# samukallio/path-tracer

Measured on AMD Instinct MI355X. Metric: Mrays/s + Msamples/s, Viking Room 1920x1080 1024spp, 1/2/4/8 GPUs, higher is better.
Workload: dtype f32; 1 GPU; C3 scene, one 1920x1080 1024-spp frame per step (Reset, Run(2), Run(1) until the frame's sample count reaches 1024 x pixels); each of 1 GPU(s) renders every pixel with its own RNG stream to 1/1 of the samples, then the reduce of radiance + sample counts to rank 0; spp_target=1024, streams=1, slots_per_launch_rank0=2073600, split=3, class_lists=False, frame_target_samples_rank0=2123366400, mesh_faces=3976, parallelism=sample-shards x1

## Files before the change

include/pt_api.h:

```cpp
#ifndef PT_API_H
#define PT_API_H

#include <stdint.h>
#include "pt_packed.h"

#ifdef __cplusplus
extern "C" {
#endif

typedef struct pt_device pt_device;
typedef struct pt_scene pt_scene;
typedef struct pt_sample_buffer pt_sample_buffer;
typedef struct pt_basic_renderer pt_basic_renderer;
typedef struct pt_comm pt_comm;
typedef struct pt_preview pt_preview;
typedef struct pt_denoise_guides pt_denoise_guides;

typedef struct pt_basic_renderer_params {
    uint32_t FrameIndex;
    uint32_t CameraIndex;
    uint32_t RenderFlags;
    uint32_t PathLengthLimit;
    float    PathTerminationProbability;
} pt_basic_renderer_params;

typedef struct pt_hit_record {
    float    time;
    uint32_t shape_material;
    uint32_t packed_normal;
    uint32_t packed_tangent;
    float    u, v;
} pt_hit_record;

typedef struct pt_pixel_state {
    float    origin[3];
    uint32_t packed_velocity;
    pt_hit_record hit;
    float    lambda0;
    float    throughput[4];
    float    probability[4];
    float    sample[3];
    uint32_t active01, active23;
} pt_pixel_state;

enum {
    PT_KERNEL_RAYGEN  = 0,
    PT_KERNEL_EXTEND  = 1,
    PT_KERNEL_SHADE   = 2,
    PT_KERNEL_RESOLVE = 3,
    PT_KERNEL_PREVIEW = 4,
    PT_KERNEL_ROUND   = 5,
    PT_KERNEL_ROUNDS  = 6,
    PT_KERNEL_DENOISE = 7,
    PT_KERNEL_GUIDES  = 8,
    PT_KERNEL_STATS   = 9,
    PT_KERNEL_REPROJECT = 10,
    PT_KERNEL_COUNT   = 11,
};

enum {
    PT_TONE_MAPPING_CLAMP    = 0,
    PT_TONE_MAPPING_REINHARD = 1,
    PT_TONE_MAPPING_HABLE    = 2,
    PT_TONE_MAPPING_ACES     = 3,
};

enum {
    PT_PREVIEW_RENDER_MODE_BASE_COLOR        = 0,
    PT_PREVIEW_RENDER_MODE_BASE_COLOR_SHADED = 1,
    PT_PREVIEW_RENDER_MODE_NORMAL            = 2,
    PT_PREVIEW_RENDER_MODE_MATERIAL_INDEX    = 3,
    PT_PREVIEW_RENDER_MODE_PRIMITIVE_INDEX   = 4,
    PT_PREVIEW_RENDER_MODE_MESH_COMPLEXITY   = 5,
    PT_PREVIEW_RENDER_MODE_SCENE_COMPLEXITY  = 6,
};

typedef struct pt_preview_parameters {
    pt_packed_transform CameraTransform;
    uint32_t RenderMode;
    float    Brightness;
    uint32_t SelectedShapeIndex;
    uint32_t RenderSizeX, RenderSizeY;
    uint32_t MouseX, MouseY;
} pt_preview_parameters;

typedef struct pt_preview_aov {
    float    time;
    uint32_t shape_index;
    uint32_t material_index;
    uint32_t primitive_index;
    uint32_t mesh_complexity;
    uint32_t scene_complexity;
    float    normal[3];
    float    u, v;
    uint32_t reserved;
} pt_preview_aov;

typedef struct pt_resolve_parameters {
    float    Brightness;
    uint32_t ToneMappingMode;
    float    ToneMappingWhiteLevel;
} pt_resolve_parameters;

const char* ptGetLastError(void);

pt_device* ptCreateDevice(int hip_device);
void       ptDestroyDevice(pt_device* device);
int        ptSynchronize(pt_device* device);
int        ptGetDeviceCount(int* count);

pt_scene* ptCreateScene(pt_device* device);
int       ptUpdateScene(pt_device* device, pt_scene* scene, const pt_scene_packs* packs, uint32_t dirty_flags);
void      ptDestroyScene(pt_device* device, pt_scene* scene);
enum {
    PT_STACK_FORMAT_AUTO       = 0,
    PT_STACK_FORMAT_WORDS32    = 1,
    PT_STACK_FORMAT_NODE_INDEX = 2,
    PT_HIT_RECORD_AUTO         = 0,
    PT_HIT_RECORD_FACE_INDEX   = 1,
};
int       ptSetSceneStackFormat(pt_scene* scene, uint32_t format);
int       ptSetSceneHitRecordForm(pt_scene* scene, uint32_t form);
enum {
    PT_EXTEND_FORM_AUTO    = 0,
    PT_EXTEND_FORM_GENERAL = 1,
    PT_EXTEND_FORM_MESH    = 2,
};
int       ptSetSceneExtendForm(pt_scene* scene, uint32_t form);
int       ptGetSceneExtendForm(pt_scene* scene, uint32_t* form);
int       ptSceneStackNeeded(pt_scene* scene, uint32_t* entries);
int       ptSceneNodeCache(pt_scene* scene, uint32_t* pairs);

pt_sample_buffer* ptCreateSampleBuffer(pt_device* device, uint32_t width, uint32_t height);
void              ptDestroySampleBuffer(pt_device* device, pt_sample_buffer* buffer);
int               ptReadSampleBuffer(pt_device* device, pt_sample_buffer* buffer, float* rgba);
int               ptWriteSampleBuffer(pt_device* device, pt_sample_buffer* buffer, const float* rgba);
int               ptRenderSampleBuffer(pt_device* device, pt_sample_buffer* buffer, const pt_resolve_parameters* params);
int               ptReadResolvedImage(pt_device* device, pt_sample_buffer* buffer, float* rgba);
int               ptReadResolvedImageSRGB8(pt_device* device, pt_sample_buffer* buffer, uint8_t* rgba8);

pt_basic_renderer* ptCreateBasicRenderer(pt_device* device, pt_scene* scene, pt_sample_buffer* buffer);
pt_basic_renderer* ptCreateBasicRendererPartitioned(pt_device* device, pt_scene* scene, pt_sample_buffer* buffer,
                                                    uint32_t rank, uint32_t nranks);
pt_basic_renderer* ptCreateBasicRendererStreams(pt_device* device, pt_scene* scene, pt_sample_buffer* buffer,
                                                uint32_t rank, uint32_t nranks, uint32_t streams);
int                ptMergeBasicRendererStreams(pt_device* device, pt_basic_renderer* renderer);
uint32_t           ptBasicRendererStreams(pt_basic_renderer* renderer);
void               ptDestroyBasicRenderer(pt_device* device, pt_basic_renderer* renderer);
pt_basic_renderer_params* ptBasicRendererParams(pt_basic_renderer* renderer);
int                ptResetBasicRenderer(pt_device* device, pt_basic_renderer* renderer);
int                ptRunBasicRenderer(pt_device* device, pt_basic_renderer* renderer, uint32_t rounds);
uint32_t           ptBasicRendererSlotCount(pt_basic_renderer* renderer);
int                ptSetBasicRendererFusedRounds(pt_basic_renderer* renderer, int mode);
int                ptRunBasicRendererRounds(pt_device* device, pt_basic_renderer* renderer, uint32_t count);
int                ptSetBasicRendererRoundBatch(pt_basic_renderer* renderer, uint32_t rounds);
#define PT_MAX_SPLIT 4
int                ptSetBasicRendererClassLists(pt_basic_renderer* renderer, uint32_t mode);
int                ptGetBasicRendererClassLists(const pt_basic_renderer* renderer, uint32_t* used);
enum { PT_RAY_ORDER_AUTO = 0, PT_RAY_ORDER_OCTANT = 1, PT_RAY_ORDER_LENGTH = 2 };
int                ptSetBasicRendererRayOrder(pt_basic_renderer* renderer, uint32_t order);
int                ptGetBasicRendererRayOrder(const pt_basic_renderer* renderer, uint32_t* order, uint32_t* used);
int                ptReadSceneLengthTable(pt_device* device, pt_scene* scene, uint8_t* classes, uint32_t* trained,
                                          uint64_t* rounds);
int                ptReadBasicRendererRayPositions(pt_device* device, pt_basic_renderer* renderer, uint16_t* positions);
int                ptSetBasicRendererSplit(pt_basic_renderer* renderer, uint32_t groups);
int                ptGetBasicRendererSplit(const pt_basic_renderer* renderer, uint32_t* groups, uint32_t* timed_tiles,
                                           uint32_t* tiles);
int                ptSetBasicRendererActiveTiles(pt_device* device, pt_basic_renderer* renderer, const uint8_t* mask,
                                                 uint32_t tiles);
int                ptGetBasicRendererActiveTiles(const pt_basic_renderer* renderer, uint32_t* active, uint32_t* tiles);
int                ptSetBasicRendererOpenPBR(pt_basic_renderer* renderer, int enable);
int                ptGetStats(pt_device* device, pt_basic_renderer* renderer, uint64_t* rays, uint64_t* samples);
int                ptRenderFrame(pt_device* device, pt_basic_renderer* renderer, uint64_t target_samples,
                                 uint32_t max_rounds, uint32_t* rounds_out, uint64_t* samples_out);
int                ptReadBasicRendererState(pt_device* device, pt_basic_renderer* renderer, pt_pixel_state* out);
int                ptReadBasicRendererStreamState(pt_device* device, pt_basic_renderer* renderer, uint32_t stream,
                                                  pt_pixel_state* out);
int                ptWriteBasicRendererState(pt_device* device, pt_basic_renderer* renderer, const pt_pixel_state* in);
int                ptWriteBasicRendererStreamState(pt_device* device, pt_basic_renderer* renderer, uint32_t stream,
                                                   const pt_pixel_state* in);
int                ptReadBasicRendererStreamAccumulator(pt_device* device, pt_basic_renderer* renderer, uint32_t stream,
                                                        float* rgba);
int                ptWriteBasicRendererStreamAccumulator(pt_device* device, pt_basic_renderer* renderer,
                                                         uint32_t stream, const float* rgba);

enum {
    PT_SHADE_DIFFUSE     = 1,
    PT_SHADE_METAL       = 2,
    PT_SHADE_TRANSLUCENT = 4,
    PT_SHADE_SCATTER     = 8,
    PT_SHADE_OPENPBR     = 16,
    PT_SHADE_PRIMS       = 32,
    PT_SHADE_SKY         = 64,
    PT_SHADE_TEXWRAP     = 128,
};
typedef struct pt_shade_info {
    uint32_t scene_mask;
    uint32_t kernel_mask;
    uint32_t completion_queue;
    uint32_t grey_records;
    uint32_t ray_order;
    uint32_t length_trained;
} pt_shade_info;
int                ptGetBasicRendererShadeInfo(pt_basic_renderer* renderer, pt_shade_info* info);

pt_preview* ptCreatePreviewRenderContext(pt_device* device, pt_scene* scene);
void        ptDestroyPreviewRenderContext(pt_device* device, pt_preview* context);
int         ptRenderPreview(pt_device* device, pt_preview* context, const pt_preview_parameters* params);
int         ptRetrievePreviewQueryResult(pt_device* device, pt_preview* context, uint32_t* hit_shape_index);
int         ptReadPreviewImage(pt_device* device, pt_preview* context, float* rgba);
int         ptReadPreviewAOVs(pt_device* device, pt_preview* context, pt_preview_aov* aov);

pt_denoise_guides* ptCreateDenoiseGuides(pt_device* device, uint32_t width, uint32_t height);
void ptDestroyDenoiseGuides(pt_device* device, pt_denoise_guides* guides);
int  ptRenderDenoiseGuides(pt_device* device, pt_scene* scene, pt_denoise_guides* guides, uint32_t camera_index);
#define PT_GUIDE_MAX_BOUNCES 8
int  ptRenderDenoiseGuidesSpecular(pt_device* device, pt_scene* scene, pt_denoise_guides* guides,
                                   uint32_t camera_index, uint32_t max_bounces);
int  ptReadDenoiseGuides(pt_device* device, pt_denoise_guides* guides, pt_denoise_guide* out);
int  ptWriteDenoiseGuides(pt_device* device, pt_denoise_guides* guides, const pt_denoise_guide* in);
int  ptDenoiseSampleBuffer(pt_device* device, pt_sample_buffer* src, pt_denoise_guides* guides,
                           const pt_denoise_parameters* params, pt_sample_buffer* dst);
enum {
    PT_DENOISE_VARIANT_AUTO    = 0,
    PT_DENOISE_VARIANT_GATHER  = 1,
    PT_DENOISE_VARIANT_LATTICE = 2,
};
int  ptSetDenoiseVariant(pt_denoise_guides* guides, uint32_t variant);
int  ptDenoiseSampleBufferPair(pt_device* device, pt_sample_buffer* a, pt_sample_buffer* b, pt_denoise_guides* guides,
                               const pt_denoise_pair_parameters* params, pt_sample_buffer* dst);
int  ptDespikeSampleBuffer(pt_device* device, pt_sample_buffer* src, pt_denoise_guides* guides,
                           const pt_despike_parameters* params, pt_sample_buffer* dst);

int  ptReprojectSampleBuffer(pt_device* device, pt_sample_buffer* prev, pt_denoise_guides* prev_guides,
                             const pt_packed_camera* prev_camera, pt_denoise_guides* guides,
                             const pt_packed_camera* camera, const pt_reproject_parameters* params,
                             pt_sample_buffer* dst);
int  ptReprojectSampleBufferMoving(pt_device* device, pt_sample_buffer* prev, pt_denoise_guides* prev_guides,
                                   const pt_packed_camera* prev_camera, pt_denoise_guides* guides,
                                   const pt_packed_camera* camera, const pt_shape_motion* motion,
                                   uint32_t motion_count, const pt_reproject_parameters* params,
                                   pt_sample_buffer* dst);
int  ptRectifyHistory(pt_device* device, pt_sample_buffer* history, pt_sample_buffer* current,
                      pt_denoise_guides* guides, const pt_rectify_parameters* params, pt_sample_buffer* dst);

int  ptComputeFrameStatistics(pt_device* device, pt_sample_buffer* a, pt_sample_buffer* b,
                              pt_frame_statistics* out);
int  ptComputeTileStatistics(pt_device* device, pt_sample_buffer* a, pt_sample_buffer* b, float noise_threshold,
                             pt_tile_statistics* out);
int  ptAccumulateSampleBuffer(pt_device* device, pt_sample_buffer* dst, pt_sample_buffer* src);
enum {
    PT_STATS_VARIANT_AUTO    = 0,
    PT_STATS_VARIANT_PLAIN   = 1,
    PT_STATS_VARIANT_UNIFORM = 2,
};
int  ptSetFrameStatisticsVariant(pt_device* device, uint32_t variant);

int ptTraceRays(pt_device* device, pt_scene* scene, uint32_t n, const float* origins,
                const uint32_t* packed_velocities, const float* durations, pt_hit_record* out);

int ptCheckFastDivision(pt_device* device, uint64_t n, uint32_t seed, uint64_t* mismatches);

int ptCheckFastReciprocal(pt_device* device, uint64_t* mismatches);

int ptEvalNumerics(pt_device* device, uint32_t op, uint32_t n, const uint32_t* a, const uint32_t* b,
                   const uint32_t* c, uint32_t* out);

int ptSampleTextures(pt_device* device, pt_scene* scene, uint32_t n, const uint32_t* texture_index,
                     const float* uv, uint32_t wrap, float* rgba);

#define PT_EXTEND_STATS_COUNT 14
int ptExtendStats(pt_device* device, pt_basic_renderer* renderer, uint64_t out[PT_EXTEND_STATS_COUNT]);
int ptExtendStepCounts(pt_device* device, pt_basic_renderer* renderer, uint32_t* steps);

int ptTraceRaysStats(pt_device* device, pt_scene* scene, uint32_t n, const float* origins,
                     const uint32_t* packed_velocities, const float* durations,
                     uint64_t out[PT_EXTEND_STATS_COUNT], uint32_t* steps);

int ptSetProfiling(pt_device* device, int enable);
int ptSetProfilingPeriod(pt_device* device, uint32_t period);
int ptGetKernelStats(pt_device* device, int kernel, uint64_t* launches, double* total_ms);
int ptGetKernelRounds(pt_device* device, int kernel, uint64_t* rounds);
int ptResetKernelStats(pt_device* device);

enum {
    PT_ERROR_COMM_ABORTED = -2,
    PT_ERROR_TIMEOUT      = -3,
};
int      ptCommGetUniqueId(uint8_t id[128]);
pt_comm* ptCommCreate(pt_device* device, int nranks, int rank, const uint8_t id[128]);
void     ptCommDestroy(pt_comm* comm);
int      ptCommSetTimeout(pt_comm* comm, double seconds);
int      ptCommReduceSampleBuffer(pt_device* device, pt_comm* comm, pt_sample_buffer* buffer, int root);
int      ptCommGatherSampleBuffer(pt_device* device, pt_comm* comm, pt_sample_buffer* buffer, int root);
int      ptCommReduceSampleBufferInto(pt_device* device, pt_comm* comm, pt_sample_buffer* buffer,
                                      pt_sample_buffer* total, int root);

#ifdef __cplusplus
}
#endif

#endif
```

path-tracer_amd/_native.py:

```python
from __future__ import annotations

import ctypes as C
import os
from pathlib import Path

import numpy as np

PKG = Path(__file__).resolve().parent
SCENE_LIB_PATH = PKG / "libptscene.so"
HIP_LIB_PATH = PKG / "libpathtracer.so"


class NativeLibraryMissing(RuntimeError):
    pass



class pt_scene_packs(C.Structure):
    _fields_ = [
        ("globals", C.c_void_p),
        ("textures", C.c_void_p), ("texture_count", C.c_uint32),
        ("material_data", C.c_void_p), ("material_word_count", C.c_uint32),
        ("shapes", C.c_void_p), ("shape_count", C.c_uint32),
        ("shape_nodes", C.c_void_p), ("shape_node_count", C.c_uint32),
        ("mesh_faces", C.c_void_p), ("mesh_face_count", C.c_uint32),
        ("mesh_vertices", C.c_void_p), ("mesh_vertex_count", C.c_uint32),
        ("mesh_nodes", C.c_void_p), ("mesh_node_count", C.c_uint32),
        ("cameras", C.c_void_p), ("camera_count", C.c_uint32),
        ("atlas", C.c_void_p),
        ("atlas_width", C.c_uint32), ("atlas_height", C.c_uint32), ("atlas_layer_count", C.c_uint32),
    ]


class pt_shade_info(C.Structure):
    _fields_ = [("scene_mask", C.c_uint32), ("kernel_mask", C.c_uint32), ("completion_queue", C.c_uint32),
                ("grey_records", C.c_uint32), ("ray_order", C.c_uint32), ("length_trained", C.c_uint32)]


RAY_ORDER_AUTO, RAY_ORDER_OCTANT, RAY_ORDER_LENGTH = 0, 1, 2
RAYKEY_COUNT = 32768


SHADE_DIFFUSE, SHADE_METAL, SHADE_TRANSLUCENT, SHADE_SCATTER = 1, 2, 4, 8
SHADE_OPENPBR, SHADE_PRIMS, SHADE_SKY, SHADE_TEXWRAP = 16, 32, 64, 128


class pt_basic_renderer_params(C.Structure):
    _fields_ = [
        ("FrameIndex", C.c_uint32),
        ("CameraIndex", C.c_uint32),
        ("RenderFlags", C.c_uint32),
        ("PathLengthLimit", C.c_uint32),
        ("PathTerminationProbability", C.c_float),
    ]


class pts_load_model_options(C.Structure):
    _fields_ = [
        ("name", C.c_char_p), ("directory_path", C.c_char_p),
        ("vertex_transform", C.c_float * 16), ("normal_transform", C.c_float * 16),
        ("texcoord_transform", C.c_float * 9), ("openpbr_as_diffuse", C.c_int),
    ]


class pt_resolve_parameters(C.Structure):
    _fields_ = [
        ("Brightness", C.c_float),
        ("ToneMappingMode", C.c_uint32),
        ("ToneMappingWhiteLevel", C.c_float),
    ]


class pt_denoise_parameters(C.Structure):
    _fields_ = [
        ("Iterations", C.c_uint32),
        ("SigmaColor", C.c_float),
        ("SigmaNormal", C.c_float),
        ("SigmaDepth", C.c_float),
        ("SigmaAlbedo", C.c_float),
    ]


class pt_denoise_pair_parameters(C.Structure):
    _fields_ = [
        ("Iterations", C.c_uint32),
        ("SigmaLuminance", C.c_float),
        ("SigmaNormal", C.c_float),
        ("SigmaDepth", C.c_float),
        ("SigmaAlbedo", C.c_float),
    ]


class pt_reproject_parameters(C.Structure):
    _fields_ = [
        ("NormalCosine", C.c_float),
        ("DepthTolerance", C.c_float),
        ("MinWeight", C.c_float),
        ("MaxHistory", C.c_float),
    ]


class pt_rectify_parameters(C.Structure):
    _fields_ = [
        ("Radius", C.c_uint32),
        ("MinNeighbours", C.c_uint32),
        ("Sigma", C.c_float),
        ("ClampedHistory", C.c_float),
        ("NormalCosine", C.c_float),
    ]


assert C.sizeof(pt_rectify_parameters) == 20


class pt_despike_parameters(C.Structure):
    _fields_ = [
        ("Radius", C.c_uint32),
        ("Rank", C.c_uint32),
        ("MinNeighbours", C.c_uint32),
        ("Scale", C.c_float),
        ("Floor", C.c_float),
        ("NormalCosine", C.c_float),
    ]


assert C.sizeof(pt_despike_parameters) == 24

STATS_BINS = 256


class pt_frame_statistics(C.Structure):
    _fields_ = [
        ("pixels", C.c_uint64),
        ("filled", C.c_uint64),
        ("empty", C.c_uint64),
        ("nonfinite", C.c_uint64),
        ("dark", C.c_uint64),
        ("luminance_histogram", C.c_uint32 * STATS_BINS),
        ("min_luminance", C.c_float),
        ("max_luminance", C.c_float),
        ("min_samples", C.c_float),
        ("max_samples", C.c_float),
        ("noise_pixels", C.c_uint64),
        ("noise_skipped", C.c_uint64),
        ("noise_histogram", C.c_uint32 * STATS_BINS),
    ]


TILE_SIZE = 16
TILE_STATS_DTYPE = np.dtype([("filled", "<u4"), ("empty", "<u4"), ("nonfinite", "<u4"), ("pair", "<u4"),
                             ("over", "<u4"), ("min_count", "<f4"), ("max_count", "<f4"), ("reserved", "<u4")])
assert TILE_STATS_DTYPE.itemsize == 32


class pt_packed_transform(C.Structure):
    _fields_ = [("To", C.c_float * 16), ("From", C.c_float * 16)]


class pt_packed_camera(C.Structure):
    _fields_ = [
        ("Model", C.c_uint32),
        ("FocalLength", C.c_float),
        ("ApertureRadius", C.c_float),
        ("SensorDistance", C.c_float),
        ("SensorSize", C.c_float * 2),
        ("Pad0", C.c_uint32 * 2),
        ("Transform", pt_packed_transform),
    ]


class pt_preview_parameters(C.Structure):
    _fields_ = [
        ("CameraTransform", pt_packed_transform),
        ("RenderMode", C.c_uint32),
        ("Brightness", C.c_float),
        ("SelectedShapeIndex", C.c_uint32),
        ("RenderSizeX", C.c_uint32), ("RenderSizeY", C.c_uint32),
        ("MouseX", C.c_uint32), ("MouseY", C.c_uint32),
    ]


class pts_config_info(C.Structure):
    _fields_ = [
        ("width", C.c_uint32), ("height", C.c_uint32), ("spp", C.c_uint32), ("camera_count", C.c_uint32),
        ("render_flags", C.c_uint32), ("termination_probability", C.c_float),
        ("mesh_face_count", C.c_uint32), ("shape_count", C.c_uint32),
    ]


HIT_RECORD_DTYPE = np.dtype([
    ("time", "<f4"), ("shape_material", "<u4"), ("packed_normal", "<u4"),
    ("packed_tangent", "<u4"), ("u", "<f4"), ("v", "<f4"),
])
assert HIT_RECORD_DTYPE.itemsize == 24

PIXEL_STATE_DTYPE = np.dtype([
    ("origin", "<f4", (3,)), ("packed_velocity", "<u4"),
    ("hit", HIT_RECORD_DTYPE),
    ("lambda0", "<f4"), ("throughput", "<f4", (4,)), ("probability", "<f4", (4,)),
    ("sample", "<f4", (3,)), ("active01", "<u4"), ("active23", "<u4"),
])
assert PIXEL_STATE_DTYPE.itemsize == 96

PREVIEW_AOV_DTYPE = np.dtype([
    ("time", "<f4"), ("shape_index", "<u4"), ("material_index", "<u4"), ("primitive_index", "<u4"),
    ("mesh_complexity", "<u4"), ("scene_complexity", "<u4"), ("normal", "<f4", (3,)), ("u", "<f4"), ("v", "<f4"),
    ("reserved", "<u4"),
])
assert PREVIEW_AOV_DTYPE.itemsize == 48

DENOISE_GUIDE_DTYPE = np.dtype([("normal", "<f4", (3,)), ("time", "<f4"), ("albedo", "<f4", (3,)), ("shape", "<u4")])
assert DENOISE_GUIDE_DTYPE.itemsize == 32

SHAPE_NODE_DTYPE = np.dtype([("Minimum", "<f4", (3,)), ("ChildNodeIndices", "<u4"),
                             ("Maximum", "<f4", (3,)), ("ShapeIndex", "<u4")])
MESH_NODE_DTYPE = np.dtype([("Minimum", "<f4", (3,)), ("FaceBeginOrNodeIndex", "<u4"),
                            ("Maximum", "<f4", (3,)), ("FaceEndIndex", "<u4")])
MESH_FACE_DTYPE = np.dtype([("Position0", "<f4", (3,)), ("VertexIndex0", "<u4"),
                            ("Position1", "<f4", (3,)), ("VertexIndex1", "<u4"),
                            ("Position2", "<f4", (3,)), ("VertexIndex2", "<u4")])
MESH_VERTEX_DTYPE = np.dtype([("PackedNormal", "<u4"), ("PackedUV", "<u4")])
TRANSFORM_DTYPE = np.dtype([("To", "<f4", (16,)), ("From", "<f4", (16,))])
SHAPE_DTYPE = np.dtype([("Type", "<i4"), ("MaterialIndex", "<u4"), ("MeshRootNodeIndex", "<u4"),
                        ("Pad0", "<u4"), ("Transform", TRANSFORM_DTYPE)])
CAMERA_DTYPE = np.dtype([("Model", "<u4"), ("FocalLength", "<f4"), ("ApertureRadius", "<f4"),
                         ("SensorDistance", "<f4"), ("SensorSize", "<f4", (2,)), ("Pad0", "<u4", (2,)),
                         ("Transform", TRANSFORM_DTYPE)])
TEXTURE_DTYPE = np.dtype([("AtlasPlacementMinimum", "<f4", (2,)), ("AtlasPlacementMaximum", "<f4", (2,)),
                          ("AtlasImageIndex", "<u4"), ("Type", "<u4"), ("Flags", "<u4"), ("Unused0", "<u4")])
GLOBALS_DTYPE = np.dtype([("SkyboxMeanDirection", "<f4", (3,)), ("SkyboxConcentration", "<f4"),
                          ("SkyboxSamplingProbability", "<f4"), ("SkyboxBrightness", "<f4"),
                          ("SkyboxTextureIndex", "<u4"), ("ShapeCount", "<u4"), ("SceneScatterRate", "<f4"),
                          ("Pad0", "<u4", (3,))])
assert SHAPE_NODE_DTYPE.itemsize == 32 and MESH_NODE_DTYPE.itemsize == 32 and MESH_FACE_DTYPE.itemsize == 48
assert SHAPE_DTYPE.itemsize == 144 and CAMERA_DTYPE.itemsize == 160 and GLOBALS_DTYPE.itemsize == 48
assert TEXTURE_DTYPE.itemsize == 32
SHAPE_MOTION_DTYPE = np.dtype([("Point", "<f4", (12,)), ("Normal", "<f4", (9,)), ("Flags", "<u4"),
                               ("Pad0", "<u4", (2,))])
assert SHAPE_MOTION_DTYPE.itemsize == 96
SHAPE_MOTION_MOVED, SHAPE_MOTION_NO_HISTORY = 1, 2

KERNEL_RAYGEN, KERNEL_EXTEND, KERNEL_SHADE, KERNEL_RESOLVE = 0, 1, 2, 3
TONE_MAPPING_CLAMP, TONE_MAPPING_REINHARD, TONE_MAPPING_HABLE, TONE_MAPPING_ACES = 0, 1, 2, 3
(PREVIEW_RENDER_MODE_BASE_COLOR, PREVIEW_RENDER_MODE_BASE_COLOR_SHADED, PREVIEW_RENDER_MODE_NORMAL,
 PREVIEW_RENDER_MODE_MATERIAL_INDEX, PREVIEW_RENDER_MODE_PRIMITIVE_INDEX, PREVIEW_RENDER_MODE_MESH_COMPLEXITY,
 PREVIEW_RENDER_MODE_SCENE_COMPLEXITY) = range(7)
KERNEL_PREVIEW = 4
KERNEL_ROUND = 5
KERNEL_ROUNDS = 6
MAX_SPLIT = 4
KERNEL_DENOISE = 7
KERNEL_GUIDES = 8
GUIDE_MAX_BOUNCES = 8
DENOISE_MAX_ITERATIONS = 8
DENOISE_VARIANT_AUTO, DENOISE_VARIANT_GATHER, DENOISE_VARIANT_LATTICE = 0, 1, 2
KERNEL_STATS = 9
STATS_VARIANT_AUTO, STATS_VARIANT_PLAIN, STATS_VARIANT_UNIFORM = 0, 1, 2
KERNEL_REPROJECT = 10

NUMERICS_OPS = (
    "add", "mul", "div", "sqrt", "fma", "min", "max", "clamp", "floor", "fract", "rint", "round_half_away", "mix",
    "exp", "log", "pow", "sin", "cos", "atan2", "asin", "u32_to_float", "floor_to_int", "random", "random01",
    "pack_snorm16", "unpack_snorm16", "half_to_float", "pack_unit_vector", "unpack_unit_vector", "fast_rcp", "xdiv",
)
NUMERICS_OPERANDS = {"fma": 3, "clamp": 3, "mix": 3, "pack_unit_vector": 3, "add": 2, "mul": 2, "div": 2, "min": 2,
                     "max": 2, "pow": 2, "atan2": 2, "xdiv": 2}
NUMERICS_OUTPUTS = {"random": 2, "unpack_unit_vector": 3}
NUMERICS_DEVICE_ONLY = ("fast_rcp", "xdiv")

_vp = C.c_void_p
_u32 = C.c_uint32
_f32 = C.c_float
_i32 = C.c_int
_fptr = C.POINTER(C.c_float)
_u32ptr = C.POINTER(C.c_uint32)

SCENE_API = {
    "ptsGetLastError": (C.c_char_p, []),
    "ptsCreateScene": (_vp, []),
    "ptsCreateEmptyScene": (_vp, []),
    "ptsCreateConfigScene": (_vp, [_i32, C.POINTER(pts_config_info)]),
    "ptsDestroyScene": (None, [_vp]),
    "ptsSceneRoot": (_vp, [_vp]),
    "ptsCreateEntity": (_vp, [_vp, _i32, _vp]),
    "ptsSetEntityTransform": (None, [_vp, _vp, _fptr, _fptr, _fptr]),
    "ptsSetEntityActive": (None, [_vp, _vp, _i32]),
    "ptsSetEntityMaterial": (None, [_vp, _vp, _vp]),
    "ptsSetEntityMesh": (None, [_vp, _vp, _vp]),
    "ptsEntityPackedShapeIndex": (_u32, [_vp]),
    "ptsSetCameraPinhole": (None, [_vp, _vp, _f32, _f32]),
    "ptsSetCameraThinLens": (None, [_vp, _vp, _f32, _f32, _f32, _f32, _f32]),
    "ptsSetCamera360": (None, [_vp, _vp]),
    "ptsFindCamera": (_vp, [_vp, _u32]),
    "ptsSetCameraTransform": (None, [_vp, _vp, _fptr, _fptr]),
    "ptsSetRootParameters": (None, [_vp, _f32, _f32, _f32, _vp]),
    "ptsCreateMaterial": (_vp, [_vp, _i32, C.c_char_p]),
    "ptsSetMaterialParameter": (_i32, [_vp, _vp, C.c_char_p, _fptr, _i32]),
    "ptsSetMaterialTexture": (_i32, [_vp, _vp, C.c_char_p, _vp]),
    "ptsMaterialPackedIndex": (_u32, [_vp]),
    "ptsCreateCheckerTexture": (_vp, [_vp, C.c_char_p, _i32, _fptr, _fptr]),
    "ptsCreateTexture": (_vp, [_vp, C.c_char_p, _i32, _u32, _u32, _fptr, _i32]),
    "ptsCreateMesh": (_vp, [_vp, C.c_char_p, _u32, _fptr, _fptr, _fptr, _u32, _u32ptr]),
    "ptsMeshDepth": (_u32, [_vp]),
    "ptsMeshNodeCount": (_u32, [_vp]),
    "ptsMeshFaces": (None, [_vp, _u32ptr]),
    "ptsDefaultLoadModelOptions": (None, [C.POINTER(pts_load_model_options)]),
    "ptsLoadTexture": (_vp, [_vp, C.c_char_p, _i32, C.c_char_p]),
    "ptsLoadImageRGBA8": (_i32, [C.c_char_p, C.POINTER(C.c_uint32), C.POINTER(C.c_uint32), _vp]),
    "ptsLoadModelAsPrefab": (_vp, [_vp, C.c_char_p, C.POINTER(pts_load_model_options)]),
    "ptsInstantiatePrefab": (_vp, [_vp, _vp, _vp]),
    "ptsLoadScene": (_vp, [C.c_char_p]),
    "ptsSaveScene": (_i32, [_vp, C.c_char_p]),
    "ptsSceneTextureCount": (_u32, [_vp]),
    "ptsSceneMaterialCount": (_u32, [_vp]),
    "ptsSceneMeshCount": (_u32, [_vp]),
    "ptsScenePrefabCount": (_u32, [_vp]),
    "ptsPrefabMeshCount": (_u32, [_vp]),
    "ptsPrefabMesh": (_vp, [_vp, _u32, C.POINTER(_vp), _fptr]),
    "ptsMeshVertexCount": (_u32, [_vp]),
    "ptsMeshFaceCount": (_u32, [_vp]),
    "ptsMeshVertices": (None, [_vp, _fptr]),
    "ptsMaterialType": (_i32, [_vp]),
    "ptsPackSceneData": (_u32, [_vp]),
    "ptsGetScenePacks": (None, [_vp, C.POINTER(pt_scene_packs)]),
    "ptsMarkDirty": (None, [_vp, _u32]),
    "ptsGetParametricSpectrumCoefficients": (_i32, [_fptr, _fptr]),
    "ptsBuildSpectrumTable": (_i32, [_i32]),
    "ptsSaveSpectrumTable": (_i32, [C.c_char_p]),
    "ptsLoadSpectrumTable": (_i32, [C.c_char_p]),
    "ptsSetSpectrumTablePath": (None, [C.c_char_p]),
    "ptsDenoise": (_i32, [_u32, _u32, _fptr, _vp, C.POINTER(pt_denoise_parameters), _fptr]),
    "ptsDenoisePair": (_i32, [_u32, _u32, _fptr, _fptr, _vp, C.POINTER(pt_denoise_pair_parameters), _fptr]),
    "ptsReproject": (_i32, [_u32, _u32, _fptr, _vp, C.POINTER(pt_packed_camera), _u32, _u32, _vp,
                            C.POINTER(pt_packed_camera), C.POINTER(pt_reproject_parameters), _fptr]),
    "ptsShapeMotion": (_i32, [_vp, _u32, _vp, _u32, _vp]),
    "ptsReprojectMoving": (_i32, [_u32, _u32, _fptr, _vp, C.POINTER(pt_packed_camera), _u32, _u32, _vp,
                                  C.POINTER(pt_packed_camera), _vp, _u32, C.POINTER(pt_reproject_parameters), _fptr]),
    "ptsRectifyHistory": (_i32, [_u32, _u32, _fptr, _fptr, _vp, C.POINTER(pt_rectify_parameters), _fptr]),
    "ptsDespike": (_i32, [_u32, _u32, _fptr, _vp, C.POINTER(pt_despike_parameters), _fptr]),
    "ptsCentralCameraRay": (_i32, [C.POINTER(pt_packed_camera), _u32, _u32, _u32, _u32, _fptr, _fptr]),
    "ptsFrameStatistics": (_i32, [_u32, _u32, _fptr, _fptr, C.POINTER(pt_frame_statistics)]),
    "ptsTileStatistics": (_i32, [_u32, _u32, _fptr, _fptr, _f32, _vp]),
    "ptsStatsBin": (_i32, [C.c_float]),
    "ptsStatsBinEdge": (C.c_double, [_i32]),
    "ptsStatsPercentileBin": (_i32, [_u32ptr, C.c_double]),
    "ptsStatsLogAverage": (C.c_double, [_u32ptr, C.c_double, C.c_double]),
    "ptsStatsAutoBrightness": (C.c_double, [C.POINTER(pt_frame_statistics), C.c_double, C.c_double, C.c_double]),
    "ptsStatsNoise": (C.c_double, [C.POINTER(pt_frame_statistics), C.c_double]),
    "ptsRayKey": (_u32, [_fptr, _fptr, _fptr, _fptr]),
}

HIP_API = {
    "ptGetLastError": (C.c_char_p, []),
    "ptGetDeviceCount": (_i32, [C.POINTER(_i32)]),
    "ptCreateDevice": (_vp, [_i32]),
    "ptDestroyDevice": (None, [_vp]),
    "ptSynchronize": (_i32, [_vp]),
    "ptCreateScene": (_vp, [_vp]),
    "ptUpdateScene": (_i32, [_vp, _vp, C.POINTER(pt_scene_packs), _u32]),
    "ptSetSceneStackFormat": (_i32, [_vp, _u32]),
    "ptSetSceneHitRecordForm": (_i32, [_vp, _u32]),
    "ptSetSceneExtendForm": (_i32, [_vp, _u32]),
    "ptGetSceneExtendForm": (_i32, [_vp, C.POINTER(C.c_uint32)]),
    "ptDestroyScene": (None, [_vp, _vp]),
    "ptCreateSampleBuffer": (_vp, [_vp, _u32, _u32]),
    "ptDestroySampleBuffer": (None, [_vp, _vp]),
    "ptReadSampleBuffer": (_i32, [_vp, _vp, _fptr]),
    "ptWriteSampleBuffer": (_i32, [_vp, _vp, _fptr]),
    "ptRenderSampleBuffer": (_i32, [_vp, _vp, C.POINTER(pt_resolve_parameters)]),
    "ptReadResolvedImage": (_i32, [_vp, _vp, _fptr]),
    "ptReadResolvedImageSRGB8": (_i32, [_vp, _vp, C.POINTER(C.c_uint8)]),
    "ptCreateBasicRenderer": (_vp, [_vp, _vp, _vp]),
    "ptCreateBasicRendererPartitioned": (_vp, [_vp, _vp, _vp, _u32, _u32]),
    "ptCreateBasicRendererStreams": (_vp, [_vp, _vp, _vp, _u32, _u32, _u32]),
    "ptMergeBasicRendererStreams": (_i32, [_vp, _vp]),
    "ptBasicRendererStreams": (_u32, [_vp]),
    "ptReadBasicRendererStreamState": (_i32, [_vp, _vp, _u32, _vp]),
    "ptWriteBasicRendererState": (_i32, [_vp, _vp, _vp]),
    "ptWriteBasicRendererStreamState": (_i32, [_vp, _vp, _u32, _vp]),
    "ptReadBasicRendererStreamAccumulator": (_i32, [_vp, _vp, _u32, _fptr]),
    "ptWriteBasicRendererStreamAccumulator": (_i32, [_vp, _vp, _u32, _fptr]),
    "ptGetBasicRendererShadeInfo": (_i32, [_vp, C.POINTER(pt_shade_info)]),
    "ptDestroyBasicRenderer": (None, [_vp, _vp]),
    "ptBasicRendererParams": (C.POINTER(pt_basic_renderer_params), [_vp]),
    "ptResetBasicRenderer": (_i32, [_vp, _vp]),
    "ptRunBasicRenderer": (_i32, [_vp, _vp, _u32]),
    "ptBasicRendererSlotCount": (_u32, [_vp]),
    "ptSetBasicRendererFusedRounds": (_i32, [_vp, _i32]),
    "ptRunBasicRendererRounds": (_i32, [_vp, _vp, _u32]),
    "ptSetBasicRendererRoundBatch": (_i32, [_vp, _u32]),
    "ptSetBasicRendererSplit": (_i32, [_vp, _u32]),
    "ptSetBasicRendererClassLists": (_i32, [_vp, _u32]),
    "ptGetBasicRendererClassLists": (_i32, [_vp, _u32ptr]),
    "ptGetBasicRendererSplit": (_i32, [_vp, _u32ptr, _u32ptr, _u32ptr]),
    "ptSetBasicRendererRayOrder": (_i32, [_vp, _u32]),
    "ptGetBasicRendererRayOrder": (_i32, [_vp, _u32ptr, _u32ptr]),
    "ptReadSceneLengthTable": (_i32, [_vp, _vp, _vp, _u32ptr, C.POINTER(C.c_uint64)]),
    "ptReadBasicRendererRayPositions": (_i32, [_vp, _vp, _vp]),
    "ptSetBasicRendererOpenPBR": (_i32, [_vp, _i32]),
    "ptGetStats": (_i32, [_vp, _vp, C.POINTER(C.c_uint64), C.POINTER(C.c_uint64)]),
    "ptTraceRaysStats": (_i32, [_vp, _vp, _u32, _fptr, _u32ptr, _fptr, C.POINTER(C.c_uint64), _vp]),
    "ptRenderFrame": (_i32, [_vp, _vp, C.c_uint64, C.c_uint32, C.POINTER(C.c_uint32), C.POINTER(C.c_uint64)]),
    "ptReadBasicRendererState": (_i32, [_vp, _vp, _vp]),
    "ptTraceRays": (_i32, [_vp, _vp, _u32, _fptr, _u32ptr, _fptr, _vp]),
    "ptCreatePreviewRenderContext": (_vp, [_vp, _vp]),
    "ptDestroyPreviewRenderContext": (None, [_vp, _vp]),
    "ptRenderPreview": (_i32, [_vp, _vp, C.POINTER(pt_preview_parameters)]),
    "ptRetrievePreviewQueryResult": (_i32, [_vp, _vp, C.POINTER(C.c_uint32)]),
    "ptReadPreviewImage": (_i32, [_vp, _vp, _fptr]),
    "ptReadPreviewAOVs": (_i32, [_vp, _vp, _vp]),
    "ptCreateDenoiseGuides": (_vp, [_vp, _u32, _u32]),
    "ptDestroyDenoiseGuides": (None, [_vp, _vp]),
    "ptRenderDenoiseGuides": (_i32, [_vp, _vp, _vp, _u32]),
    "ptRenderDenoiseGuidesSpecular": (_i32, [_vp, _vp, _vp, _u32, _u32]),
    "ptReadDenoiseGuides": (_i32, [_vp, _vp, _vp]),
    "ptWriteDenoiseGuides": (_i32, [_vp, _vp, _vp]),
    "ptDenoiseSampleBuffer": (_i32, [_vp, _vp, _vp, C.POINTER(pt_denoise_parameters), _vp]),
    "ptSetDenoiseVariant": (_i32, [_vp, _u32]),
    "ptDenoiseSampleBufferPair": (_i32, [_vp, _vp, _vp, _vp, C.POINTER(pt_denoise_pair_parameters), _vp]),
    "ptReprojectSampleBuffer": (_i32, [_vp, _vp, _vp, C.POINTER(pt_packed_camera), _vp, C.POINTER(pt_packed_camera),
                                       C.POINTER(pt_reproject_parameters), _vp]),
    "ptReprojectSampleBufferMoving": (_i32, [_vp, _vp, _vp, C.POINTER(pt_packed_camera), _vp,
                                             C.POINTER(pt_packed_camera), _vp, _u32,
                                             C.POINTER(pt_reproject_parameters), _vp]),
    "ptRectifyHistory": (_i32, [_vp, _vp, _vp, _vp, C.POINTER(pt_rectify_parameters), _vp]),
    "ptDespikeSampleBuffer": (_i32, [_vp, _vp, _vp, C.POINTER(pt_despike_parameters), _vp]),
    "ptComputeFrameStatistics": (_i32, [_vp, _vp, _vp, C.POINTER(pt_frame_statistics)]),
    "ptComputeTileStatistics": (_i32, [_vp, _vp, _vp, _f32, _vp]),
    "ptSetBasicRendererActiveTiles": (_i32, [_vp, _vp, _vp, _u32]),
    "ptGetBasicRendererActiveTiles": (_i32, [_vp, _u32ptr, _u32ptr]),
    "ptAccumulateSampleBuffer": (_i32, [_vp, _vp, _vp]),
    "ptSetFrameStatisticsVariant": (_i32, [_vp, _u32]),
    "ptCheckFastDivision": (_i32, [_vp, C.c_uint64, _u32, C.POINTER(C.c_uint64)]),
    "ptCheckFastReciprocal": (_i32, [_vp, C.POINTER(C.c_uint64)]),
    "ptEvalNumerics": (_i32, [_vp, _u32, _u32, _u32ptr, _u32ptr, _u32ptr, _u32ptr]),
    "ptSampleTextures": (_i32, [_vp, _vp, _u32, _u32ptr, _fptr, _u32, _fptr]),
    "ptExtendStats": (_i32, [_vp, _vp, C.POINTER(C.c_uint64)]),
    "ptExtendStepCounts": (_i32, [_vp, _vp, _vp]),
    "ptSetProfilingPeriod": (_i32, [_vp, C.c_uint32]),
    "ptSceneStackNeeded": (_i32, [_vp, C.POINTER(C.c_uint32)]),
    "ptSceneNodeCache": (_i32, [_vp, C.POINTER(C.c_uint32)]),
    "ptSetProfiling": (_i32, [_vp, _i32]),
    "ptGetKernelStats": (_i32, [_vp, _i32, C.POINTER(C.c_uint64), C.POINTER(C.c_double)]),
    "ptGetKernelRounds": (_i32, [_vp, _i32, C.POINTER(C.c_uint64)]),
    "ptResetKernelStats": (_i32, [_vp]),
    "ptCommGetUniqueId": (_i32, [C.POINTER(C.c_uint8)]),
    "ptCommCreate": (_vp, [_vp, _i32, _i32, C.POINTER(C.c_uint8)]),
    "ptCommDestroy": (None, [_vp]),
    "ptCommSetTimeout": (_i32, [_vp, C.c_double]),
    "ptCommReduceSampleBuffer": (_i32, [_vp, _vp, _vp, _i32]),
    "ptCommGatherSampleBuffer": (_i32, [_vp, _vp, _vp, _i32]),
    "ptCommReduceSampleBufferInto": (_i32, [_vp, _vp, _vp, _vp, _i32]),
}

_scene_lib = None
_hip_lib = None


def _bind(lib, table, required=True):
    for name, (res, args) in table.items():
        if not required and not hasattr(lib, name):
            continue
        fn = getattr(lib, name)
        fn.restype = res
        fn.argtypes = args
    return lib


def scene_lib():
    global _scene_lib
    if _scene_lib is None:
        if not SCENE_LIB_PATH.exists():
            raise NativeLibraryMissing(f"{SCENE_LIB_PATH} not built (run __graft_entry__.build())")
        lib = C.CDLL(str(SCENE_LIB_PATH))
        _scene_lib = _bind(lib, SCENE_API)
        table = os.environ.get("PT_SPECTRUM_TABLE")
        if table and Path(table).exists():
            _scene_lib.ptsLoadSpectrumTable(table.encode())
    return _scene_lib


def hip_lib():
    global _hip_lib
    if _hip_lib is None:
        path = Path(os.environ.get("PT_HIP_LIB", str(HIP_LIB_PATH)))
        if not path.exists():
            raise NativeLibraryMissing(f"{path} not built (run __graft_entry__.build())")
        lib = C.CDLL(str(path))
        _hip_lib = _bind(lib, HIP_API, required="PT_HIP_LIB" not in os.environ)
    return _hip_lib


def fptr(a: np.ndarray):
    assert a.dtype == np.float32 and a.flags.c_contiguous
    return a.ctypes.data_as(_fptr)


def u32ptr(a: np.ndarray):
    assert a.dtype == np.uint32 and a.flags.c_contiguous
    return a.ctypes.data_as(_u32ptr)
```

path-tracer_amd/csrc/hip/extend.hip:

```cpp
#include "extend.hpp"
#include "variants.hpp"

namespace ptd {

template <class Src, bool SPILL, int MINW, int CAP, class E = uint32_t, bool NC = false, bool MESH = false,
          bool TRAIN = false>
__global__ __launch_bounds__(256, (MESH && !NC) ? 8 : MINW) void extend_kernel(dscene S, Src src, uint32_t n,
                                                                               uint32_t* spill, uint32_t spill_stride)
{
    __shared__ E smem[CAP * 256];
    __shared__ float4 ncache[NC ? 4 * PT_NODE_CACHE_PAIRS : 1];
    if constexpr (kRendererSource<Src>) {
        if (src.L.stop && *src.L.stop) return;
    }
    const uint32_t ncn = NC ? NodeCacheFill(S, ncache) : 0u;
    uint32_t tile = blockIdx.x;
    bool timed = false;
    if constexpr (kRendererSource<Src>) {
        if (src.L.order) {
            tile = src.L.order[blockIdx.x];
            timed = true;
        }
    }
    ExtendTile<Src, SPILL, CAP, E, MESH, TRAIN>(S, src, n, spill, spill_stride, smem, tile, timed, ncache, ncn);
}

constexpr uint32_t LEN_MEAN_BINS = 4096;
__global__ __launch_bounds__(1024) void length_classes_kernel(uint32_t* sum, uint32_t* cnt, uint8_t* cls)
{
    __shared__ unsigned long long hist[LEN_MEAN_BINS];
    __shared__ unsigned long long part[1024];
    __shared__ uint32_t bound[PT_RAYKEY_CLASSES - 1];
    const uint32_t t = threadIdx.x;
    for (uint32_t i = t; i < LEN_MEAN_BINS; i += 1024) hist[i] = 0;
    if (t < PT_RAYKEY_CLASSES - 1) bound[t] = LEN_MEAN_BINS;
    __syncthreads();
    auto mean = [](uint32_t s, uint32_t c) { return min((s << 4) / c, LEN_MEAN_BINS - 1u); };
    for (uint32_t i = t; i < PT_RAYKEY_COUNT; i += 1024) {
        uint32_t c = cnt[i], s = sum[i];
        if (c > 65535u) {
            const uint32_t sh = 16u - (uint32_t)__clz(c);
            c >>= sh;
            s >>= sh;
            cnt[i] = c;
        }
        s = min(s, 255u * c);
        sum[i] = s;
        if (c) atomicAdd(&hist[mean(s, c)], (unsigned long long)c);
    }
    __syncthreads();
    unsigned long long h[4], own = 0;
#pragma unroll
    for (uint32_t k = 0; k < 4; k++) { h[k] = hist[4 * t + k]; own += h[k]; }
    part[t] = own;
    __syncthreads();
    for (uint32_t o = 1; o < 1024; o <<= 1) {
        const unsigned long long v = t >= o ? part[t - o] : 0ull;
        __syncthreads();
        part[t] += v;
        __syncthreads();
    }
    const unsigned long long total = part[1023];
    unsigned long long before = part[t] - own;
#pragma unroll
    for (uint32_t k = 0; k < 4; k++) {
        const unsigned long long after = before + h[k];
        for (uint32_t j = 1; j < PT_RAYKEY_CLASSES; j++)
            if (before * PT_RAYKEY_CLASSES < j * total && after * PT_RAYKEY_CLASSES >= j * total) bound[j - 1] = 4 * t + k;
        before = after;
    }
    __syncthreads();
    for (uint32_t i = t; i < PT_RAYKEY_COUNT; i += 1024) {
        const uint32_t c = cnt[i];
        uint32_t k = PT_RAYKEY_CLASSES / 2;
        if (c) {
            const uint32_t m = mean(sum[i], c);
            k = 0;
            for (uint32_t j = 0; j < PT_RAYKEY_CLASSES - 1; j++) k += m > bound[j] ? 1u : 0u;
        }
        cls[i] = (uint8_t)k;
    }
}

PT_DEV uint32_t WaveSum(uint32_t v)
{
    for (int o = 32; o > 0; o >>= 1) v += __shfl_xor(v, o, 64);
    return v;
}

PT_DEV uint32_t WaveMax(uint32_t v)
{
    for (int o = 32; o > 0; o >>= 1) v = max(v, (uint32_t)__shfl_xor(v, o, 64));
    return v;
}

template <class Src, bool SPILL, int CAP, class E = uint32_t>
__global__ __launch_bounds__(256) void extend_stats_kernel(dscene S, Src src, uint32_t n, uint32_t* spill,
                                                           uint32_t spill_stride, unsigned long long* out,
                                                           uint32_t* steps)
{
    __shared__ E smem[CAP * 256];
    uint32_t slot = blockIdx.x * 256 + threadIdx.x;
    tstack<SPILL, CAP, E> st;
    st.lds = &smem[threadIdx.x];
    st.spill = spill + slot;
    st.stride = spill_stride;
    lane_stats ss;
    pt3 O, V;
    float D;
    uint32_t ray = 0;
    if (slot < n && src.load(slot, O, V, D)) {
        ray = 1;
        lane_state Ln;
        LaneBegin(S, Ln, O, V, D);
        if (S.g.ShapeCount != 0)
            while (!LaneStep<SPILL, CAP, Src, lane_stats, true, E>(S, Ln, st, src, slot, ss)) {}
        src.store(slot, Ln, S.vidx21 != 0);
    }
    if (steps && slot < n) steps[slot] = ss.steps;
    uint32_t v[14] = {WaveSum(ray), WaveSum(ss.steps), WaveMax(ss.steps) * 64u, WaveSum(ss.internals),
                      WaveSum(ss.leaves), WaveSum(ss.faces), WaveSum(ss.pops), WaveSum(ss.shapes), 1u,
                      WaveSum(ss.uniq[0]), WaveSum(ss.uniq[1]), WaveSum(ss.uniq[2]), WaveSum(ss.uniq[3]),
                      WaveSum(ss.uniq[4])};
    if ((threadIdx.x & 63u) == 0)
        for (int i = 0; i < 14; i++) atomicAdd(&out[i], (unsigned long long)v[i]);
}

}


using ptv::Blocks;

uint32_t pt_extend_stack_cap() { return PT_EXTEND_CAP; }

template <class Src>
static hipError_t LaunchExtend(const ptd::dscene& S, const Src& src, uint32_t n, uint32_t blocks, uint32_t* spill,
                               bool train, hipStream_t st)
{
    constexpr bool renderer = ptd::kRendererSource<Src>;
    if (train && !ptv::HasTrain(renderer, S.single_mesh != 0, spill != nullptr)) return hipErrorNotSupported;
    if (n == 0 || blocks == 0) return hipSuccess;
    ptv::SelectStackEntry(S.stack16 != 0, [&](auto entry) {
        using E = typename decltype(entry)::type;
        const bool cache = S.node_cache && ptv::HasNodeCache<E>(spill != nullptr);
        ptv::SelectFlags(
            [&](auto SPILL, auto NC, auto MESH, auto TRAIN) {
                if constexpr ((!NC || ptv::HasNodeCache<E>(SPILL)) && (!TRAIN || ptv::HasTrain(renderer, MESH, SPILL)))
                    hipLaunchKernelGGL((ptd::extend_kernel<Src, SPILL, PT_EXTEND_MINW, PT_EXTEND_CAP, E, NC, MESH, TRAIN>),
                                       dim3(blocks), dim3(256), 0, st, S, src, n, spill, n);
            },
            spill != nullptr, cache, S.single_mesh != 0, train);
    });
    return hipGetLastError();
}

bool pt_length_train_supported(const ptd::dscene& S, bool spill) { return ptv::HasTrain(true, S.single_mesh != 0, spill); }

hipError_t pt_launch_extend(const ptd::dscene& S, const ptd::dslots& L, const ptd::dframe& F, uint32_t* spill,
                            hipStream_t st, bool train)
{
    if (train && (!L.len_sum || !L.len_cnt || !L.len_cam)) return hipErrorNotSupported;
    return LaunchExtend(S, ptd::ray_source_slots{L, F}, L.n, L.tile_count, spill, train, st);
}

hipError_t pt_launch_trace_rays(const ptd::dscene& S, uint32_t n, const float* origins, const uint32_t* vel,
                                const float* dur, float4* hit, float2* hc, float4* rec, float2* uv, uint32_t* spill,
                                hipStream_t st)
{
    hipError_t e = LaunchExtend(S, ptd::ray_source_arrays{origins, vel, dur, hit, hc}, n, Blocks(n), spill, false, st);
    if (e != hipSuccess) return e;
    return pt_launch_finalize(S, n, hit, hc, rec, uv, st);
}

template <class Src>
static hipError_t LaunchExtendStats(const ptd::dscene& S, const Src& src, uint32_t n, uint32_t* spill,
                                    unsigned long long* out, uint32_t* steps, hipStream_t st)
{
    if (n == 0) return hipSuccess;
    ptv::SelectStackEntry(S.stack16 != 0, [&](auto entry) {
        using E = typename decltype(entry)::type;
        ptv::SelectFlags(
            [&](auto SPILL) {
                hipLaunchKernelGGL((ptd::extend_stats_kernel<Src, SPILL, PT_EXTEND_CAP, E>), dim3(Blocks(n)), dim3(256),
                                   0, st, S, src, n, spill, n, out, steps);
            },
            spill != nullptr);
    });
    return hipGetLastError();
}

hipError_t pt_launch_trace_rays_stats(const ptd::dscene& S, uint32_t n, const float* origins, const uint32_t* vel,
                                      const float* dur, float4* hit, float2* hc, uint32_t* spill,
                                      unsigned long long* out, uint32_t* steps, hipStream_t st)
{
    return LaunchExtendStats(S, ptd::ray_source_arrays{origins, vel, dur, hit, hc}, n, spill, out, steps, st);
}

hipError_t pt_launch_extend_stats(const ptd::dscene& S, const ptd::dslots& L, const ptd::dframe& F, uint32_t* spill,
                                  unsigned long long* out, uint32_t* steps, hipStream_t st)
{
    return LaunchExtendStats(S, ptd::ray_source_slots{L, F}, L.n, spill, out, steps, st);
}

hipError_t pt_launch_length_classes(uint32_t* sum, uint32_t* cnt, uint8_t* cls, hipStream_t st)
{
    hipLaunchKernelGGL(ptd::length_classes_kernel, dim3(1), dim3(1024), 0, st, sum, cnt, cls);
    return hipGetLastError();
}
```

path-tracer_amd/csrc/hip/extend.hpp:

```cpp
#pragma once

#include "path.hpp"

#include <type_traits>

namespace ptd {


struct ray_source_slots {
    dslots L;
    dframe F;
    PT_DEV bool load(uint32_t s, pt3& O, pt3& V, float& D) const
    {
        if (!PositionValid(F, s)) return false;
        float4 r = L.ray[s];
        O = v3(r.x, r.y, r.z);
        V = UnpackUnitVector(__float_as_uint(r.w));
        D = PT_HIT_TIME_LIMIT;
        return true;
    }
    PT_DEV void store(uint32_t s, const lane_state& Ln, bool vidx21) const
    {
        L.hit[s] = CompactHit(Ln, vidx21);
        L.uv[s] = make_float2(Ln.C.y, Ln.C.z);
    }
    PT_DEV void outcome(uint32_t q, uint32_t cls, bool classes) const
    {
        uint64_t* m = L.outcome + (size_t)(q >> 8) * (4 * PT_OUTCOME_CLASSES) + ((q >> 6) & 3u);
        if (!classes) {
            uint64_t b = __ballot(cls == PT_OUTCOME_CLASSES - 1);
            if ((q & 63u) == 0) m[4 * (PT_OUTCOME_CLASSES - 1)] = b;
            return;
        }
#pragma unroll
        for (uint32_t c = 0; c < PT_OUTCOME_CLASSES; c++) {
            uint64_t b = __ballot(cls == c);
            if ((q & 63u) == 0) m[4 * c] = b;
        }
    }
};

struct ray_source_arrays {
    PT_DEV void outcome(uint32_t, uint32_t, bool) const {}
    const float* origins;
    const uint32_t* vel;
    const float* dur;
    float4* hit;
    float2* hc;
    PT_DEV bool load(uint32_t i, pt3& O, pt3& V, float& D) const
    {
        O = v3(origins[3 * i], origins[3 * i + 1], origins[3 * i + 2]);
        V = UnpackUnitVector(vel[i]);
        D = dur[i];
        return true;
    }
    PT_DEV void store(uint32_t i, const lane_state& Ln, bool vidx21) const
    {
        hit[i] = CompactHit(Ln, vidx21);
        hc[i] = make_float2(Ln.C.y, Ln.C.z);
    }
};

template <class Src>
constexpr bool kRendererSource = std::is_same<Src, ray_source_slots>::value;

template <bool SPILL, int CAP, class E, bool MESH = false, bool TRAIN = false, class Src>
PT_DEV void ExtendRay(const dscene& S, const Src& src, tstack<SPILL, CAP, E>& st, uint32_t slot)
{
    static_assert(!TRAIN || (MESH && kRendererSource<Src>), "training counts the mesh-only loop's steps");
    pt3 O, V;
    float D;
    uint32_t cls = 0;
    if (src.load(slot, O, V, D)) {
        lane_state Ln;
        if constexpr (MESH && TRAIN) {
            uint32_t steps = 0;
            MeshBegin(S, Ln, O, V, D);
            if (Ln.exact) {
                while (!MeshStep<true>(S, Ln, st)) steps++;
            } else {
                while (!MeshStep<false>(S, Ln, st)) steps++;
            }
            if (Ln.Shape == 0xFFFFFFFEu) Ln.Shape = 0;
            if ((slot & 255u) >= src.L.len_cam[slot >> 8]) {
                const float4 r = src.L.ray[slot];
                const pt3 W = UnpackUnitVector(__float_as_uint(r.w));
                const uint32_t key = pt_ray_key(r.x, r.y, r.z, W.x, W.y, W.z, &src.L.len_bounds);
                atomicAdd(&src.L.len_sum[key], min(steps, 255u));
                atomicAdd(&src.L.len_cnt[key], 1u);
            }
        } else if constexpr (MESH) {
            MeshBegin(S, Ln, O, V, D);
            if (Ln.exact) {
                while (!MeshStep<true>(S, Ln, st)) {}
            } else {
                while (!MeshStep<false>(S, Ln, st)) {}
            }
            if (Ln.Shape == 0xFFFFFFFEu) Ln.Shape = 0;
        } else {
            LaneBegin(S, Ln, O, V, D);
            no_stats ns;
            if (S.g.ShapeCount != 0) {
                while (!LaneStep<SPILL, CAP, Src, no_stats, true, E>(S, Ln, st, src, slot, ns)) {}
            }
        }
        src.store(slot, Ln, S.vidx21 != 0);
        if (Ln.Shape == SHAPE_INDEX_NONE) {
            cls = 4;
        } else if (S.mat_classes) {
            uint32_t T = S.material[32 * (size_t)S.shapes[Ln.Shape].MaterialIndex];
            cls = T == PT_MATERIAL_TYPE_BASIC_DIFFUSE ? 0u
                : T == PT_MATERIAL_TYPE_BASIC_METAL ? 1u
                : T == PT_MATERIAL_TYPE_BASIC_TRANSLUCENT ? 2u : 3u;
        }
    }
    src.outcome(slot, cls, S.mat_classes != 0);
}

template <class Src, bool SPILL, int CAP, class E, bool MESH = false, bool TRAIN = false>
PT_DEV void ExtendTile(const dscene& S, const Src& src, uint32_t n, uint32_t* spill, uint32_t spill_stride, E* smem,
                       uint32_t tile, bool timed, const float4* nc = nullptr, uint32_t ncn = 0)
{
    uint64_t t0 = timed ? __builtin_amdgcn_s_memtime() : 0;
    uint32_t slot = tile * 256 + threadIdx.x;
    if (slot >= n) return;
    tstack<SPILL, CAP, E> st;
    st.lds = &smem[threadIdx.x];
    st.spill = spill + slot;
    st.stride = spill_stride;
    st.nc = nc;
    st.ncn = ncn;
    ExtendRay<SPILL, CAP, E, MESH, TRAIN>(S, src, st, slot);
    if constexpr (kRendererSource<Src>) {
        if (timed && (threadIdx.x & 63u) == 0)
            src.L.tilecost[tile * 4 + (threadIdx.x >> 6)] = (uint32_t)(__builtin_amdgcn_s_memtime() - t0);
    }
}

PT_DEV uint32_t NodeCacheFill(const dscene& S, float4* nc)
{
    const uint32_t nodes = min(S.node_cache, 2u * PT_NODE_CACHE_PAIRS);
    for (uint32_t i = threadIdx.x; i < 2 * nodes; i += 256) nc[i] = S.mesh_nodes[i];
    __syncthreads();
    return nodes;
}

}
```

path-tracer_amd/csrc/hip/kernels.hip:

```cpp
#include "pt_device.hpp"
#include "kernels.hpp"
#include "variants.hpp"

namespace ptd {

__global__ __launch_bounds__(1024) void tile_order_kernel(const uint32_t* cost, uint32_t* order, uint32_t tiles,
                                                          uint32_t groups, uint32_t group, uint32_t start)
{
    const uint32_t nt = pt_tile_group_count(tiles, groups, group);
    __shared__ uint32_t count[512];
    for (uint32_t i = threadIdx.x; i < 512; i += 1024) count[i] = 0;
    __syncthreads();
    auto key = [&](uint32_t t) -> uint32_t {
        uint32_t c = max(max(cost[4 * t], cost[4 * t + 1]), max(cost[4 * t + 2], cost[4 * t + 3]));
        if (c < 16) return 511u;
        uint32_t e = 31u - __clz(c);
        uint32_t m = (c >> (e - 4)) & 15u;
        uint32_t k = min(e * 16u + m, 511u);
        return 511u - k;
    };
    for (uint32_t i = threadIdx.x; i < nt; i += 1024) atomicAdd(&count[key(pt_tile_group_tile(tiles, groups, group, i))], 1u);
    __syncthreads();
    __shared__ uint32_t wsum[8];
    uint32_t c = 0, incl = 0;
    if (threadIdx.x < 512) {
        c = count[threadIdx.x];
        incl = c;
        for (int o = 1; o < 64; o <<= 1) {
            uint32_t t = (uint32_t)__shfl_up((int)incl, o, 64);
            if ((threadIdx.x & 63u) >= (uint32_t)o) incl += t;
        }
        if ((threadIdx.x & 63u) == 63u) wsum[threadIdx.x >> 6] = incl;
    }
    __syncthreads();
    if (threadIdx.x < 512) {
        uint32_t before = 0;
        for (uint32_t w = 0; w < (threadIdx.x >> 6); w++) before += wsum[w];
        count[threadIdx.x] = before + incl - c;
    }
    __syncthreads();
    for (uint32_t i = threadIdx.x; i < nt; i += 1024) {
        const uint32_t t = pt_tile_group_tile(tiles, groups, group, i);
        order[start + atomicAdd(&count[key(t)], 1u)] = t;
    }
}

__global__ __launch_bounds__(1024) void guard_kernel(const uint32_t* done, uint32_t words, unsigned long long target,
                                                     uint32_t* flags)
{
    __shared__ unsigned long long part[1024];
    unsigned long long s = 0;
    for (uint32_t i = threadIdx.x; i < words; i += 1024) s += done[i];
    part[threadIdx.x] = s;
    __syncthreads();
    for (uint32_t h = 512; h > 0; h >>= 1) {
        if (threadIdx.x < h) part[threadIdx.x] += part[threadIdx.x + h];
        __syncthreads();
    }
    if (threadIdx.x == 0 && flags[0] == 0u) {
        if (part[0] >= target) flags[0] = 1u;
        else flags[1] += 1u;
    }
}

__global__ __launch_bounds__(256) void vertex_decode_kernel(const uint2* v, uint32_t n, float4* attr, float* vv)
{
    uint32_t i = blockIdx.x * 256 + threadIdx.x;
    if (i >= n) return;
    uint2 V = v[i];
    pt3 N = UnpackUnitVector(V.x);
    attr[i] = make_float4(N.x, N.y, N.z, pt_half_to_float(V.y & 0xFFFF));
    vv[i] = pt_half_to_float(V.y >> 16);
}

__global__ __launch_bounds__(256) void atlas_tile_kernel(const float4* src, float4* dst, uint32_t w, uint32_t h,
                                                         uint64_t texels)
{
    for (uint64_t i = (uint64_t)blockIdx.x * 256 + threadIdx.x; i < texels; i += (uint64_t)gridDim.x * 256) {
        uint64_t plane = (uint64_t)w * h;
        uint64_t layer = i / plane, r = i - layer * plane;
        uint32_t blk = (uint32_t)(r >> 3), in = (uint32_t)(r & 7u);
        uint32_t by = blk / (w >> 2), bx = blk - by * (w >> 2);
        uint32_t x = bx * 4 + (in & 3u), y = by * 2 + (in >> 2);
        dst[i] = src[layer * plane + (uint64_t)y * w + x];
    }
}

__global__ __launch_bounds__(256) void merge_streams_kernel(float4* accum, float4* accx, uint32_t width, uint32_t height,
                                                            uint32_t rank, uint32_t nranks, uint32_t streams)
{
    const size_t frame = (size_t)width * height;
    for (uint32_t y = blockIdx.y; y < height; y += gridDim.y) {
        if (((y >> 4) % nranks) != rank) continue;
        for (uint32_t x = blockIdx.x * 256 + threadIdx.x; x < width; x += gridDim.x * 256) {
            const size_t p = (size_t)y * width + x;
            float4 v = accx[p];
            for (uint32_t k = 1; k < streams; k++) {
                float4 a = accx[(size_t)k * frame + p];
                v.x = v.x + a.x; v.y = v.y + a.y; v.z = v.z + a.z; v.w = v.w + a.w;
            }
            accum[p] = v;
        }
    }
}

__global__ __launch_bounds__(256) void zero_unowned_kernel(float4* accum, uint32_t width, uint32_t height,
                                                           uint32_t rank, uint32_t nranks)
{
    for (uint32_t y = blockIdx.y; y < height; y += gridDim.y) {
        if (((y >> 4) % nranks) == rank) continue;
        for (uint32_t x = blockIdx.x * 256 + threadIdx.x; x < width; x += gridDim.x * 256)
            accum[(size_t)y * width + x] = make_float4(0, 0, 0, 0);
    }
}

__global__ __launch_bounds__(256) void rcp_check_kernel(unsigned long long* mismatches)
{
    uint64_t i = (uint64_t)blockIdx.x * 256 + threadIdx.x;
    uint64_t stride = (uint64_t)gridDim.x * 256;
    unsigned long long bad = 0;
    for (; i < (1ull << 32); i += stride) {
        float d = __uint_as_float((uint32_t)i);
        if (!FastRcpRange(d)) continue;
        bad += __float_as_uint(FastRcp(d)) != __float_as_uint(1.0f / d);
    }
    if (bad) atomicAdd(mismatches, bad);
}

__global__ __launch_bounds__(256) void xdiv_check_kernel(uint64_t n, uint32_t seed, unsigned long long* mismatches)
{
    uint64_t i = (uint64_t)blockIdx.x * 256 + threadIdx.x;
    uint64_t stride = (uint64_t)gridDim.x * 256;
    unsigned long long bad = 0;
    for (; i < n; i += stride) {
        uint32_t s = (uint32_t)i * 2654435761u ^ seed;
        uint32_t ra = pt_random(&s), rb = pt_random(&s), rc = pt_random(&s);
        float a = pt_u2f(((87u + (ra >> 26) + (rc & 15)) << 23) | (ra & 0x7fffffu) | ((rc >> 31) << 31));
        float b = pt_u2f(((107u + ((rb >> 27) & 31)) << 23) | (rb & 0x7fffffu) | (((rc >> 30) & 1u) << 31));
        if ((rc & 0xff0) == 0) a = 0.0f;
        if ((rc & 0xff00) == 0) b = 0.0f;
        float y = RecipForDiv(b);
        float q = XDiv(a, b, y);
        float e = a / b;
        if (pt_f2u(q) != pt_f2u(e) && !(q != q && e != e)) bad++;
    }
    if (bad) atomicAdd(mismatches, bad);
}

}


using ptv::Blocks;

hipError_t pt_launch_vertex_decode(const uint2* v, uint32_t n, float4* attr, float* vv, hipStream_t st)
{
    if (n == 0) return hipSuccess;
    hipLaunchKernelGGL(ptd::vertex_decode_kernel, dim3(Blocks(n)), dim3(256), 0, st, v, n, attr, vv);
    return hipGetLastError();
}

hipError_t pt_launch_guard(const uint32_t* done, uint32_t words, uint64_t target, uint32_t* flags, hipStream_t st)
{
    hipLaunchKernelGGL(ptd::guard_kernel, dim3(1), dim3(1024), 0, st, done, words, (unsigned long long)target, flags);
    return hipGetLastError();
}

hipError_t pt_launch_tile_order(const ptd::dslots& L, hipStream_t st, uint32_t groups, uint32_t group)
{
    if (!L.order || L.tile_count == 0 || groups == 0 || group >= groups) return hipSuccess;
    hipLaunchKernelGGL(ptd::tile_order_kernel, dim3(1), dim3(1024), 0, st, L.tilecost, L.order, L.tile_count, groups,
                       group, pt_tile_group_start(L.tile_count, groups, group));
    return hipGetLastError();
}

hipError_t pt_launch_atlas_tile(const float4* src, float4* dst, uint32_t w, uint32_t h, uint32_t layers, hipStream_t st)
{
    uint64_t texels = (uint64_t)w * h * layers;
    if (texels == 0) return hipSuccess;
    uint64_t blocks = (texels + 255) / 256;
    hipLaunchKernelGGL(ptd::atlas_tile_kernel, dim3((uint32_t)(blocks < 65536 ? blocks : 65536)), dim3(256), 0, st, src,
                       dst, w, h, texels);
    return hipGetLastError();
}

hipError_t pt_launch_merge_streams(float4* accum, float4* accx, uint32_t width, uint32_t height, uint32_t rank,
                                   uint32_t nranks, uint32_t streams, hipStream_t st)
{
    if (streams <= 1 || width == 0 || height == 0) return hipSuccess;
    hipLaunchKernelGGL(ptd::merge_streams_kernel, dim3(Blocks(width), height < 32768u ? height : 32768u), dim3(256), 0,
                       st, accum, accx, width, height, rank, nranks, streams);
    return hipGetLastError();
}

hipError_t pt_launch_zero_unowned(float4* accum, uint32_t width, uint32_t height, uint32_t rank, uint32_t nranks,
                                  hipStream_t st)
{
    if (nranks <= 1 || width == 0 || height == 0) return hipSuccess;
    hipLaunchKernelGGL(ptd::zero_unowned_kernel, dim3(Blocks(width), height < 32768u ? height : 32768u), dim3(256), 0,
                       st, accum, width, height, rank, nranks);
    return hipGetLastError();
}

hipError_t pt_launch_rcp_check(unsigned long long* mismatches, hipStream_t st)
{
    hipLaunchKernelGGL(ptd::rcp_check_kernel, dim3(8192), dim3(256), 0, st, mismatches);
    return hipGetLastError();
}

hipError_t pt_launch_xdiv_check(uint64_t n, uint32_t seed, unsigned long long* mismatches, hipStream_t st)
{
    hipLaunchKernelGGL(ptd::xdiv_check_kernel, dim3(4096), dim3(256), 0, st, n, seed, mismatches);
    return hipGetLastError();
}
```

path-tracer_amd/csrc/hip/kernels.hpp:

```cpp
#pragma once

#include <hip/hip_runtime.h>
#include <stdint.h>
#include "../../../include/pt_packed.h"
#include "../../../include/pt_api.h"
#include "../../../include/pt_raykey.h"

namespace ptd {

struct dscene;

constexpr uint32_t PT_OUTCOME_CLASSES = 5;

struct dslots {
    float4* ray;
    float4* hit;
    float2* uv;
    float4* thr;
    float4* prob;
    float* prob1;
    float* lam;
    uint2* act;
    uint16_t* pos;
    uint8_t* slotof;
    uint64_t* outcome;
    uint32_t* tilecost;
    uint32_t* order;
    uint32_t* done;
    uint32_t* spill;
    const uint32_t* stop = nullptr;
    uint32_t n;
    uint32_t tile_count;
    uint32_t len_order = 0;
    const uint8_t* len_cls = nullptr;
    uint16_t* len_cam = nullptr;
    uint32_t* len_sum = nullptr;
    uint32_t* len_cnt = nullptr;
    pt_raykey_bounds len_bounds{};
};

struct dframe {
    float4* accum;
    uint32_t width, height;
    uint32_t rank, nranks;
    uint32_t tiles_x;
    uint32_t tiles_x_magic;
    uint32_t streams;
    uint32_t stream_tiles;
    uint32_t stream_magic;
    float4* accx;
};

struct dparams {
    uint32_t camera_index;
    uint32_t render_flags;
    float termination_probability;
    uint32_t seed;
    uint32_t rounds = 1;
    uint32_t seed_step = 0;
};

}

hipError_t pt_launch_raygen(const ptd::dscene& S, const ptd::dslots& L, const ptd::dframe& F, const ptd::dparams& P,
                            hipStream_t st);
hipError_t pt_launch_extend(const ptd::dscene& S, const ptd::dslots& L, const ptd::dframe& F, uint32_t* spill,
                            hipStream_t st, bool train = false);
bool pt_length_train_supported(const ptd::dscene& S, bool spill);
bool pt_length_order_supported(uint32_t scene_mats);
hipError_t pt_launch_length_classes(uint32_t* sum, uint32_t* cnt, uint8_t* cls, hipStream_t st);
hipError_t pt_launch_extend_stats(const ptd::dscene& S, const ptd::dslots& L, const ptd::dframe& F, uint32_t* spill,
                                  unsigned long long* out, uint32_t* steps, hipStream_t st);
enum : uint32_t {
    PT_MATS_DIFFUSE = 1,
    PT_MATS_METAL = 2,
    PT_MATS_TRANSLUCENT = 4,
    PT_MATS_SCATTER = 8,
    PT_MATS_ALL = 15,
    PT_MATS_OPENPBR = 16,
    PT_MATS_PRIMS = 32,
    PT_MATS_SKY = 64,
    PT_MATS_SCENE = PT_MATS_PRIMS | PT_MATS_SKY,
    PT_MATS_TEXWRAP = 128,
};
uint32_t pt_shade_mats(uint32_t scene_mats);
constexpr bool pt_grey_mats(uint32_t shade_mats) { return !(shade_mats & (PT_MATS_TRANSLUCENT | PT_MATS_OPENPBR)); }
hipError_t pt_launch_restore_rays(const ptd::dslots& L, const ptd::dframe& F, const float4* rays, uint32_t tile0,
                                  uint32_t tiles, hipStream_t st);
hipError_t pt_launch_grey_check(const ptd::dslots& L, const ptd::dframe& F, uint32_t* count, hipStream_t st);
hipError_t pt_launch_grey_convert(const ptd::dslots& L, const ptd::dframe& F, float* prob1, bool to_grey,
                                  hipStream_t st);
constexpr uint32_t PT_OBSERVE_TABLE_FLOATS = 16 * 5;
hipError_t pt_launch_observe_table(float* table, hipStream_t st);
hipError_t pt_launch_preview(const ptd::dscene& S, const pt_preview_parameters* p, uint32_t* spill, float4* out,
                             pt_preview_aov* aov, uint32_t* query, const float* observe_table, hipStream_t st);
uint32_t pt_preview_stack_cap();
hipError_t pt_launch_resolve(const float4* accum, uint32_t n, float brightness, uint32_t mode, float white, float4* out,
                             uint32_t* out8, hipStream_t st);
hipError_t pt_launch_denoise_guides(const ptd::dscene& S, uint32_t camera_index, uint32_t w, uint32_t h,
                                    uint32_t* spill, float4* guides, const float* observe_table, hipStream_t st);
hipError_t pt_launch_denoise_guides_specular(const ptd::dscene& S, uint32_t camera_index, uint32_t max_bounces,
                                             uint32_t w, uint32_t h, uint32_t* spill, float4* guides,
                                             const float* observe_table, hipStream_t st);
uint32_t pt_guides_stack_cap();
hipError_t pt_launch_denoise(const float4* in, bool accumulator, const float4* guides, uint32_t w, uint32_t h,
                             const pt_denoise_parameters* p, uint32_t iteration, bool lattice, float4* out,
                             hipStream_t st);
hipError_t pt_launch_denoise_mean(const float4* accum, uint32_t n, float4* out, hipStream_t st);
hipError_t pt_launch_denoise_pair_prepare(const float4* a, const float4* b, const float4* guides, uint32_t w,
                                          uint32_t h, bool final, float4* out, hipStream_t st);
hipError_t pt_launch_denoise_pair(const float4* in, const float4* guides, uint32_t w, uint32_t h,
                                  const pt_denoise_pair_parameters* p, uint32_t iteration, bool last, bool lattice,
                                  float4* out, hipStream_t st);
uint32_t pt_frame_statistics_grid(uint64_t n, uint32_t cu_count);
hipError_t pt_launch_frame_statistics(const float4* a, const float4* b, uint64_t n, uint32_t cu_count, bool uniform,
                                      pt_frame_statistics* out, hipStream_t st);
hipError_t pt_launch_tile_statistics(const float4* a, const float4* b, uint32_t width, uint32_t height,
                                     float threshold, pt_tile_statistics* out, hipStream_t st);
hipError_t pt_launch_reproject(const float4* prev, const float4* prev_guides, uint32_t wp, uint32_t hp,
                               const pt_packed_camera* prev_camera, const float4* guides, uint32_t w, uint32_t h,
                               const pt_packed_camera* camera, const pt_shape_motion* motion, uint32_t motion_count,
                               const pt_reproject_parameters* p, float4* out, hipStream_t st);
hipError_t pt_launch_rectify(const float4* hist, const float4* cur, const float4* guides, uint32_t w, uint32_t h,
                             const pt_rectify_parameters* p, float4* out, hipStream_t st);
hipError_t pt_launch_despike(const float4* src, const float4* guides, uint32_t w, uint32_t h,
                             const pt_despike_parameters* p, float4* out, hipStream_t st);
hipError_t pt_launch_accumulate(float4* dst, const float4* src, uint64_t n, hipStream_t st);
hipError_t pt_launch_shade(const ptd::dscene& S, const ptd::dslots& L, const ptd::dframe& F, const ptd::dparams& P,
                           uint32_t scene_mats, bool compact, hipStream_t st);
constexpr uint32_t CQ_SUB = 1;
inline uint32_t pt_classq_sub_capacity(uint32_t tiles) { return (tiles + CQ_SUB - 1) / CQ_SUB * 256; }
bool pt_class_lists_supported(uint32_t scene_mats);
hipError_t pt_launch_shade_classq(const ptd::dscene& S, const ptd::dslots& L, const ptd::dframe& F,
                                  const ptd::dparams& P, uint32_t scene_mats, bool compact, uint32_t* counts,
                                  uint32_t* next_counts, uint32_t* list, hipStream_t st, uint32_t tiles_all = 0,
                                  uint32_t groups = 1, uint32_t group = 0);
hipError_t pt_launch_vertex_decode(const uint2* v, uint32_t n, float4* attr, float* vv, hipStream_t st);
__host__ __device__ inline uint32_t pt_tile_group_count(uint32_t tiles, uint32_t groups, uint32_t group)
{
    return group < tiles ? (tiles - group + groups - 1) / groups : 0u;
}
__host__ __device__ inline uint32_t pt_tile_group_tile(uint32_t tiles, uint32_t groups, uint32_t group, uint32_t i)
{
    return group + i * groups;
}
__host__ __device__ inline uint32_t pt_tile_group_start(uint32_t tiles, uint32_t groups, uint32_t group)
{
    uint32_t s = 0;
    for (uint32_t h = 0; h < group; h++) s += pt_tile_group_count(tiles, groups, h);
    return s;
}
hipError_t pt_launch_tile_order(const ptd::dslots& L, hipStream_t st, uint32_t groups = 1, uint32_t group = 0);
hipError_t pt_launch_guard(const uint32_t* done, uint32_t words, uint64_t target, uint32_t* flags, hipStream_t st);
uint32_t pt_round_capacity(uint32_t scene_mats, bool stack16, uint32_t cu_count);
hipError_t pt_launch_round(const ptd::dscene& S, const ptd::dslots& L, const ptd::dframe& F, const ptd::dparams& P,
                           uint32_t scene_mats, hipStream_t st);
hipError_t pt_launch_rounds(const ptd::dscene& S, const ptd::dslots& L, const ptd::dframe& F, const ptd::dparams& P,
                            uint32_t scene_mats, hipStream_t st);
bool pt_rounds_available(const ptd::dslots& L);
hipError_t pt_launch_zero_unowned(float4* accum, uint32_t width, uint32_t height, uint32_t rank, uint32_t nranks,
                                  hipStream_t st);
hipError_t pt_launch_merge_streams(float4* accum, float4* accx, uint32_t width, uint32_t height, uint32_t rank,
                                   uint32_t nranks, uint32_t streams, hipStream_t st);
hipError_t pt_launch_atlas_tile(const float4* src, float4* dst, uint32_t w, uint32_t h, uint32_t layers, hipStream_t st);
hipError_t pt_launch_rcp_check(unsigned long long* mismatches, hipStream_t st);
hipError_t pt_launch_xdiv_check(uint64_t n, uint32_t seed, unsigned long long* mismatches, hipStream_t st);
hipError_t pt_launch_trace_rays_stats(const ptd::dscene& S, uint32_t n, const float* origins, const uint32_t* vel,
                                      const float* dur, float4* hit, float2* hc, uint32_t* spill,
                                      unsigned long long* out, uint32_t* steps, hipStream_t st);
hipError_t pt_launch_trace_rays(const ptd::dscene& S, uint32_t n, const float* origins, const uint32_t* vel,
                                const float* dur, float4* hit, float2* hc, float4* rec, float2* uv, uint32_t* spill,
                                hipStream_t st);
hipError_t pt_launch_finalize(const ptd::dscene& S, uint32_t n, const float4* hit, const float2* hc, float4* rec,
                              float2* uv, hipStream_t st);
uint32_t pt_extend_stack_cap();
hipError_t pt_launch_numerics_probe(uint32_t op, uint32_t n, const uint32_t* a, const uint32_t* b, const uint32_t* c,
                                    uint32_t* out, hipStream_t st);
hipError_t pt_launch_sample_textures(const ptd::dscene& S, uint32_t n, const uint32_t* index, const float2* uv,
                                     bool unit_wrap, float4* rgba, hipStream_t st);
```

path-tracer_amd/csrc/hip/rt_renderer.hip:

```cpp
#include "runtime.hpp"

using namespace ptrt;

extern "C" {

pt_basic_renderer* ptCreateBasicRendererStreams(pt_device* d, pt_scene* s, pt_sample_buffer* b, uint32_t rank,
                                                uint32_t nranks, uint32_t streams)
{
    if (!d || !s || !b) { SetError("null argument"); return nullptr; }
    if (nranks == 0 || rank >= nranks) { SetError("bad partition %u/%u", rank, nranks); return nullptr; }
    if (streams == 0 || streams > 256) { SetError("bad stream count %u (1..256)", streams); return nullptr; }
    if (hipSetDevice(d->id) != hipSuccess) { SetError("hipSetDevice failed"); return nullptr; }
    pt_basic_renderer* r = new pt_basic_renderer;
    r->dev = d;
    r->scene = s;
    r->buffer = b;
    r->rank = rank;
    r->nranks = nranks;
    r->tiles_x = (b->width + 15) / 16;
    uint32_t bands = (b->height + 15) / 16;
    uint32_t owned = bands > rank ? (bands - rank + nranks - 1) / nranks : 0;
    const uint64_t T = (uint64_t)owned * r->tiles_x;
    uint64_t n = T * streams * 256;
    if (T * r->tiles_x >= (1ull << 32) || (streams > 1 && T * T * streams >= (1ull << 32))) {
        SetError("frame too large");
        delete r;
        return nullptr;
    }
    if (n > 0xFFFFFFFFull / 2) { SetError("too many slots"); delete r; return nullptr; }
    uint32_t ns = (uint32_t)n;
    const size_t tiles = ns / 256, frame_px = (size_t)b->width * b->height;
    bool ok = r->ray.alloc_zero(ns) == hipSuccess && r->hit.alloc_zero(ns) == hipSuccess &&
              r->thr.alloc_zero(ns) == hipSuccess && r->prob.alloc_zero(ns) == hipSuccess &&
              r->prob1.alloc_zero(ns) == hipSuccess && r->grey_count.alloc(1) == hipSuccess &&
              r->lam.alloc_zero(ns) == hipSuccess && r->uv.alloc_zero(ns) == hipSuccess &&
              r->act.alloc_zero(ns) == hipSuccess && r->pos.alloc(ns) == hipSuccess && r->slotof.alloc(ns) == hipSuccess &&
              r->outcome.alloc_zero(tiles * 4 * ptd::PT_OUTCOME_CLASSES + 1) == hipSuccess &&
              r->tilecost.alloc_zero(tiles * 4 + 1) == hipSuccess && r->order.alloc(tiles + 1) == hipSuccess &&
              r->done.alloc_zero(ns / 64 + 1) == hipSuccess &&
              (streams == 1 || r->accx.alloc_zero((size_t)streams * frame_px) == hipSuccess);
    if (ok && ns) {
        std::vector<uint16_t> pos(ns);
        std::vector<uint8_t> slotof(ns);
        for (uint32_t i = 0; i < ns; i++) { pos[i] = (uint16_t)(((i & 255u) << 8) | (i & 255u)); slotof[i] = (uint8_t)(i & 255u); }
        std::vector<uint32_t> order(tiles);
        for (uint32_t t = 0; t < tiles; t++) order[t] = t;
        ok = hipMemcpy(r->pos.ptr, pos.data(), (size_t)ns * 2, hipMemcpyHostToDevice) == hipSuccess &&
             hipMemcpy(r->slotof.ptr, slotof.data(), ns, hipMemcpyHostToDevice) == hipSuccess &&
             hipMemcpy(r->order.ptr, order.data(), tiles * 4, hipMemcpyHostToDevice) == hipSuccess;
    }
    if (!ok) {
        SetError("renderer slot allocation failed (%u slots)", ns);
        delete r;
        return nullptr;
    }
    r->streams = streams;
    r->stream_tiles = (uint32_t)T;
    r->slots.ray = r->ray.ptr;
    r->slots.hit = r->hit.ptr;
    r->slots.uv = r->uv.ptr;
    r->slots.thr = r->thr.ptr;
    r->slots.prob = r->prob.ptr;
    r->slots.lam = r->lam.ptr;
    r->slots.act = r->act.ptr;
    r->slots.pos = r->pos.ptr;
    r->slots.slotof = r->slotof.ptr;
    r->slots.outcome = r->outcome.ptr;
    r->slots.tilecost = r->tilecost.ptr;
    r->slots.order = ns ? r->order.ptr : nullptr;
    r->slots.done = r->done.ptr;
    r->slots.spill = nullptr;
    r->slots.n = ns;
    r->slots.tile_count = ns / 256;
    for (uint32_t band = rank; band < bands; band += nranks)
        r->pixels += (uint64_t)b->width * std::min<uint32_t>(16u, b->height - band * 16u);
    r->valid_slots = r->pixels * streams;
    b->rank = rank;
    b->nranks = nranks;
    return r;
}

pt_basic_renderer* ptCreateBasicRendererPartitioned(pt_device* d, pt_scene* s, pt_sample_buffer* b, uint32_t rank,
                                                    uint32_t nranks)
{
    return ptCreateBasicRendererStreams(d, s, b, rank, nranks, 1);
}

int ptMergeBasicRendererStreams(pt_device* d, pt_basic_renderer* r)
{
    if (!d || !r || !r->buffer) { SetError("null argument"); return -1; }
    if (r->streams == 1) return 0;
    PT_HIP(hipSetDevice(d->id));
    PT_HIP(pt_launch_merge_streams(r->buffer->accum, r->accx.ptr, r->buffer->width, r->buffer->height, r->rank,
                                   r->nranks, r->streams, d->stream));
    return 0;
}

uint32_t ptBasicRendererStreams(pt_basic_renderer* r) { return r ? r->streams : 0; }

pt_basic_renderer* ptCreateBasicRenderer(pt_device* d, pt_scene* s, pt_sample_buffer* b)
{
    return ptCreateBasicRendererPartitioned(d, s, b, 0, 1);
}

void ptDestroyBasicRenderer(pt_device* d, pt_basic_renderer* r)
{
    if (!r) return;
    if (d) { (void)hipSetDevice(d->id); (void)DeviceWait(d); }
    delete r;
}

pt_basic_renderer_params* ptBasicRendererParams(pt_basic_renderer* r) { return r ? &r->params : nullptr; }
uint32_t ptBasicRendererSlotCount(pt_basic_renderer* r) { return r ? r->slots.n : 0; }

int ptResetBasicRenderer(pt_device* d, pt_basic_renderer* r)
{
    if (!d) { SetError("null device"); return -1; }
    if (CheckReady(r) != 0) return -1;
    PT_HIP(hipSetDevice(d->id));
    r->grey = GreyForm(r);
    r->grey_blocked = false;
    r->slots.prob1 = r->grey ? r->prob1.ptr : nullptr;
    if (int e = SyncRayOrder(r)) return e;
    r->len_cam_stale = false;
    PT_TIMED(d, PT_KERNEL_RAYGEN,
             pt_launch_raygen(r->scene->d, r->slots, Frame(r), Params(r, r->params.FrameIndex), d->stream));
    PT_HIP(hipMemsetAsync(r->done.ptr, 0, (size_t)(r->slots.n / 64 + 1) * 4, d->stream));
    r->rays = 0;
    return 0;
}

int ptSetBasicRendererRoundBatch(pt_basic_renderer* r, uint32_t rounds)
{
    if (!r) { SetError("ptSetBasicRendererRoundBatch: null renderer"); return -1; }
    r->round_batch = rounds;
    return 0;
}

int ptSetBasicRendererClassLists(pt_basic_renderer* r, uint32_t mode)
{
    if (!r || mode > 1) { SetError("ptSetBasicRendererClassLists: bad argument (0 automatic, 1 off)"); return -1; }
    r->class_lists = mode;
    return 0;
}

int ptGetBasicRendererClassLists(const pt_basic_renderer* r, uint32_t* used)
{
    if (!r || !used) { SetError("ptGetBasicRendererClassLists: null argument"); return -1; }
    *used = ClassListRounds(r) ? 1u : 0u;
    return 0;
}

int ptSetBasicRendererRayOrder(pt_basic_renderer* r, uint32_t order)
{
    if (!r || order > PT_RAY_ORDER_LENGTH) {
        SetError("ptSetBasicRendererRayOrder: bad argument (0 automatic, 1 octant, 2 length)");
        return -1;
    }
    r->ray_order = order;
    return 0;
}

int ptGetBasicRendererRayOrder(const pt_basic_renderer* r, uint32_t* order, uint32_t* used)
{
    if (!r) { SetError("ptGetBasicRendererRayOrder: null renderer"); return -1; }
    if (used && (!r->scene || !r->scene->valid)) {
        SetError("renderer: scene has no valid packs (call ptUpdateScene)");
        return -1;
    }
    if (order) *order = r->ray_order;
    if (used) *used = LengthOrder(r) ? PT_RAY_ORDER_LENGTH : PT_RAY_ORDER_OCTANT;
    return 0;
}

int ptReadBasicRendererRayPositions(pt_device* d, pt_basic_renderer* r, uint16_t* positions)
{
    if (!d || !r || !positions) { SetError("ptReadBasicRendererRayPositions: null argument"); return -1; }
    PT_HIP(hipSetDevice(d->id));
    PT_WAIT(d);
    if (r->slots.n) PT_HIP(hipMemcpy(positions, r->pos.ptr, (size_t)r->slots.n * 2, hipMemcpyDeviceToHost));
    return 0;
}

int ptSetBasicRendererSplit(pt_basic_renderer* r, uint32_t groups)
{
    if (!r || groups > PT_MAX_SPLIT) {
        SetError("ptSetBasicRendererSplit: bad argument (groups 0..%u)", PT_MAX_SPLIT);
        return -1;
    }
    r->split = groups;
    return 0;
}

int ptGetBasicRendererSplit(const pt_basic_renderer* r, uint32_t* groups, uint32_t* timed_tiles, uint32_t* tiles)
{
    if (!r) { SetError("ptGetBasicRendererSplit: null renderer"); return -1; }
    const uint32_t K = SplitGroups(r);
    if (groups) *groups = K;
    if (timed_tiles) *timed_tiles = pt_tile_group_count(r->slots.tile_count, K, 0);
    if (tiles) *tiles = r->slots.tile_count;
    return 0;
}

int ptSetBasicRendererFusedRounds(pt_basic_renderer* r, int mode)
{
    if (!r || mode < 0 || mode > 2) { SetError("ptSetBasicRendererFusedRounds: bad argument"); return -1; }
    r->fused = mode;
    return 0;
}

int ptSetBasicRendererOpenPBR(pt_basic_renderer* r, int enable)
{
    if (!r || enable < 0 || enable > 1) { SetError("ptSetBasicRendererOpenPBR: bad argument"); return -1; }
    r->openpbr = enable;
    return 0;
}

int ptGetStats(pt_device* d, pt_basic_renderer* r, uint64_t* rays, uint64_t* samples)
{
    if (!d || !r) { SetError("null argument"); return -1; }
    PT_HIP(hipSetDevice(d->id));
    PT_WAIT(d);
    if (rays) *rays = r->rays;
    if (samples) {
        std::vector<uint32_t> w(r->slots.n / 64 + 1);
        PT_HIP(hipMemcpy(w.data(), r->done.ptr, w.size() * 4, hipMemcpyDeviceToHost));
        uint64_t sum = 0;
        for (uint32_t v : w) sum += v;
        *samples = sum;
    }
    return 0;
}

int ptReadBasicRendererStreamState(pt_device* d, pt_basic_renderer* r, uint32_t stream, pt_pixel_state* out)
{
    if (!d || !r || !out) { SetError("null argument"); return -1; }
    if (stream >= r->streams) { SetError("stream %u >= the renderer's %u streams", stream, r->streams); return -1; }
    PT_HIP(hipSetDevice(d->id));
    PT_WAIT(d);
    uint32_t n = r->slots.n;
    std::vector<float4> ray(n), hit(n), thr(n), prob(n);
    std::vector<float> lam(n);
    std::vector<float2> uv(n);
    std::vector<uint2> act(n);
    std::vector<uint16_t> pos(n);
    if (n && r->scene->valid) {
        dbuf<float4> rec;
        dbuf<float2> ruv;
        PT_HIP(rec.alloc(n));
        PT_HIP(ruv.alloc(n));
        PT_HIP(pt_launch_finalize(r->scene->d, n, r->hit.ptr, r->uv.ptr, rec.ptr, ruv.ptr, d->stream));
        PT_HIP(hipStreamSynchronize(d->stream));
        PT_HIP(hipMemcpy(hit.data(), rec.ptr, (size_t)n * 16, hipMemcpyDeviceToHost));
        PT_HIP(hipMemcpy(uv.data(), ruv.ptr, (size_t)n * 8, hipMemcpyDeviceToHost));
    }
    PT_HIP(hipMemcpy(ray.data(), r->ray.ptr, (size_t)n * 16, hipMemcpyDeviceToHost));
    PT_HIP(hipMemcpy(thr.data(), r->thr.ptr, (size_t)n * 16, hipMemcpyDeviceToHost));
    if (r->grey) {
        std::vector<float> p1(n);
        PT_HIP(hipMemcpy(p1.data(), r->prob1.ptr, (size_t)n * 4, hipMemcpyDeviceToHost));
        for (uint32_t i = 0; i < n; i++) prob[i] = make_float4(p1[i], p1[i], p1[i], p1[i]);
    } else {
        PT_HIP(hipMemcpy(prob.data(), r->prob.ptr, (size_t)n * 16, hipMemcpyDeviceToHost));
    }
    PT_HIP(hipMemcpy(lam.data(), r->lam.ptr, (size_t)n * 4, hipMemcpyDeviceToHost));
    PT_HIP(hipMemcpy(act.data(), r->act.ptr, (size_t)n * 8, hipMemcpyDeviceToHost));
    PT_HIP(hipMemcpy(pos.data(), r->pos.ptr, (size_t)n * 2, hipMemcpyDeviceToHost));
    uint32_t W = r->buffer->width, H = r->buffer->height;
    auto bits = [](float f) { uint32_t u; std::memcpy(&u, &f, 4); return u; };
    const uint32_t s0 = stream * r->stream_tiles * 256, s1 = s0 + r->stream_tiles * 256;
    for (uint32_t s = s0; s < s1; s++) {
        uint32_t t = (s >> 8) - stream * r->stream_tiles, l = s & 255u, k = t / r->tiles_x, tx = t - k * r->tiles_x;
        uint32_t x = tx * 16 + (l & 15u), y = (r->rank + k * r->nranks) * 16 + (l >> 4);
        if (x >= W || y >= H) continue;
        pt_pixel_state& O = out[(size_t)y * W + x];
        uint32_t qr = (s & ~255u) | (pos[s] >> 8u), qh = (s & ~255u) | (pos[s] & 255u);
        O.origin[0] = ray[qr].x; O.origin[1] = ray[qr].y; O.origin[2] = ray[qr].z;
        O.packed_velocity = bits(ray[qr].w);
        O.hit.time = hit[qh].x;
        O.hit.shape_material = bits(hit[qh].y);
        O.hit.packed_normal = bits(hit[qh].z);
        O.hit.packed_tangent = bits(hit[qh].w);
        O.hit.u = uv[qh].x;
        O.hit.v = uv[qh].y;
        O.lambda0 = lam[s];
        O.throughput[0] = thr[s].x; O.throughput[1] = thr[s].y; O.throughput[2] = thr[s].z; O.throughput[3] = thr[s].w;
        O.probability[0] = prob[s].x; O.probability[1] = prob[s].y; O.probability[2] = prob[s].z; O.probability[3] = prob[s].w;
        O.sample[0] = O.sample[1] = O.sample[2] = 0.0f;
        O.active01 = act[s].x;
        O.active23 = act[s].y;
    }
    return 0;
}

int ptReadBasicRendererState(pt_device* d, pt_basic_renderer* r, pt_pixel_state* out)
{
    return ptReadBasicRendererStreamState(d, r, 0, out);
}

int ptWriteBasicRendererStreamState(pt_device* d, pt_basic_renderer* r, uint32_t stream, const pt_pixel_state* in)
{
    if (!d || !in) { SetError("null argument"); return -1; }
    if (CheckReady(r) != 0) return -1;
    if (stream >= r->streams) { SetError("stream %u >= the renderer's %u streams", stream, r->streams); return -1; }
    const uint32_t W = r->buffer->width, H = r->buffer->height;
    const uint32_t shapes = r->scene->d.g.ShapeCount;
    const uint32_t T = r->stream_tiles, s0 = stream * T * 256;
    std::vector<float4> ray((size_t)T * 256), thr((size_t)T * 256), prob((size_t)T * 256);
    std::vector<float> lam((size_t)T * 256);
    std::vector<uint2> act((size_t)T * 256);
    for (uint32_t i = 0; i < T * 256; i++) {
        const uint32_t t = i >> 8, l = i & 255u, k = t / r->tiles_x, tx = t - k * r->tiles_x;
        const uint32_t x = tx * 16 + (l & 15u), y = (r->rank + k * r->nranks) * 16 + (l >> 4);
        ray[i] = make_float4(0, 0, 0, 0);
        thr[i] = prob[i] = make_float4(0, 0, 0, 0);
        lam[i] = 0.0f;
        act[i] = make_uint2(0xFFFFFFFFu, 0xFFFFFFFFu);
        if (x >= W || y >= H) continue;
        const pt_pixel_state& S = in[(size_t)y * W + x];
        if (S.sample[0] != 0.0f || S.sample[1] != 0.0f || S.sample[2] != 0.0f) {
            SetError("pixel (%u, %u): a live path's sample is 0 between rounds", x, y);
            return -1;
        }
        if (!(S.lambda0 >= 0.0f && S.lambda0 <= 1.0f)) {
            SetError("pixel (%u, %u): lambda0 %g outside [0, 1]", x, y, (double)S.lambda0);
            return -1;
        }
        const uint32_t e[4] = {S.active01 & 0xFFFFu, S.active01 >> 16, S.active23 & 0xFFFFu, S.active23 >> 16};
        for (uint32_t v : e)
            if (v != 0xFFFFu && v >= shapes) {
                SetError("pixel (%u, %u): active shape %u >= the scene's %u shapes", x, y, v, shapes);
                return -1;
            }
        float w;
        std::memcpy(&w, &S.packed_velocity, 4);
        ray[i] = make_float4(S.origin[0], S.origin[1], S.origin[2], w);
        thr[i] = make_float4(S.throughput[0], S.throughput[1], S.throughput[2], S.throughput[3]);
        prob[i] = make_float4(S.probability[0], S.probability[1], S.probability[2], S.probability[3]);
        lam[i] = S.lambda0;
        act[i] = make_uint2(S.active01, S.active23);
    }
    PT_HIP(hipSetDevice(d->id));
    if (r->grey) PT_HIP(pt_launch_grey_convert(r->slots, Frame(r), r->prob1.ptr, false, d->stream));
    r->grey = false;
    r->grey_blocked = false;
    r->slots.prob1 = nullptr;
    PT_WAIT(d);
    const size_t n = (size_t)T * 256;
    PT_HIP(hipMemcpy(r->thr.ptr + s0, thr.data(), n * 16, hipMemcpyHostToDevice));
    PT_HIP(hipMemcpy(r->prob.ptr + s0, prob.data(), n * 16, hipMemcpyHostToDevice));
    PT_HIP(hipMemcpy(r->lam.ptr + s0, lam.data(), n * 4, hipMemcpyHostToDevice));
    PT_HIP(hipMemcpy(r->act.ptr + s0, act.data(), n * 8, hipMemcpyHostToDevice));
    dbuf<float4> stage;
    PT_HIP(stage.upload(ray.data(), n));
    if (int e = SyncRayOrder(r)) return e;
    if (r->slots.len_order && r->len_cam_stale) {
        PT_HIP(hipMemsetAsync(r->len_cam.ptr, 0, ((size_t)r->slots.tile_count + 1) * sizeof(uint16_t), d->stream));
        r->len_cam_stale = false;
    }
    PT_HIP(pt_launch_restore_rays(r->slots, Frame(r), stage.ptr, s0 / 256, T, d->stream));
    PT_WAIT(d);
    return 0;
}

int ptWriteBasicRendererState(pt_device* d, pt_basic_renderer* r, const pt_pixel_state* in)
{
    return ptWriteBasicRendererStreamState(d, r, 0, in);
}

static float4* StreamAccumulator(pt_basic_renderer* r, uint32_t stream)
{
    return r->streams == 1 ? r->buffer->accum : r->accx.ptr + (size_t)stream * r->buffer->width * r->buffer->height;
}

int ptReadBasicRendererStreamAccumulator(pt_device* d, pt_basic_renderer* r, uint32_t stream, float* rgba)
{
    if (!d || !r || !r->buffer || !rgba) { SetError("null argument"); return -1; }
    if (stream >= r->streams) { SetError("stream %u >= the renderer's %u streams", stream, r->streams); return -1; }
    return ReadBack(d, rgba, StreamAccumulator(r, stream), (size_t)r->buffer->width * r->buffer->height * 16);
}

int ptWriteBasicRendererStreamAccumulator(pt_device* d, pt_basic_renderer* r, uint32_t stream, const float* rgba)
{
    if (!d || !r || !r->buffer || !rgba) { SetError("null argument"); return -1; }
    if (stream >= r->streams) { SetError("stream %u >= the renderer's %u streams", stream, r->streams); return -1; }
    return WriteThrough(d, StreamAccumulator(r, stream), rgba, (size_t)r->buffer->width * r->buffer->height * 16);
}

static_assert(PT_SHADE_DIFFUSE == PT_MATS_DIFFUSE && PT_SHADE_METAL == PT_MATS_METAL &&
              PT_SHADE_TRANSLUCENT == PT_MATS_TRANSLUCENT && PT_SHADE_SCATTER == PT_MATS_SCATTER &&
              PT_SHADE_OPENPBR == PT_MATS_OPENPBR && PT_SHADE_PRIMS == PT_MATS_PRIMS && PT_SHADE_SKY == PT_MATS_SKY &&
              PT_SHADE_TEXWRAP == PT_MATS_TEXWRAP, "pt_api.h shade mask bits");

int ptGetBasicRendererShadeInfo(pt_basic_renderer* r, pt_shade_info* info)
{
    if (!r || !info) { SetError("null argument"); return -1; }
    if (!r->scene || !r->scene->valid) { SetError("renderer: scene has no valid packs (call ptUpdateScene)"); return -1; }
    info->scene_mask = ShadeMats(r);
    info->kernel_mask = pt_shade_mats(ShadeMats(r));
    info->completion_queue = ShadeCompact(r) ? 1u : 0u;
    info->grey_records = r->grey ? 1u : 0u;
    info->ray_order = LengthOrder(r) ? PT_RAY_ORDER_LENGTH : PT_RAY_ORDER_OCTANT;
    info->length_trained = r->scene->len_trained ? 1u : 0u;
    return 0;
}

}
```

path-tracer_amd/csrc/hip/rt_rounds.hip:

```cpp
#include "runtime.hpp"

using namespace ptrt;

constexpr uint32_t AUTO_BATCH = 16;

#ifndef PT_TILE_ORDER_PERIOD
#define PT_TILE_ORDER_PERIOD 16
#endif
constexpr uint32_t TILE_ORDER_PERIOD = PT_TILE_ORDER_PERIOD;

uint32_t ptrt::ShadeMats(const pt_basic_renderer* r)
{
    uint32_t m = r->scene->mats;
    if (!(m & PT_MATS_OPENPBR)) return m;
    if (!r->openpbr) return m & ~(uint32_t)PT_MATS_OPENPBR;
    return m | PT_MATS_SCATTER;
}

bool ptrt::GreyForm(const pt_basic_renderer* r) { return pt_grey_mats(pt_shade_mats(ShadeMats(r))); }

static int SyncRecordForm(pt_device* d, pt_basic_renderer* r)
{
    const bool want = GreyForm(r);
    if (want != r->grey && r->slots.n) {
        const ptd::dframe F = Frame(r);
        if (!want) {
            PT_HIP(pt_launch_grey_convert(r->slots, F, r->prob1.ptr, false, d->stream));
            r->grey = false;
        } else if (!r->grey_blocked) {
            PT_HIP(hipMemsetAsync(r->grey_count.ptr, 0, sizeof(uint32_t), d->stream));
            PT_HIP(pt_launch_grey_check(r->slots, F, r->grey_count.ptr, d->stream));
            PT_WAIT(d);
            uint32_t bad = 0;
            PT_HIP(hipMemcpy(&bad, r->grey_count.ptr, sizeof(bad), hipMemcpyDeviceToHost));
            if (bad == 0) {
                PT_HIP(pt_launch_grey_convert(r->slots, F, r->prob1.ptr, true, d->stream));
                r->grey = true;
            } else {
                r->grey_blocked = true;
            }
        }
    }
    r->slots.prob1 = r->grey ? r->prob1.ptr : nullptr;
    return 0;
}


bool ptrt::ShadeCompact(const pt_basic_renderer* r)
{
    const uint32_t m = ShadeMats(r);
    return (m & (PT_MATS_METAL | PT_MATS_TRANSLUCENT | PT_MATS_OPENPBR)) != 0 ||
           r->scene->d.g.SkyboxSamplingProbability > 0.0f || r->params.PathTerminationProbability > 0.0f;
}

static bool Masked(const pt_basic_renderer* r) { return !r->mask.empty(); }

static uint64_t RoundSlots(const pt_basic_renderer* r) { return Masked(r) ? r->active_slots : r->valid_slots; }

static ptd::dslots ActiveSlots(const pt_basic_renderer* r)
{
    ptd::dslots L = r->slots;
    if (Masked(r)) L.tile_count = r->active_tiles;
    return L;
}

static bool RoundFused(const pt_basic_renderer* r, const ptd::dslots& g)
{
    const int mode = r->fused;
    if (mode == 0 || g.spill || g.tile_count == 0) return false;
    uint32_t cap = pt_round_capacity(ShadeMats(r), r->scene->d.stack16 != 0, r->dev->cu_count);
    if (cap == 0) return false;
    return mode == 2 || g.tile_count <= cap;
}

static size_t ClassListStride(uint32_t tiles, uint32_t K)
{
    return (size_t)ptd::PT_OUTCOME_CLASSES * CQ_SUB * pt_classq_sub_capacity((tiles + K - 1) / K);
}

static int ClassListBuffers(pt_device* d, pt_basic_renderer* r, uint32_t K)
{
    const size_t nc = (size_t)ptd::PT_OUTCOME_CLASSES * CQ_SUB;
    const uint32_t T = r->slots.tile_count;
    if (!r->cq_counts.ptr) {
        if (r->cq_counts.alloc((PT_MAX_SPLIT + 1) * 2 * nc) != hipSuccess ||
            hipMemsetAsync(r->cq_counts.ptr, 0, (PT_MAX_SPLIT + 1) * 2 * nc * sizeof(uint32_t), d->stream) != hipSuccess) {
            SetError("class list allocation failed");
            return -1;
        }
    }
    const size_t need = std::max(ClassListStride(T, 1), K * ClassListStride(T, K));
    if (need > r->cq_list.count) {
        if (r->cq_list.ptr) PT_WAIT(d);
        if (r->cq_list.alloc(need) != hipSuccess) {
            SetError("class list allocation failed");
            return -1;
        }
    }
    return 0;
}

constexpr uint32_t SPLIT_MIN_TILES = 2048;
constexpr uint32_t SPLIT_AUTO_GROUPS = 3;

uint32_t ptrt::SplitGroups(const pt_basic_renderer* r)
{
    const ptd::dslots L = ActiveSlots(r);
    if (!L.order || r->slots.tile_count < 2 || r->split == 1) return 1;
    if (r->split >= 2) return std::min(r->split, r->slots.tile_count);
    return (!RoundFused(r, L) && L.tile_count >= SPLIT_MIN_TILES) ? SPLIT_AUTO_GROUPS : 1u;
}

static bool ClassLists(const pt_basic_renderer* r)
{
    return r->class_lists != 1 && !Masked(r) && r->scene->d.mat_classes != 0 &&
           pt_class_lists_supported(ShadeMats(r));
}

bool ptrt::ClassListRounds(const pt_basic_renderer* r) { return SplitGroups(r) > 1 && ClassLists(r); }

constexpr uint64_t LEN_TRAIN_FIRST = 16, LEN_TRAIN_PERIOD = 64;

static bool LengthSupported(const pt_basic_renderer* r)
{
    return pt_length_train_supported(r->scene->d, Spills(r)) && pt_length_order_supported(ShadeMats(r));
}

bool ptrt::LengthOrder(const pt_basic_renderer* r)
{
    return r->ray_order != PT_RAY_ORDER_OCTANT && LengthSupported(r);
}

int ptrt::SyncRayOrder(pt_basic_renderer* r)
{
    ptd::dslots& L = r->slots;
    if (!LengthOrder(r)) {
        if (L.len_order) r->len_cam_stale = true;
        L.len_order = 0;
        L.len_cls = nullptr;
        L.len_cam = nullptr;
        L.len_sum = L.len_cnt = nullptr;
        return 0;
    }
    pt_scene* s = r->scene;
    if (!r->len_cam.ptr) {
        PT_HIP(r->len_cam.alloc((size_t)L.tile_count + 1));
        r->len_cam_stale = true;
    }
    if (!L.len_order) r->len_cam_stale = true;
    L.len_order = 1;
    L.len_cls = s->len_trained ? s->len_cls.ptr : nullptr;
    L.len_cam = r->len_cam.ptr;
    L.len_sum = s->len_sum.ptr;
    L.len_cnt = s->len_cnt.ptr;
    L.len_bounds = s->len_bounds;
    return 0;
}

static bool LengthTrainRound(pt_basic_renderer* r)
{
    if (!r->slots.len_order) return false;
    pt_scene* s = r->scene;
    const uint64_t t = s->len_rounds++;
    const bool train = t < LEN_TRAIN_FIRST || t % LEN_TRAIN_PERIOD == 0;
    if (train) s->len_pending = true;
    return train;
}

static int LengthFinalize(pt_device* d, pt_basic_renderer* r)
{
    pt_scene* s = r->scene;
    if (!r->slots.len_order || !s->len_pending) return 0;
    PT_HIP(pt_launch_length_classes(s->len_sum.ptr, s->len_cnt.ptr, s->len_cls.ptr, d->stream));
    s->len_pending = false;
    s->len_trained = true;
    return SyncRayOrder(r);
}

static int WriteOrder(pt_device* d, pt_basic_renderer* r, uint32_t K)
{
    if (!r->slots.order) return 0;
    const uint32_t T = r->slots.tile_count;
    std::vector<uint32_t> order(T);
    uint32_t i = 0;
    for (uint32_t g = 0; g < PT_MAX_SPLIT; g++) r->group_active[g] = 0;
    for (uint32_t g = 0; g < K; g++) {
        const uint32_t n = pt_tile_group_count(T, K, g);
        for (uint32_t pass = 0; pass < (Masked(r) ? 2u : 1u); pass++) {
            for (uint32_t j = 0; j < n; j++) {
                const uint32_t t = pt_tile_group_tile(T, K, g, j);
                if (Masked(r) && (r->mask[t] != 0) != (pass == 0)) continue;
                order[i++] = t;
                if (Masked(r) && pass == 0) r->group_active[g]++;
            }
        }
    }
    PT_WAIT(d);
    PT_HIP(hipMemcpy(r->order.ptr, order.data(), (size_t)T * 4, hipMemcpyHostToDevice));
    r->order_groups = K;
    return 0;
}

static int EnsureOrderGroups(pt_device* d, pt_basic_renderer* r, uint32_t K)
{
    if (r->order_groups == K || !r->slots.order) return 0;
    return WriteOrder(d, r, K);
}

static int EnsureGroupStreams(pt_device* d, uint32_t K)
{
    if (!d->fork_event) PT_HIP(hipEventCreateWithFlags(&d->fork_event, hipEventDisableTiming));
    for (uint32_t g = 0; g + 1 < K; g++) {
        if (!d->group_stream[g]) PT_HIP(hipStreamCreateWithFlags(&d->group_stream[g], hipStreamNonBlocking));
        if (!d->join_event[g]) PT_HIP(hipEventCreateWithFlags(&d->join_event[g], hipEventDisableTiming));
    }
    return 0;
}


struct class_lists { uint32_t *counts, *next_counts, *list; };

static int NextClassLists(pt_device* d, pt_basic_renderer* r, uint32_t K, uint32_t g, class_lists& q)
{
    if (int e = ClassListBuffers(d, r, K)) return e;
    const size_t nc = (size_t)ptd::PT_OUTCOME_CLASSES * CQ_SUB;
    const uint32_t region = K > 1 ? g : PT_MAX_SPLIT;
    uint32_t* cnt = r->cq_counts.ptr + region * 2 * nc;
    uint32_t& parity = r->cq_parity[region];
    q.counts = cnt + nc * parity;
    q.next_counts = cnt + nc * (parity ^ 1u);
    q.list = r->cq_list.ptr + (K > 1 ? g * ClassListStride(r->slots.tile_count, K) : 0);
    parity ^= 1u;
    return 0;
}

static int ResetGroupLists(pt_device* d, pt_basic_renderer* r, uint32_t K)
{
    if (int e = ClassListBuffers(d, r, K)) return e;
    PT_HIP(hipMemsetAsync(r->cq_counts.ptr, 0, PT_MAX_SPLIT * 2 * ptd::PT_OUTCOME_CLASSES * CQ_SUB * sizeof(uint32_t),
                          d->stream));
    for (uint32_t g = 0; g < PT_MAX_SPLIT; g++) r->cq_parity[g] = 0;
    return 0;
}

struct round_setup {
    bool idle;
    ptd::dframe F;
    uint32_t mats;
    bool compact;
    bool fused;
    bool lists;
};

static int BeginRounds(pt_device* d, pt_basic_renderer* r, uint32_t K, uint64_t seeds, round_setup& S)
{
    S = {};
    PT_HIP(hipSetDevice(d->id));
    S.idle = Masked(r) && r->active_tiles == 0;
    if (S.idle) {
        r->params.FrameIndex += (uint32_t)seeds;
        return 0;
    }
    if (int e = EnsureSpill(r)) return e;
    if (int e = SyncRecordForm(d, r)) return e;
    if (K > 1 || Masked(r))
        if (int e = EnsureOrderGroups(d, r, K)) return e;
    if (K > 1)
        if (int e = EnsureGroupStreams(d, K)) return e;
    S.F = Frame(r);
    S.mats = ShadeMats(r);
    S.compact = ShadeCompact(r);
    S.fused = K == 1 && RoundFused(r, ActiveSlots(r));
    S.lists = !S.fused && ClassLists(r) && (K > 1 || SplitGroups(r) > 1);
    if (int e = SyncRayOrder(r)) return e;
    if (r->slots.len_order && r->len_cam_stale && !S.fused) {
        PT_HIP(hipMemsetAsync(r->len_cam.ptr, 0, ((size_t)r->slots.tile_count + 1) * sizeof(uint16_t), d->stream));
        r->len_cam_stale = false;
    }
    return 0;
}

struct round_tick { bool sampled, sort; };

static round_tick NextRound(const pt_device* d, const pt_basic_renderer* r)
{
    return {d->profiling && d->run_tick % d->profile_period == 0,
            r->slots.order && r->order_tick % TILE_ORDER_PERIOD == 0 && !Masked(r)};
}

static void RoundsDone(pt_device* d, pt_basic_renderer* r, uint32_t n, uint32_t seeds, uint64_t slots)
{
    r->params.FrameIndex += seeds;
    r->rays += slots * n;
    d->run_tick += n;
    if (r->slots.order) r->order_tick += n;
}

static int Resort(pt_basic_renderer* r, uint32_t g0, uint32_t g1, hipStream_t st)
{
    for (uint32_t g = g0; g < g1; g++) PT_HIP(pt_launch_tile_order(r->slots, st, r->order_groups, g));
    return 0;
}

static int IssueRound(pt_device* d, pt_basic_renderer* r, const round_setup& S, const ptd::dslots& L,
                      const ptd::dparams& P, hipStream_t st, bool timed, uint32_t K = 1, uint32_t g = 0,
                      bool train = false)
{
    event_pair ep{};
    if (S.fused) {
        if (int e = BeginTimed(d, PT_KERNEL_ROUND, ep, timed)) return e;
        PT_HIP(pt_launch_round(r->scene->d, L, S.F, P, S.mats, st));
        r->len_cam_stale = true;
        return EndTimed(d, ep);
    }
    if (int e = BeginTimed(d, PT_KERNEL_EXTEND, ep, timed)) return e;
    PT_HIP(pt_launch_extend(r->scene->d, L, S.F, L.spill, st, train));
    if (int e = EndTimed(d, ep)) return e;
    if (int e = BeginTimed(d, PT_KERNEL_SHADE, ep, timed)) return e;
    if (S.lists) {
        class_lists q;
        if (int e = NextClassLists(d, r, K, g, q)) return e;
        PT_HIP(pt_launch_shade_classq(r->scene->d, L, S.F, P, S.mats, S.compact, q.counts, q.next_counts, q.list, st,
                                      r->slots.tile_count, K, g));
    } else {
        PT_HIP(pt_launch_shade(r->scene->d, L, S.F, P, S.mats, S.compact, st));
    }
    return EndTimed(d, ep);
}

static int IssueBatch(pt_device* d, pt_basic_renderer* r, const round_setup& S, const ptd::dslots& L,
                      uint32_t first_seed, uint32_t seed_step, uint32_t n)
{
    ptd::dparams P = Params(r, first_seed);
    P.rounds = n;
    P.seed_step = seed_step;
    const uint64_t t = d->run_tick % d->profile_period;
    const bool sampled = d->profiling && (t == 0 || t + n > d->profile_period);
    d->run_tick += n;
    event_pair ep{};
    if (int e = BeginTimed(d, PT_KERNEL_ROUNDS, ep, sampled, n)) return e;
    PT_HIP(pt_launch_rounds(r->scene->d, L, S.F, P, S.mats, d->stream));
    r->len_cam_stale = true;
    if (int e = EndTimed(d, ep)) return e;
    if (!Masked(r))
        if (int e = Resort(r, 0, r->order_groups, d->stream)) return e;
    r->rays += RoundSlots(r) * n;
    return 0;
}

static int SplitRounds(pt_device* d, pt_basic_renderer* r, const round_setup& S, uint64_t k, uint32_t K)
{
    ptd::dslots G[PT_MAX_SPLIT];
    hipStream_t St[PT_MAX_SPLIT];
    for (uint32_t g = 0; g < K; g++) {
        G[g] = r->slots;
        G[g].order = r->slots.order + pt_tile_group_start(r->slots.tile_count, K, g);
        G[g].tile_count = Masked(r) ? r->group_active[g] : pt_tile_group_count(r->slots.tile_count, K, g);
        St[g] = g ? d->group_stream[g - 1] : d->stream;
    }
    if (S.lists)
        if (int e = ResetGroupLists(d, r, K)) return e;
    PT_HIP(hipEventRecord(d->fork_event, d->stream));
    for (uint32_t g = 1; g < K; g++) PT_HIP(hipStreamWaitEvent(St[g], d->fork_event, 0));
    auto rounds = [&]() -> int {
        for (uint64_t i = 0; i < k; i++) {
            const ptd::dparams P = Params(r, r->params.FrameIndex + 1);
            const round_tick tick = NextRound(d, r);
            const bool train = LengthTrainRound(r);
            for (uint32_t g = 0; g < K; g++) {
                if (G[g].tile_count == 0) continue;
                if (int e = IssueRound(d, r, S, G[g], P, St[g], g == 0 && tick.sampled, K, g, train)) return e;
                if (tick.sort)
                    if (int e = Resort(r, g, g + 1, St[g])) return e;
            }
            RoundsDone(d, r, 1, 1, RoundSlots(r));
        }
        return 0;
    };
    const int rc = rounds();
    for (uint32_t g = 1; g < K; g++) {
        PT_HIP(hipEventRecord(d->join_event[g - 1], St[g]));
        PT_HIP(hipStreamWaitEvent(d->stream, d->join_event[g - 1], 0));
    }
    return rc;
}

static int RunRounds(pt_device* d, pt_basic_renderer* r, uint64_t k)
{
    if (!r || CheckReady(r) != 0) return -1;
    uint32_t B = r->round_batch;
    if (B == 0) B = RoundFused(r, ActiveSlots(r)) && r->fused == 1 ? AUTO_BATCH : 1u;
    const bool batches = B > 1 && !Spills(r);
    const uint32_t K = batches || k < 2 ? 1u : SplitGroups(r);
    round_setup S;
    if (int e = BeginRounds(d, r, K, k, S)) return e;
    if (S.idle) return 0;
    if (batches) {
        const ptd::dslots L = ActiveSlots(r);
        while (k > 0) {
            const uint32_t n = (uint32_t)std::min<uint64_t>(k, B);
            if (int e = IssueBatch(d, r, S, L, r->params.FrameIndex + 1, 1, n)) return e;
            r->params.FrameIndex += n;
            k -= n;
        }
        return 0;
    }
    if (K > 1) {
        while (k > 0) {
            uint64_t n = k;
            if (r->slots.len_order && r->scene->len_rounds < LEN_TRAIN_FIRST)
                n = std::min<uint64_t>(k, LEN_TRAIN_FIRST - r->scene->len_rounds);
            if (int e = SplitRounds(d, r, S, n, K)) return e;
            if (int e = LengthFinalize(d, r)) return e;
            k -= n;
        }
        return 0;
    }
    for (uint64_t i = 0; i < k; i++)
        if (int e = ptRunBasicRenderer(d, r, 1)) return e;
    return 0;
}

static int RunGuardedRounds(pt_device* d, pt_basic_renderer* r, uint32_t n, uint64_t target, uint32_t* ran)
{
    round_setup S;
    if (int e = BeginRounds(d, r, 1, 0, S)) return e;
    if (!r->guard.ptr) PT_HIP(r->guard.alloc(2));
    PT_HIP(hipMemsetAsync(r->guard.ptr, 0, 2 * sizeof(uint32_t), d->stream));
    ptd::dslots L = r->slots;
    L.stop = r->guard.ptr;
    const uint32_t base = r->params.FrameIndex;
    uint32_t& parity = r->cq_parity[PT_MAX_SPLIT];
    const uint32_t parity0 = parity;
    for (uint32_t i = 0; i < n; i++) {
        PT_HIP(pt_launch_guard(r->done.ptr, r->slots.n / 64 + 1, target, r->guard.ptr, d->stream));
        if (int e = IssueRound(d, r, S, L, Params(r, base + i + 1), d->stream, false)) return e;
    }
    uint32_t flags[2] = {0, 0};
    PT_WAIT(d);
    PT_HIP(hipMemcpy(flags, r->guard.ptr, sizeof(flags), hipMemcpyDeviceToHost));
    *ran = flags[1];
    if (S.lists) parity = parity0 ^ (*ran & 1u);
    RoundsDone(d, r, *ran, *ran, r->valid_slots);
    return 0;
}

constexpr double GUARD_PREDICTED = 8.0;

extern "C" {

int ptRunBasicRenderer(pt_device* d, pt_basic_renderer* r, uint32_t rounds)
{
    if (!d) { SetError("null device"); return -1; }
    if (CheckReady(r) != 0) return -1;
    round_setup S;
    if (int e = BeginRounds(d, r, 1, 1, S)) return e;
    if (S.idle) return 0;
    r->params.FrameIndex += 1;
    const uint32_t seed = r->params.FrameIndex;
    const ptd::dslots L = ActiveSlots(r);
    const uint32_t B = r->round_batch ? r->round_batch : (S.fused && r->fused == 1 ? AUTO_BATCH : 1u);
    if (S.fused && rounds >= 2 && B >= 2 && pt_rounds_available(L)) {
        for (uint32_t left = rounds; left > 0;) {
            const uint32_t n = std::min(left, B);
            if (int e = IssueBatch(d, r, S, L, seed, 0, n)) return e;
            left -= n;
        }
        return 0;
    }
    const ptd::dparams P = Params(r, seed);
    for (uint32_t i = 0; i < rounds; i++) {
        const round_tick tick = NextRound(d, r);
        const bool train = !S.fused && LengthTrainRound(r);
        if (int e = IssueRound(d, r, S, L, P, d->stream, tick.sampled, 1, 0, train)) return e;
        if (tick.sort)
            if (int e = Resort(r, 0, r->order_groups, d->stream)) return e;
        RoundsDone(d, r, 1, 0, RoundSlots(r));
    }
    return LengthFinalize(d, r);
}

int ptRunBasicRendererRounds(pt_device* d, pt_basic_renderer* r, uint32_t count)
{
    if (!d) { SetError("null device"); return -1; }
    if (CheckReady(r) != 0) return -1;
    return RunRounds(d, r, count);
}

int ptSetBasicRendererActiveTiles(pt_device* d, pt_basic_renderer* r, const uint8_t* mask, uint32_t tiles)
{
    if (!d || !r) { SetError("ptSetBasicRendererActiveTiles: null argument"); return -1; }
    if (r->dev != d) { SetError("ptSetBasicRendererActiveTiles: renderer of another device"); return -1; }
    if (r->nranks != 1 || r->streams != 1) {
        SetError("ptSetBasicRendererActiveTiles: partitioned and multi-stream renderers take no active tile set");
        return -1;
    }
    if (!mask && tiles != 0) { SetError("ptSetBasicRendererActiveTiles: null mask with %u tiles", tiles); return -1; }
    if (mask && tiles != r->slots.tile_count) {
        SetError("ptSetBasicRendererActiveTiles: %u tiles given, the renderer has %u", tiles, r->slots.tile_count);
        return -1;
    }
    if (!mask && !Masked(r)) return 0;
    PT_HIP(hipSetDevice(d->id));
    std::vector<uint8_t> previous;
    const uint32_t previous_tiles = r->active_tiles;
    const uint64_t previous_slots = r->active_slots;
    previous.swap(r->mask);
    r->active_tiles = 0;
    r->active_slots = 0;
    if (mask && tiles) {
        r->mask.assign(mask, mask + tiles);
        const uint32_t w = r->buffer->width, h = r->buffer->height;
        for (uint32_t t = 0; t < tiles; t++) {
            if (!mask[t]) continue;
            const uint32_t ty = t / r->tiles_x, tx = t - ty * r->tiles_x;
            r->active_tiles++;
            r->active_slots += (uint64_t)std::min(16u, w - tx * 16u) * std::min(16u, h - ty * 16u);
        }
    }
    if (int e = WriteOrder(d, r, r->order_groups)) {
        r->mask.swap(previous);
        r->active_tiles = previous_tiles;
        r->active_slots = previous_slots;
        return e;
    }
    return 0;
}

int ptGetBasicRendererActiveTiles(const pt_basic_renderer* r, uint32_t* active, uint32_t* tiles)
{
    if (!r) { SetError("ptGetBasicRendererActiveTiles: null renderer"); return -1; }
    if (active) *active = Masked(r) ? r->active_tiles : r->slots.tile_count;
    if (tiles) *tiles = r->slots.tile_count;
    return 0;
}

int ptRenderFrame(pt_device* d, pt_basic_renderer* r, uint64_t target_samples, uint32_t max_rounds,
                  uint32_t* rounds_out, uint64_t* samples_out)
{
    if (!d || !r) { SetError("null argument"); return -1; }
    if (max_rounds < 2) { SetError("ptRenderFrame: max_rounds must be >= 2"); return -1; }
    if (Masked(r)) { SetError("ptRenderFrame: an active tile set is in place (ptSetBasicRendererActiveTiles)"); return -1; }
    if (int e = ptResetBasicRenderer(d, r)) return e;
    if (int e = ptRunBasicRenderer(d, r, 2)) return e;
    uint32_t rounds = 2;
    uint64_t samples = 0, prev = 0;
    uint32_t last_batch = 0;
    const uint64_t px = std::max<uint64_t>(r->valid_slots, 1);
    if (target_samples > 2 * px) {
        const uint64_t k = std::min<uint64_t>((target_samples - 2 * px + px - 1) / px, max_rounds - rounds);
        if (k >= 1) {
            if (int e = RunRounds(d, r, k)) return e;
            rounds += (uint32_t)k;
            last_batch = rounds;
        }
    }
    for (;;) {
        if (int e = ptGetStats(d, r, nullptr, &samples)) return e;
        if (samples >= target_samples || rounds >= max_rounds) break;
        const uint64_t remaining = target_samples - samples;
        if (last_batch > 0 && samples > prev) {
            const double rate = (double)(samples - prev) / last_batch;
            const double predicted = (double)remaining / rate;
            if (predicted <= GUARD_PREDICTED) {
                const uint64_t ks = std::min<uint64_t>((remaining + px - 1) / px, max_rounds - rounds);
                if (int e = RunRounds(d, r, ks)) return e;
                rounds += (uint32_t)ks;
                const double left = std::max(predicted - (double)ks, 0.0);
                const uint32_t n = (uint32_t)std::min<uint64_t>((uint64_t)(1.25 * left) + 2, max_rounds - rounds);
                uint32_t ran = 0;
                if (n >= 1)
                    if (int e = RunGuardedRounds(d, r, n, target_samples, &ran)) return e;
                rounds += ran;
                prev = samples;
                last_batch = (uint32_t)ks + ran;
                continue;
            }
        }
        const uint64_t k = std::min<uint64_t>((remaining + px - 1) / px, max_rounds - rounds);
        if (int e = RunRounds(d, r, k)) return e;
        rounds += (uint32_t)k;
        prev = samples;
        last_batch = (uint32_t)k;
    }
    if (rounds_out) *rounds_out = rounds;
    if (samples_out) *samples_out = samples;
    return 0;
}

}
```

path-tracer_amd/csrc/hip/runtime.hpp:

```cpp
#pragma once
#include "pt_device.hpp"
#include "kernels.hpp"
#include "../../../include/pt_api.h"
#include "../../../include/pt_denoise.h"
#include "../../../include/pt_reproject.h"
#include "../../../include/pt_rectify.h"
#include "../../../include/pt_despike.h"
#include "../../../include/pt_guides.h"
#include "../../../include/pt_stats.h"
#include "../../../include/pt_numerics.h"

#include <rccl/rccl.h>

#include <algorithm>
#include <cstring>
#include <vector>

namespace ptrt __attribute__((visibility("hidden"))) {

void SetError(const char* fmt, ...);

#define PT_HIP(call)                                                                         \
    do {                                                                                     \
        hipError_t e_ = (call);                                                              \
        if (e_ != hipSuccess) {                                                              \
            ptrt::SetError("%s failed: %s (%s:%d)", #call, hipGetErrorString(e_), __FILE__, __LINE__); \
            return (int)e_;                                                                  \
        }                                                                                    \
    } while (0)

template <class T>
struct dbuf {
    T* ptr = nullptr;
    size_t count = 0;
    dbuf() = default;
    dbuf(const dbuf&) = delete;
    dbuf& operator=(const dbuf&) = delete;
    ~dbuf() { release(); }
    void release() { if (ptr) (void)hipFree(ptr); ptr = nullptr; count = 0; }
    hipError_t upload(const T* src, size_t n)
    {
        if (!ptr || n > count) {
            release();
            hipError_t e = hipMalloc(&ptr, std::max<size_t>(n, 1) * sizeof(T));
            if (e != hipSuccess) { ptr = nullptr; return e; }
            count = n;
        }
        if (n == 0) return hipMemset(ptr, 0, sizeof(T));
        return hipMemcpy(ptr, src, n * sizeof(T), hipMemcpyHostToDevice);
    }
    hipError_t alloc(size_t n)
    {
        if (n <= count && ptr) return hipSuccess;
        release();
        hipError_t e = hipMalloc(&ptr, std::max<size_t>(n, 1) * sizeof(T));
        if (e != hipSuccess) { ptr = nullptr; return e; }
        count = n;
        return hipSuccess;
    }
    hipError_t alloc_zero(size_t n)
    {
        hipError_t e = alloc(n);
        return e != hipSuccess || n == 0 ? e : hipMemset(ptr, 0, n * sizeof(T));
    }
};

struct event_pair { hipEvent_t a, b; int kernel; uint32_t rounds; hipStream_t stream; };

}

struct pt_device {
    int id = 0;
    hipStream_t stream = nullptr;
    uint32_t cu_count = 256;
    bool profiling = false;
    uint32_t profile_period = 1;
    uint64_t run_tick = 0;
    std::vector<ptrt::event_pair> pending;
    std::vector<ptrt::event_pair> free_events;
    std::vector<pt_comm*> comms;
    bool comm_failed = false;
    uint64_t launches[PT_KERNEL_COUNT] = {};
    uint64_t rounds[PT_KERNEL_COUNT] = {};
    double total_ms[PT_KERNEL_COUNT] = {};
    hipStream_t group_stream[PT_MAX_SPLIT - 1] = {};
    hipEvent_t fork_event = nullptr;
    hipEvent_t join_event[PT_MAX_SPLIT - 1] = {};
    ptrt::dbuf<pt_frame_statistics> stats;
    uint32_t stats_variant = PT_STATS_VARIANT_AUTO;
    ptrt::dbuf<pt_tile_statistics> tile_stats;
    ptrt::dbuf<pt_shape_motion> motion;
    pt_shape_motion* motion_host = nullptr;
    size_t motion_host_count = 0;
    hipEvent_t motion_copied = nullptr;
};

struct pt_scene {
    pt_device* dev = nullptr;
    ptd::dscene d{};
    ptrt::dbuf<pt_packed_texture> textures;
    ptrt::dbuf<uint32_t> material;
    ptrt::dbuf<pt_packed_shape> shapes;
    ptrt::dbuf<pt_packed_shape_node> shape_nodes;
    ptrt::dbuf<pt_packed_mesh_face> faces;
    ptrt::dbuf<pt_packed_mesh_vertex> vertices;
    ptrt::dbuf<float4> vertex_attr;
    ptrt::dbuf<float> vertex_v;
    ptrt::dbuf<pt_packed_mesh_node> mesh_nodes;
    ptrt::dbuf<pt_packed_camera> cameras;
    ptrt::dbuf<float> atlas;
    bool atlas_tiled = false;
    uint32_t camera_count = 0;
    uint32_t texture_count = 0;
    uint32_t stack_needed = 0;
    uint32_t mats = PT_MATS_ALL | PT_MATS_SCENE;
    uint32_t stack_format = PT_STACK_FORMAT_AUTO;
    uint32_t hit_record = PT_HIT_RECORD_AUTO;
    uint32_t cached_pairs = 0;
    bool blas_packable = false;
    uint32_t blas16_bits = 0;
    uint32_t extend_form = PT_EXTEND_FORM_AUTO;
    bool one_mesh = false;
    ptrt::dbuf<uint32_t> len_sum, len_cnt;
    ptrt::dbuf<uint8_t> len_cls;
    pt_raykey_bounds len_bounds{};
    bool len_trained = false;
    bool len_pending = false;
    uint64_t len_rounds = 0;
    bool valid = false;
};

struct pt_sample_buffer {
    pt_device* dev = nullptr;
    uint32_t width = 0, height = 0;
    float4* accum = nullptr;
    ptrt::dbuf<float4> display;
    ptrt::dbuf<uint32_t> display8;
    bool resolved = false;
    uint32_t rank = 0, nranks = 1;
};

struct pt_preview {
    pt_device* dev = nullptr;
    pt_scene* scene = nullptr;
    uint32_t width = 0, height = 0;
    ptrt::dbuf<float4> image;
    ptrt::dbuf<pt_preview_aov> aov;
    ptrt::dbuf<uint32_t> spill;
    ptrt::dbuf<float> observe;
    ptrt::dbuf<uint32_t> query;
    bool rendered = false;
};

struct pt_denoise_guides {
    pt_device* dev = nullptr;
    uint32_t width = 0, height = 0;
    ptrt::dbuf<float4> records;
    ptrt::dbuf<float4> scratch;
    ptrt::dbuf<uint32_t> spill;
    ptrt::dbuf<float> observe;
    uint32_t variant = PT_DENOISE_VARIANT_AUTO;
};

struct pt_basic_renderer {
    pt_basic_renderer_params params{};
    pt_device* dev = nullptr;
    pt_scene* scene = nullptr;
    pt_sample_buffer* buffer = nullptr;
    uint32_t rank = 0, nranks = 1;
    uint32_t tiles_x = 0;
    ptd::dslots slots{};
    ptrt::dbuf<float4> ray, hit, thr, prob;
    ptrt::dbuf<float> prob1;
    bool grey = false;
    bool grey_blocked = false;
    ptrt::dbuf<uint32_t> grey_count;
    ptrt::dbuf<uint32_t> cq_counts, cq_list;
    uint32_t cq_parity[PT_MAX_SPLIT + 1] = {};
    uint32_t class_lists = 0;
    ptrt::dbuf<float> lam;
    ptrt::dbuf<float2> uv;
    ptrt::dbuf<uint2> act;
    ptrt::dbuf<uint16_t> pos;
    ptrt::dbuf<uint8_t> slotof;
    ptrt::dbuf<uint64_t> outcome;
    ptrt::dbuf<uint32_t> tilecost, order;
    uint64_t order_tick = 0;
    ptrt::dbuf<uint32_t> done;
    int fused = 1;
    int openpbr = 0;
    uint32_t round_batch = 0;
    uint32_t split = 0;
    ptrt::dbuf<uint32_t> guard;
    uint32_t order_groups = 1;
    std::vector<uint8_t> mask;
    uint32_t active_tiles = 0;
    uint64_t active_slots = 0;
    uint32_t group_active[PT_MAX_SPLIT] = {};
    uint64_t pixels = 0;
    uint32_t streams = 1;
    uint32_t stream_tiles = 0;
    uint64_t valid_slots = 0;
    ptrt::dbuf<float4> accx;
    uint64_t rays = 0;
    ptrt::dbuf<uint32_t> spill;
    uint32_t ray_order = PT_RAY_ORDER_AUTO;
    ptrt::dbuf<uint16_t> len_cam;
    bool len_cam_stale = true;
};

struct pt_comm {
    pt_device* dev = nullptr;
    ncclComm_t comm = nullptr;
    int nranks = 1, rank = 0;
    double timeout_s = 600.0;
    bool aborted = false;
    int* flag = nullptr;
    int* host_flag = nullptr;
};

namespace ptrt __attribute__((visibility("hidden"))) {


void AbortComms(pt_device* dev);

int DeviceWait(pt_device* dev);

#define PT_WAIT(dev)                                    \
    do {                                                \
        if (int w_ = ptrt::DeviceWait(dev)) return w_;  \
    } while (0)

int BeginTimed(pt_device* dev, int kernel, event_pair& ep, bool sampled = true, uint32_t rounds = 1);
int EndTimed(pt_device* dev, event_pair& ep);

#define PT_TIMED(dev, KERNEL, launch)                               \
    do {                                                            \
        ptrt::event_pair ep_{};                                     \
        if (int b_ = ptrt::BeginTimed(dev, KERNEL, ep_)) return b_; \
        PT_HIP(launch);                                             \
        if (int d_ = ptrt::EndTimed(dev, ep_)) return d_;           \
    } while (0)

int CollectTimes(pt_device* dev);

inline int CopyAndWait(pt_device* d, void* dst, const void* src, size_t bytes, hipMemcpyKind kind)
{
    PT_HIP(hipSetDevice(d->id));
    PT_HIP(hipMemcpyAsync(dst, src, bytes, kind, d->stream));
    PT_WAIT(d);
    return 0;
}
inline int ReadBack(pt_device* d, void* host, const void* device, size_t bytes)
{
    return CopyAndWait(d, host, device, bytes, hipMemcpyDeviceToHost);
}
inline int WriteThrough(pt_device* d, void* device, const void* host, size_t bytes)
{
    return CopyAndWait(d, device, host, bytes, hipMemcpyHostToDevice);
}


inline ptd::dframe Frame(pt_basic_renderer* r)
{
    ptd::dframe F;
    F.accum = r->buffer->accum;
    F.width = r->buffer->width;
    F.height = r->buffer->height;
    F.rank = r->rank;
    F.nranks = r->nranks;
    F.tiles_x = r->tiles_x;
    F.tiles_x_magic = r->tiles_x > 1 ? (uint32_t)(((1ull << 32) + r->tiles_x - 1) / r->tiles_x) : 0u;
    F.streams = r->streams;
    F.stream_tiles = r->stream_tiles;
    F.stream_magic = r->streams > 1 ? (uint32_t)(((1ull << 32) + r->stream_tiles - 1) / r->stream_tiles) : 0u;
    F.accx = r->accx.ptr;
    return F;
}

inline ptd::dparams Params(pt_basic_renderer* r, uint32_t seed)
{
    ptd::dparams P;
    P.camera_index = r->params.CameraIndex;
    P.render_flags = r->params.RenderFlags;
    P.termination_probability = r->params.PathTerminationProbability;
    P.seed = seed;
    return P;
}

inline bool Spills(const pt_basic_renderer* r) { return r->scene->stack_needed > pt_extend_stack_cap(); }

inline int EnsureSpill(pt_basic_renderer* r)
{
    if (!Spills(r)) { r->slots.spill = nullptr; return 0; }
    size_t rows = r->scene->stack_needed - pt_extend_stack_cap();
    PT_HIP(r->spill.alloc(rows * (size_t)r->slots.n));
    r->slots.spill = r->spill.ptr;
    return 0;
}

inline int CheckReady(pt_basic_renderer* r)
{
    if (!r || !r->scene || !r->buffer) { SetError("renderer: null"); return -1; }
    if (!r->scene->valid) { SetError("renderer: scene has no valid packs (call ptUpdateScene)"); return -1; }
    if (r->params.CameraIndex >= r->scene->camera_count) {
        SetError("renderer: CameraIndex %u >= camera count %u", r->params.CameraIndex, r->scene->camera_count);
        return -1;
    }
    return 0;
}


uint32_t ShadeMats(const pt_basic_renderer* r);
bool GreyForm(const pt_basic_renderer* r);
bool ShadeCompact(const pt_basic_renderer* r);
uint32_t SplitGroups(const pt_basic_renderer* r);
bool ClassListRounds(const pt_basic_renderer* r);
bool LengthOrder(const pt_basic_renderer* r);
int SyncRayOrder(pt_basic_renderer* r);

}
```

path-tracer_amd/csrc/hip/variants.hpp:

```cpp
#pragma once

#include "kernels.hpp"

#include <type_traits>
#include <utility>

#ifndef PT_EXTEND_MINW
#define PT_EXTEND_MINW 5
#endif
#ifndef PT_EXTEND_CAP
#define PT_EXTEND_CAP 20
#endif

namespace ptv {

inline uint32_t Blocks(uint32_t n) { return (n + 255) / 256; }

template <class F, bool... Bs>
void SelectFlags(F&& f, std::integer_sequence<bool, Bs...>)
{
    f(std::bool_constant<Bs>{}...);
}
template <class F, bool... Bs, class... Rest>
void SelectFlags(F&& f, std::integer_sequence<bool, Bs...>, bool flag, Rest... rest)
{
    if (flag) SelectFlags(f, std::integer_sequence<bool, Bs..., true>{}, rest...);
    else SelectFlags(f, std::integer_sequence<bool, Bs..., false>{}, rest...);
}
template <class F, class... Flags>
void SelectFlags(F&& f, bool flag, Flags... rest)
{
    SelectFlags(f, std::integer_sequence<bool>{}, flag, rest...);
}


constexpr uint32_t MATS_D = PT_MATS_DIFFUSE;
constexpr uint32_t MATS_DS = PT_MATS_DIFFUSE | PT_MATS_SCENE;
constexpr uint32_t MATS_DM = PT_MATS_DIFFUSE | PT_MATS_METAL | PT_MATS_SCENE;
constexpr uint32_t MATS_A = PT_MATS_ALL | PT_MATS_SCENE;
constexpr uint32_t MATS_AO = PT_MATS_ALL | PT_MATS_OPENPBR | PT_MATS_SCENE;

template <class F>
auto SelectShadeMats(uint32_t scene_mats, F&& f)
{
    switch (pt_shade_mats(scene_mats)) {
    case MATS_D: return f(std::integral_constant<uint32_t, MATS_D>{});
    case MATS_DS: return f(std::integral_constant<uint32_t, MATS_DS>{});
    case MATS_DM: return f(std::integral_constant<uint32_t, MATS_DM>{});
    case MATS_A: return f(std::integral_constant<uint32_t, MATS_A>{});
    default: return f(std::integral_constant<uint32_t, MATS_AO>{});
    }
}

constexpr bool HasLengthShade(uint32_t shade_mats) { return shade_mats == MATS_D || shade_mats == MATS_DS; }
constexpr bool HasClassListShade(uint32_t shade_mats) { return shade_mats == MATS_DM || shade_mats == MATS_A; }


template <class E>
struct stack_entry { using type = E; };

template <class F>
auto SelectStackEntry(bool stack16, F&& f)
{
    return stack16 ? f(stack_entry<uint16_t>{}) : f(stack_entry<uint32_t>{});
}

template <class E>
constexpr bool HasNodeCache(bool spill) { return sizeof(E) == 2 && !spill; }

constexpr bool HasTrain(bool renderer_source, bool mesh, bool spill) { return renderer_source && mesh && !spill; }

}
```

path-tracer_amd/renderer.py:

```python
from __future__ import annotations

import ctypes as C

import numpy as np

from . import _native as N
from ._core import U32, U64, Handle, extend_stats, hip, hip_get, tile_grid
from .device import Device, DeviceScene
from .frame import SampleBuffer

REFINE_MIN_ROUNDS = 128


def refine_tiles(renderer_a: "BasicRenderer", renderer_b: "BasicRenderer", threshold: float, q: float = 0.95,
                 min_rounds: int = REFINE_MIN_ROUNDS, rounds_per_step: int = 8, max_rounds: int = 1024,
                 min_count: "float | None" = None):
    if rounds_per_step < 1 or min_rounds < 0 or max_rounds < 1:
        raise ValueError("rounds_per_step >= 1, min_rounds >= 0 and max_rounds >= 1 are required")
    if not 0.0 < q <= 1.0:
        raise ValueError("q must lie in (0, 1]")
    sa, sb = renderer_a.sample_buffer, renderer_b.sample_buffer
    if (sa.width, sa.height) != (sb.width, sb.height):
        raise ValueError("the two renderers' sample buffers differ in size")
    active = np.ones(tile_grid(sa.width, sa.height), dtype=bool)
    rounds = np.zeros(active.shape, dtype=np.int64)
    done, stats = 0, None
    try:
        while True:
            step = min(rounds_per_step, max_rounds - done)
            if done < min_rounds:
                step = min(step, min_rounds - done)
            for r in (renderer_a, renderer_b):
                r.set_active_tiles(None if active.all() else active)
                r.run_rounds(step)
            done += step
            rounds[active] += step
            stats = sa.tile_statistics(sb, threshold)
            need = (stats["pair"] == 0) | (stats["over"] > (1.0 - q) * stats["pair"])
            if min_count is not None:
                need |= (stats["filled"] > 0) & (stats["min_count"] < np.float32(min_count))
            if done < min_rounds:
                need[:] = True
            active &= need
            if not active.any() or done >= max_rounds:
                return rounds, stats
    finally:
        for r in (renderer_a, renderer_b):
            r.set_active_tiles(None)


def render_until_noise(renderer_a: "BasicRenderer", renderer_b: "BasicRenderer", threshold: float, q: float = 0.95,
                       check_every: int = 8, min_pair_fraction: float = 0.99, max_rounds: int = 1024):
    if check_every < 1 or max_rounds < 2:
        raise ValueError("check_every >= 1 and max_rounds >= 2 are required")
    sa, sb = renderer_a.sample_buffer, renderer_b.sample_buffer
    renderer_b.FrameIndex = renderer_a.FrameIndex + (1 << 24)
    for r in (renderer_a, renderer_b):
        r.reset()
    for r in (renderer_a, renderer_b):
        r.run(2)
    rounds, stats = 2, None
    while True:
        if rounds % check_every == 0 or rounds >= max_rounds:
            stats = sa.statistics(sb)
            if rounds >= max_rounds or (stats.noise_pixels >= min_pair_fraction * stats.pixels and
                                        stats.noise(q) <= threshold):
                return rounds, stats
        for r in (renderer_a, renderer_b):
            r.run(1)
        rounds += 1


class BasicRenderer(Handle):

    _destroy = "ptDestroyBasicRenderer"
    _FIELDS = ("FrameIndex", "CameraIndex", "RenderFlags", "PathLengthLimit", "PathTerminationProbability")

    def __init__(self, device: Device, scene: DeviceScene, sample_buffer: SampleBuffer, rank: int = 0, nranks: int = 1,
                 streams: int = 1):
        self.device, self.scene, self.sample_buffer = device, scene, sample_buffer
        self.rank, self.nranks, self.streams = rank, nranks, streams
        self._create("ptCreateBasicRendererStreams", device.handle, scene.handle, sample_buffer.handle, rank, nranks,
                     streams)
        self._params = N.hip_lib().ptBasicRendererParams(self._h)

    def __getattr__(self, name):
        if name in BasicRenderer._FIELDS:
            return getattr(self._params.contents, name)
        raise AttributeError(name)

    def __setattr__(self, name, value):
        if name in BasicRenderer._FIELDS:
            setattr(self._params.contents, name, value)
        else:
            object.__setattr__(self, name, value)

    @property
    def slot_count(self) -> int:
        return int(N.hip_lib().ptBasicRendererSlotCount(self._h))

    def merge_streams(self):
        hip("ptMergeBasicRendererStreams", self.device.handle, self._h)

    def set_fused_rounds(self, mode: int):
        hip("ptSetBasicRendererFusedRounds", self._h, int(mode))

    def set_round_batch(self, rounds: int):
        hip("ptSetBasicRendererRoundBatch", self._h, int(rounds))

    def set_split(self, groups: int):
        hip("ptSetBasicRendererSplit", self._h, int(groups))

    def split(self) -> dict:
        return dict(zip(("groups", "timed_tiles", "tiles"),
                        hip_get("ptGetBasicRendererSplit", self._h, types=(U32, U32, U32))))

    def set_class_lists(self, mode: int):
        hip("ptSetBasicRendererClassLists", self._h, int(mode))

    def class_lists(self) -> bool:
        return bool(hip_get("ptGetBasicRendererClassLists", self._h))

    def set_ray_order(self, order: int):
        hip("ptSetBasicRendererRayOrder", self._h, int(order))

    def ray_order(self) -> dict:
        return dict(zip(("order", "used"), hip_get("ptGetBasicRendererRayOrder", self._h, types=(U32, U32))))

    def ray_positions(self) -> np.ndarray:
        out = np.zeros(self.slot_count, dtype=np.uint16)
        hip("ptReadBasicRendererRayPositions", self.device.handle, self._h, out.ctypes.data)
        return out

    def set_active_tiles(self, mask: "np.ndarray | None"):
        if mask is None:
            hip("ptSetBasicRendererActiveTiles", self.device.handle, self._h, None, 0)
            return
        m = np.asarray(mask)
        grid = tile_grid(self.sample_buffer.width, self.sample_buffer.height)
        if m.shape != grid:
            raise ValueError(f"mask of shape {m.shape}, the frame has {grid} tiles")
        m = np.ascontiguousarray(m != 0, dtype=np.uint8)
        hip("ptSetBasicRendererActiveTiles", self.device.handle, self._h, m.ctypes.data, m.size)

    def active_tiles(self) -> dict:
        return dict(zip(("active", "tiles"), hip_get("ptGetBasicRendererActiveTiles", self._h, types=(U32, U32))))

    def run_rounds(self, count: int):
        hip("ptRunBasicRendererRounds", self.device.handle, self._h, int(count))

    def set_openpbr(self, enable: bool):
        hip("ptSetBasicRendererOpenPBR", self._h, int(bool(enable)))

    def reset(self):
        hip("ptResetBasicRenderer", self.device.handle, self._h)

    def run(self, rounds: int = 1):
        hip("ptRunBasicRenderer", self.device.handle, self._h, int(rounds))

    def render_frame(self, target_samples: int, max_rounds: int = 1 << 30):
        return hip_get("ptRenderFrame", self.device.handle, self._h, int(target_samples), int(max_rounds),
                       types=(U32, U64))

    def stats(self):
        return hip_get("ptGetStats", self.device.handle, self._h, types=(U64, U64))

    def extend_stats(self) -> dict:
        out = (C.c_uint64 * 14)()
        hip("ptExtendStats", self.device.handle, self._h, out)
        d = extend_stats(out)
        for k in ("lane_steps", "internal_nodes", "blas_leaves", "faces", "pops", "tlas_leaves"):
            d[k + "_per_ray"] = d[k] / max(d["rays"], 1)
        return d

    def extend_step_counts(self) -> np.ndarray:
        out = np.zeros(self.slot_count, dtype=np.uint32)
        hip("ptExtendStepCounts", self.device.handle, self._h, out.ctypes.data)
        return out

    def read_state(self, stream: int = 0) -> np.ndarray:
        sb = self.sample_buffer
        out = np.zeros(sb.width * sb.height, dtype=N.PIXEL_STATE_DTYPE)
        hip("ptReadBasicRendererStreamState", self.device.handle, self._h, int(stream), out.ctypes.data)
        return out.reshape(sb.height, sb.width)

    def write_state(self, state: np.ndarray, stream: int = 0):
        sb = self.sample_buffer
        a = np.ascontiguousarray(state, dtype=N.PIXEL_STATE_DTYPE).reshape(-1)
        if a.size != sb.width * sb.height:
            raise ValueError(f"state has {a.size} pixels, the sample buffer {sb.width * sb.height}")
        hip("ptWriteBasicRendererStreamState", self.device.handle, self._h, int(stream), a.ctypes.data)

    def read_accumulator(self, stream: int = 0) -> np.ndarray:
        sb = self.sample_buffer
        out = np.zeros((sb.height, sb.width, 4), dtype=np.float32)
        hip("ptReadBasicRendererStreamAccumulator", self.device.handle, self._h, int(stream), N.fptr(out))
        return out

    def write_accumulator(self, rgba: np.ndarray, stream: int = 0):
        sb = self.sample_buffer
        a = np.ascontiguousarray(rgba, dtype=np.float32).reshape(sb.height, sb.width, 4)
        hip("ptWriteBasicRendererStreamAccumulator", self.device.handle, self._h, int(stream), N.fptr(a))

    def shade_info(self) -> dict:
        info = N.pt_shade_info()
        hip("ptGetBasicRendererShadeInfo", self._h, C.byref(info))
        return {"scene_mask": int(info.scene_mask), "kernel_mask": int(info.kernel_mask),
                "completion_queue": bool(info.completion_queue), "grey_records": bool(info.grey_records),
                "ray_order": int(info.ray_order), "length_trained": bool(info.length_trained)}
```

Baseline: 6524 Mrays/s.

## Add RUN block map scheduling extend blocks as per-wave units sorted longest-first

Adds a block-map mode in which each extend block gathers four 64-lane wavefronts drawn from a 4-tile run, each wave picked independently. A unit list is sorted longest-first by per-wave cost, so the waves packed into one block have similar trace times. The goal is to cut intra-block imbalance, where a 256-thread block stays resident until its slowest wave finishes. The cost is an extra sort kernel block, a unit indirection buffer and more template variants. The mode is limited to mesh-only, non-spill, length-ordered, unfused rounds.

```diff
diff --git a/include/pt_api.h b/include/pt_api.h
--- a/include/pt_api.h
+++ b/include/pt_api.h
@@ -166,6 +166,17 @@
 int                ptSetBasicRendererSplit(pt_basic_renderer* renderer, uint32_t groups);
 int                ptGetBasicRendererSplit(const pt_basic_renderer* renderer, uint32_t* groups, uint32_t* timed_tiles,
                                            uint32_t* tiles);
+enum { PT_BLOCK_MAP_AUTO = 0, PT_BLOCK_MAP_TILE = 1, PT_BLOCK_MAP_RUN = 2 };
+int                ptSetBasicRendererBlockMap(pt_basic_renderer* renderer, uint32_t map);
+int                ptGetBasicRendererBlockMap(const pt_basic_renderer* renderer, uint32_t* map, uint32_t* used);
+uint32_t           ptBlockMapGroupTileCount(uint32_t tiles, uint32_t groups, uint32_t group, uint32_t granule);
+uint32_t           ptBlockMapGroupTile(uint32_t tiles, uint32_t groups, uint32_t group, uint32_t granule, uint32_t i);
+uint32_t           ptBlockMapGroupTileStart(uint32_t tiles, uint32_t groups, uint32_t group, uint32_t granule);
+uint32_t           ptBlockMapGroupUnitCount(uint32_t tiles, uint32_t groups, uint32_t group, uint32_t granule);
+uint32_t           ptBlockMapGroupUnit(uint32_t tiles, uint32_t groups, uint32_t group, uint32_t granule, uint32_t i);
+uint32_t           ptBlockMapGroupUnitStart(uint32_t tiles, uint32_t groups, uint32_t group, uint32_t granule);
+uint32_t           ptBlockMapUnitTile(uint32_t unit, uint32_t wave, uint32_t granule);
+uint32_t           ptBlockMapUnitQuarter(uint32_t unit, uint32_t wave, uint32_t granule);
 int                ptSetBasicRendererActiveTiles(pt_device* device, pt_basic_renderer* renderer, const uint8_t* mask,
                                                  uint32_t tiles);
 int                ptGetBasicRendererActiveTiles(const pt_basic_renderer* renderer, uint32_t* active, uint32_t* tiles);
@@ -201,6 +212,7 @@
     uint32_t grey_records;
     uint32_t ray_order;
     uint32_t length_trained;
+    uint32_t block_map;
 } pt_shade_info;
 int                ptGetBasicRendererShadeInfo(pt_basic_renderer* renderer, pt_shade_info* info);
 
diff --git a/include/pt_blockmap.h b/include/pt_blockmap.h
--- /dev/null
+++ b/include/pt_blockmap.h
@@ -0,0 +1,66 @@
+#ifndef PT_BLOCKMAP_H
+#define PT_BLOCKMAP_H
+
+#include "pt_fp.h"
+
+#define PT_BLOCK_MAP_TILE_GRANULE 1u
+#define PT_BLOCK_MAP_RUN_GRANULE  4u
+
+PT_HD uint32_t pt_granule_count(uint32_t tiles, uint32_t granule) { return (tiles + granule - 1u) / granule; }
+
+PT_HD uint32_t pt_group_granules(uint32_t tiles, uint32_t groups, uint32_t group, uint32_t granule)
+{
+    const uint32_t n = pt_granule_count(tiles, granule);
+    return group < n ? (n - group + groups - 1u) / groups : 0u;
+}
+
+PT_HD uint32_t pt_group_tile_count(uint32_t tiles, uint32_t groups, uint32_t group, uint32_t granule)
+{
+    const uint32_t own = pt_group_granules(tiles, groups, group, granule);
+    if (own == 0u) return 0u;
+    const uint32_t last = group + (own - 1u) * groups;
+    const uint32_t end = last * granule + granule;
+    return own * granule - (end > tiles ? end - tiles : 0u);
+}
+
+PT_HD uint32_t pt_group_tile(uint32_t groups, uint32_t group, uint32_t i, uint32_t granule)
+{
+    return (group + (i / granule) * groups) * granule + i % granule;
+}
+
+PT_HD uint32_t pt_group_tile_start(uint32_t tiles, uint32_t groups, uint32_t group, uint32_t granule)
+{
+    uint32_t s = 0;
+    for (uint32_t h = 0; h < group; h++) s += pt_group_tile_count(tiles, groups, h, granule);
+    return s;
+}
+
+PT_HD uint32_t pt_unit_count(uint32_t tiles, uint32_t granule) { return pt_granule_count(tiles, granule) * granule; }
+
+PT_HD uint32_t pt_group_unit_count(uint32_t tiles, uint32_t groups, uint32_t group, uint32_t granule)
+{
+    return pt_group_granules(tiles, groups, group, granule) * granule;
+}
+
+PT_HD uint32_t pt_group_unit(uint32_t groups, uint32_t group, uint32_t i, uint32_t granule)
+{
+    return (group + (i / granule) * groups) * granule + i % granule;
+}
+
+PT_HD uint32_t pt_group_unit_start(uint32_t tiles, uint32_t groups, uint32_t group, uint32_t granule)
+{
+    uint32_t s = 0;
+    for (uint32_t h = 0; h < group; h++) s += pt_group_unit_count(tiles, groups, h, granule);
+    return s;
+}
+
+PT_HD uint32_t pt_unit_tile(uint32_t unit, uint32_t wave, uint32_t granule)
+{
+    return granule == PT_BLOCK_MAP_RUN_GRANULE ? (unit & ~3u) + wave : unit;
+}
+PT_HD uint32_t pt_unit_quarter(uint32_t unit, uint32_t wave, uint32_t granule)
+{
+    return granule == PT_BLOCK_MAP_RUN_GRANULE ? (unit & 3u) : wave;
+}
+
+#endif
diff --git a/path-tracer_amd/_native.py b/path-tracer_amd/_native.py
--- a/path-tracer_amd/_native.py
+++ b/path-tracer_amd/_native.py
@@ -34,10 +34,12 @@
 
 class pt_shade_info(C.Structure):
     _fields_ = [("scene_mask", C.c_uint32), ("kernel_mask", C.c_uint32), ("completion_queue", C.c_uint32),
-                ("grey_records", C.c_uint32), ("ray_order", C.c_uint32), ("length_trained", C.c_uint32)]
+                ("grey_records", C.c_uint32), ("ray_order", C.c_uint32), ("length_trained", C.c_uint32),
+                ("block_map", C.c_uint32)]
 
 
 RAY_ORDER_AUTO, RAY_ORDER_OCTANT, RAY_ORDER_LENGTH = 0, 1, 2
+BLOCK_MAP_AUTO, BLOCK_MAP_TILE, BLOCK_MAP_RUN = 0, 1, 2
 RAYKEY_COUNT = 32768
 
 
@@ -395,6 +397,16 @@
     "ptGetBasicRendererSplit": (_i32, [_vp, _u32ptr, _u32ptr, _u32ptr]),
     "ptSetBasicRendererRayOrder": (_i32, [_vp, _u32]),
     "ptGetBasicRendererRayOrder": (_i32, [_vp, _u32ptr, _u32ptr]),
+    "ptSetBasicRendererBlockMap": (_i32, [_vp, _u32]),
+    "ptGetBasicRendererBlockMap": (_i32, [_vp, _u32ptr, _u32ptr]),
+    "ptBlockMapGroupTileCount": (_u32, [_u32, _u32, _u32, _u32]),
+    "ptBlockMapGroupTile": (_u32, [_u32, _u32, _u32, _u32, _u32]),
+    "ptBlockMapGroupTileStart": (_u32, [_u32, _u32, _u32, _u32]),
+    "ptBlockMapGroupUnitCount": (_u32, [_u32, _u32, _u32, _u32]),
+    "ptBlockMapGroupUnit": (_u32, [_u32, _u32, _u32, _u32, _u32]),
+    "ptBlockMapGroupUnitStart": (_u32, [_u32, _u32, _u32, _u32]),
+    "ptBlockMapUnitTile": (_u32, [_u32, _u32, _u32]),
+    "ptBlockMapUnitQuarter": (_u32, [_u32, _u32, _u32]),
     "ptReadSceneLengthTable": (_i32, [_vp, _vp, _vp, _u32ptr, C.POINTER(C.c_uint64)]),
     "ptReadBasicRendererRayPositions": (_i32, [_vp, _vp, _vp]),
     "ptSetBasicRendererOpenPBR": (_i32, [_vp, _i32]),
diff --git a/path-tracer_amd/csrc/hip/extend.hip b/path-tracer_amd/csrc/hip/extend.hip
--- a/path-tracer_amd/csrc/hip/extend.hip
+++ b/path-tracer_amd/csrc/hip/extend.hip
@@ -4,7 +4,7 @@
 namespace ptd {
 
 template <class Src, bool SPILL, int MINW, int CAP, class E = uint32_t, bool NC = false, bool MESH = false,
-          bool TRAIN = false>
+          bool TRAIN = false, bool RUN = false>
 __global__ __launch_bounds__(256, (MESH && !NC) ? 8 : MINW) void extend_kernel(dscene S, Src src, uint32_t n,
                                                                                uint32_t* spill, uint32_t spill_stride)
 {
@@ -22,7 +22,7 @@
             timed = true;
         }
     }
-    ExtendTile<Src, SPILL, CAP, E, MESH, TRAIN>(S, src, n, spill, spill_stride, smem, tile, timed, ncache, ncn);
+    ExtendTile<Src, SPILL, CAP, E, MESH, TRAIN, RUN>(S, src, n, spill, spill_stride, smem, tile, timed, ncache, ncn);
 }
 
 constexpr uint32_t LEN_MEAN_BINS = 4096;
@@ -135,39 +135,47 @@
 
 template <class Src>
 static hipError_t LaunchExtend(const ptd::dscene& S, const Src& src, uint32_t n, uint32_t blocks, uint32_t* spill,
-                               bool train, hipStream_t st)
+                               bool train, bool run, hipStream_t st)
 {
     constexpr bool renderer = ptd::kRendererSource<Src>;
     if (train && !ptv::HasTrain(renderer, S.single_mesh != 0, spill != nullptr)) return hipErrorNotSupported;
+    if (run && !ptv::HasRunMap(renderer, S.single_mesh != 0, spill != nullptr)) return hipErrorNotSupported;
     if (n == 0 || blocks == 0) return hipSuccess;
     ptv::SelectStackEntry(S.stack16 != 0, [&](auto entry) {
         using E = typename decltype(entry)::type;
         const bool cache = S.node_cache && ptv::HasNodeCache<E>(spill != nullptr);
         ptv::SelectFlags(
-            [&](auto SPILL, auto NC, auto MESH, auto TRAIN) {
-                if constexpr ((!NC || ptv::HasNodeCache<E>(SPILL)) && (!TRAIN || ptv::HasTrain(renderer, MESH, SPILL)))
-                    hipLaunchKernelGGL((ptd::extend_kernel<Src, SPILL, PT_EXTEND_MINW, PT_EXTEND_CAP, E, NC, MESH, TRAIN>),
-                                       dim3(blocks), dim3(256), 0, st, S, src, n, spill, n);
+            [&](auto SPILL, auto NC, auto MESH, auto TRAIN, auto RUN) {
+                if constexpr ((!NC || ptv::HasNodeCache<E>(SPILL)) && (!TRAIN || ptv::HasTrain(renderer, MESH, SPILL)) &&
+                              (!RUN || ptv::HasRunMap(renderer, MESH, SPILL)))
+                    hipLaunchKernelGGL(
+                        (ptd::extend_kernel<Src, SPILL, PT_EXTEND_MINW, PT_EXTEND_CAP, E, NC, MESH, TRAIN, RUN>),
+                        dim3(blocks), dim3(256), 0, st, S, src, n, spill, n);
             },
-            spill != nullptr, cache, S.single_mesh != 0, train);
+            spill != nullptr, cache, S.single_mesh != 0, train, run);
     });
     return hipGetLastError();
 }
 
 bool pt_length_train_supported(const ptd::dscene& S, bool spill) { return ptv::HasTrain(true, S.single_mesh != 0, spill); }
 
+bool pt_block_map_run_supported(const ptd::dscene& S, bool spill) { return ptv::HasRunMap(true, S.single_mesh != 0, spill); }
+
 hipError_t pt_launch_extend(const ptd::dscene& S, const ptd::dslots& L, const ptd::dframe& F, uint32_t* spill,
-                            hipStream_t st, bool train)
+                            hipStream_t st, bool train, const uint32_t* units, uint32_t unit_count)
 {
     if (train && (!L.len_sum || !L.len_cnt || !L.len_cam)) return hipErrorNotSupported;
-    return LaunchExtend(S, ptd::ray_source_slots{L, F}, L.n, L.tile_count, spill, train, st);
+    if (!units) return LaunchExtend(S, ptd::ray_source_slots{L, F}, L.n, L.tile_count, spill, train, false, st);
+    ptd::dslots U = L;
+    U.order = const_cast<uint32_t*>(units);
+    return LaunchExtend(S, ptd::ray_source_slots{U, F}, L.n, unit_count, spill, train, true, st);
 }
 
 hipError_t pt_launch_trace_rays(const ptd::dscene& S, uint32_t n, const float* origins, const uint32_t* vel,
                                 const float* dur, float4* hit, float2* hc, float4* rec, float2* uv, uint32_t* spill,
                                 hipStream_t st)
 {
-    hipError_t e = LaunchExtend(S, ptd::ray_source_arrays{origins, vel, dur, hit, hc}, n, Blocks(n), spill, false, st);
+    hipError_t e = LaunchExtend(S, ptd::ray_source_arrays{origins, vel, dur, hit, hc}, n, Blocks(n), spill, false, false, st);
     if (e != hipSuccess) return e;
     return pt_launch_finalize(S, n, hit, hc, rec, uv, st);
 }
diff --git a/path-tracer_amd/csrc/hip/extend.hpp b/path-tracer_amd/csrc/hip/extend.hpp
--- a/path-tracer_amd/csrc/hip/extend.hpp
+++ b/path-tracer_amd/csrc/hip/extend.hpp
@@ -117,12 +117,20 @@
     src.outcome(slot, cls, S.mat_classes != 0);
 }
 
-template <class Src, bool SPILL, int CAP, class E, bool MESH = false, bool TRAIN = false>
+template <class Src, bool SPILL, int CAP, class E, bool MESH = false, bool TRAIN = false, bool RUN = false>
 PT_DEV void ExtendTile(const dscene& S, const Src& src, uint32_t n, uint32_t* spill, uint32_t spill_stride, E* smem,
                        uint32_t tile, bool timed, const float4* nc = nullptr, uint32_t ncn = 0)
 {
+    static_assert(!RUN || (MESH && !SPILL && kRendererSource<Src>), "the RUN block map rides the renderer's mesh-only loop");
     uint64_t t0 = timed ? __builtin_amdgcn_s_memtime() : 0;
     uint32_t slot = tile * 256 + threadIdx.x;
+    uint32_t first = 0;
+    if constexpr (RUN) {
+        const uint32_t wave = (uint32_t)__builtin_amdgcn_readfirstlane((int)(threadIdx.x >> 6));
+        first = pt_unit_tile(tile, wave, PT_BLOCK_MAP_RUN_GRANULE) * 256 +
+                pt_unit_quarter(tile, wave, PT_BLOCK_MAP_RUN_GRANULE) * 64;
+        slot = first + (threadIdx.x & 63u);
+    }
     if (slot >= n) return;
     tstack<SPILL, CAP, E> st;
     st.lds = &smem[threadIdx.x];
@@ -133,7 +141,7 @@
     ExtendRay<SPILL, CAP, E, MESH, TRAIN>(S, src, st, slot);
     if constexpr (kRendererSource<Src>) {
         if (timed && (threadIdx.x & 63u) == 0)
-            src.L.tilecost[tile * 4 + (threadIdx.x >> 6)] = (uint32_t)(__builtin_amdgcn_s_memtime() - t0);
+            src.L.tilecost[RUN ? first >> 6 : tile * 4 + (threadIdx.x >> 6)] = (uint32_t)(__builtin_amdgcn_s_memtime() - t0);
     }
 }
 
diff --git a/path-tracer_amd/csrc/hip/kernels.hip b/path-tracer_amd/csrc/hip/kernels.hip
--- a/path-tracer_amd/csrc/hip/kernels.hip
+++ b/path-tracer_amd/csrc/hip/kernels.hip
@@ -4,24 +4,22 @@
 
 namespace ptd {
 
-__global__ __launch_bounds__(1024) void tile_order_kernel(const uint32_t* cost, uint32_t* order, uint32_t tiles,
-                                                          uint32_t groups, uint32_t group, uint32_t start)
-{
-    const uint32_t nt = pt_tile_group_count(tiles, groups, group);
-    __shared__ uint32_t count[512];
+template <class Item, class Time>
+PT_DEV void SortLongestFirst(uint32_t n, uint32_t* out, uint32_t* count, uint32_t* wsum, Item item, Time time)
+{
+    __syncthreads();
     for (uint32_t i = threadIdx.x; i < 512; i += 1024) count[i] = 0;
     __syncthreads();
-    auto key = [&](uint32_t t) -> uint32_t {
-        uint32_t c = max(max(cost[4 * t], cost[4 * t + 1]), max(cost[4 * t + 2], cost[4 * t + 3]));
+    auto key = [&](uint32_t x) -> uint32_t {
+        uint32_t c = time(x);
         if (c < 16) return 511u;
         uint32_t e = 31u - __clz(c);
         uint32_t m = (c >> (e - 4)) & 15u;
         uint32_t k = min(e * 16u + m, 511u);
         return 511u - k;
     };
-    for (uint32_t i = threadIdx.x; i < nt; i += 1024) atomicAdd(&count[key(pt_tile_group_tile(tiles, groups, group, i))], 1u);
-    __syncthreads();
-    __shared__ uint32_t wsum[8];
+    for (uint32_t i = threadIdx.x; i < n; i += 1024) atomicAdd(&count[key(item(i))], 1u);
+    __syncthreads();
     uint32_t c = 0, incl = 0;
     if (threadIdx.x < 512) {
         c = count[threadIdx.x];
@@ -39,9 +37,41 @@
         count[threadIdx.x] = before + incl - c;
     }
     __syncthreads();
-    for (uint32_t i = threadIdx.x; i < nt; i += 1024) {
-        const uint32_t t = pt_tile_group_tile(tiles, groups, group, i);
-        order[start + atomicAdd(&count[key(t)], 1u)] = t;
+    for (uint32_t i = threadIdx.x; i < n; i += 1024) {
+        const uint32_t x = item(i);
+        out[atomicAdd(&count[key(x)], 1u)] = x;
+    }
+}
+
+template <bool UNITS>
+__global__ __launch_bounds__(1024) void tile_order_kernel(const uint32_t* cost, uint32_t* order, uint32_t tiles,
+                                                          uint32_t groups, uint32_t group, uint32_t start,
+                                                          uint32_t* units, uint32_t ustart)
+{
+    __shared__ uint32_t count[512];
+    __shared__ uint32_t wsum[8];
+    auto tile_time = [&](uint32_t t) {
+        return max(max(cost[4 * t], cost[4 * t + 1]), max(cost[4 * t + 2], cost[4 * t + 3]));
+    };
+    if constexpr (!UNITS) {
+        SortLongestFirst(pt_tile_group_count(tiles, groups, group), order + start, count, wsum,
+                         [&](uint32_t i) { return pt_tile_group_tile(tiles, groups, group, i); }, tile_time);
+    } else {
+        constexpr uint32_t G = PT_BLOCK_MAP_RUN_GRANULE;
+        if (blockIdx.x == 0)
+            SortLongestFirst(pt_group_tile_count(tiles, groups, group, G), order + start, count, wsum,
+                             [&](uint32_t i) { return pt_group_tile(groups, group, i, G); }, tile_time);
+        else
+            SortLongestFirst(pt_group_unit_count(tiles, groups, group, G), units + ustart, count, wsum,
+                             [&](uint32_t i) { return pt_group_unit(groups, group, i, G); },
+                             [&](uint32_t x) {
+                                 uint32_t c = 0;
+                                 for (uint32_t w = 0; w < 4; w++) {
+                                     const uint32_t t = pt_unit_tile(x, w, G);
+                                     if (t < tiles) c = max(c, cost[4 * t + pt_unit_quarter(x, w, G)]);
+                                 }
+                                 return c;
+                             });
     }
 }
 
@@ -165,11 +195,19 @@
     return hipGetLastError();
 }
 
-hipError_t pt_launch_tile_order(const ptd::dslots& L, hipStream_t st, uint32_t groups, uint32_t group)
+hipError_t pt_launch_tile_order(const ptd::dslots& L, hipStream_t st, uint32_t groups, uint32_t group, uint32_t granule,
+                                uint32_t* units)
 {
     if (!L.order || L.tile_count == 0 || groups == 0 || group >= groups) return hipSuccess;
-    hipLaunchKernelGGL(ptd::tile_order_kernel, dim3(1), dim3(1024), 0, st, L.tilecost, L.order, L.tile_count, groups,
-                       group, pt_tile_group_start(L.tile_count, groups, group));
+    if (granule == PT_BLOCK_MAP_RUN_GRANULE) {
+        if (!units) return hipErrorInvalidValue;
+        hipLaunchKernelGGL(ptd::tile_order_kernel<true>, dim3(2), dim3(1024), 0, st, L.tilecost, L.order, L.tile_count,
+                           groups, group, pt_group_tile_start(L.tile_count, groups, group, granule), units,
+                           pt_group_unit_start(L.tile_count, groups, group, granule));
+    } else {
+        hipLaunchKernelGGL(ptd::tile_order_kernel<false>, dim3(1), dim3(1024), 0, st, L.tilecost, L.order, L.tile_count,
+                           groups, group, pt_tile_group_start(L.tile_count, groups, group), (uint32_t*)nullptr, 0u);
+    }
     return hipGetLastError();
 }
 
diff --git a/path-tracer_amd/csrc/hip/kernels.hpp b/path-tracer_amd/csrc/hip/kernels.hpp
--- a/path-tracer_amd/csrc/hip/kernels.hpp
+++ b/path-tracer_amd/csrc/hip/kernels.hpp
@@ -5,6 +5,7 @@
 #include "../../../include/pt_packed.h"
 #include "../../../include/pt_api.h"
 #include "../../../include/pt_raykey.h"
+#include "../../../include/pt_blockmap.h"
 
 namespace ptd {
 
@@ -65,7 +66,9 @@
 hipError_t pt_launch_raygen(const ptd::dscene& S, const ptd::dslots& L, const ptd::dframe& F, const ptd::dparams& P,
                             hipStream_t st);
 hipError_t pt_launch_extend(const ptd::dscene& S, const ptd::dslots& L, const ptd::dframe& F, uint32_t* spill,
-                            hipStream_t st, bool train = false);
+                            hipStream_t st, bool train = false, const uint32_t* units = nullptr,
+                            uint32_t unit_count = 0);
+bool pt_block_map_run_supported(const ptd::dscene& S, bool spill);
 bool pt_length_train_supported(const ptd::dscene& S, bool spill);
 bool pt_length_order_supported(uint32_t scene_mats);
 hipError_t pt_launch_length_classes(uint32_t* sum, uint32_t* cnt, uint8_t* cls, hipStream_t st);
@@ -150,7 +153,8 @@
     for (uint32_t h = 0; h < group; h++) s += pt_tile_group_count(tiles, groups, h);
     return s;
 }
-hipError_t pt_launch_tile_order(const ptd::dslots& L, hipStream_t st, uint32_t groups = 1, uint32_t group = 0);
+hipError_t pt_launch_tile_order(const ptd::dslots& L, hipStream_t st, uint32_t groups = 1, uint32_t group = 0,
+                                uint32_t granule = 1, uint32_t* units = nullptr);
 hipError_t pt_launch_guard(const uint32_t* done, uint32_t words, uint64_t target, uint32_t* flags, hipStream_t st);
 uint32_t pt_round_capacity(uint32_t scene_mats, bool stack16, uint32_t cu_count);
 hipError_t pt_launch_round(const ptd::dscene& S, const ptd::dslots& L, const ptd::dframe& F, const ptd::dparams& P,
diff --git a/path-tracer_amd/csrc/hip/rt_renderer.hip b/path-tracer_amd/csrc/hip/rt_renderer.hip
--- a/path-tracer_amd/csrc/hip/rt_renderer.hip
+++ b/path-tracer_amd/csrc/hip/rt_renderer.hip
@@ -37,6 +37,7 @@
               r->act.alloc_zero(ns) == hipSuccess && r->pos.alloc(ns) == hipSuccess && r->slotof.alloc(ns) == hipSuccess &&
               r->outcome.alloc_zero(tiles * 4 * ptd::PT_OUTCOME_CLASSES + 1) == hipSuccess &&
               r->tilecost.alloc_zero(tiles * 4 + 1) == hipSuccess && r->order.alloc(tiles + 1) == hipSuccess &&
+              r->units.alloc(pt_unit_count((uint32_t)tiles, PT_BLOCK_MAP_RUN_GRANULE) + 1) == hipSuccess &&
               r->done.alloc_zero(ns / 64 + 1) == hipSuccess &&
               (streams == 1 || r->accx.alloc_zero((size_t)streams * frame_px) == hipSuccess);
     if (ok && ns) {
@@ -173,6 +174,72 @@
     return 0;
 }
 
+int ptSetBasicRendererBlockMap(pt_basic_renderer* r, uint32_t map)
+{
+    if (!r || map > PT_BLOCK_MAP_RUN) {
+        SetError("ptSetBasicRendererBlockMap: bad argument (0 automatic, 1 tile, 2 run)");
+        return -1;
+    }
+    if (map == PT_BLOCK_MAP_RUN && r->scene && r->scene->valid && !RunMapPossible(r)) {
+        SetError("ptSetBasicRendererBlockMap: the RUN block map runs where ray order LENGTH does "
+                 "(a one-mesh diffuse scene without a spilled stack, ray order not OCTANT)");
+        return -1;
+    }
+    r->block_map = map;
+    return 0;
+}
+
+int ptGetBasicRendererBlockMap(const pt_basic_renderer* r, uint32_t* map, uint32_t* used)
+{
+    if (!r) { SetError("ptGetBasicRendererBlockMap: null renderer"); return -1; }
+    if (used && (!r->scene || !r->scene->valid)) {
+        SetError("renderer: scene has no valid packs (call ptUpdateScene)");
+        return -1;
+    }
+    if (map) *map = r->block_map;
+    if (used) *used = RunMap(r) ? PT_BLOCK_MAP_RUN : PT_BLOCK_MAP_TILE;
+    return 0;
+}
+
+static bool MapArgs(uint32_t groups, uint32_t granule)
+{
+    return groups != 0 && (granule == PT_BLOCK_MAP_TILE_GRANULE || granule == PT_BLOCK_MAP_RUN_GRANULE);
+}
+uint32_t ptBlockMapGroupTileCount(uint32_t tiles, uint32_t groups, uint32_t group, uint32_t granule)
+{
+    return MapArgs(groups, granule) ? pt_group_tile_count(tiles, groups, group, granule) : 0u;
+}
+uint32_t ptBlockMapGroupTile(uint32_t tiles, uint32_t groups, uint32_t group, uint32_t granule, uint32_t i)
+{
+    return MapArgs(groups, granule) && i < pt_group_tile_count(tiles, groups, group, granule)
+               ? pt_group_tile(groups, group, i, granule) : 0u;
+}
+uint32_t ptBlockMapGroupTileStart(uint32_t tiles, uint32_t groups, uint32_t group, uint32_t granule)
+{
+    return MapArgs(groups, granule) ? pt_group_tile_start(tiles, groups, std::min(group, groups), granule) : 0u;
+}
+uint32_t ptBlockMapGroupUnitCount(uint32_t tiles, uint32_t groups, uint32_t group, uint32_t granule)
+{
+    return MapArgs(groups, granule) ? pt_group_unit_count(tiles, groups, group, granule) : 0u;
+}
+uint32_t ptBlockMapGroupUnit(uint32_t tiles, uint32_t groups, uint32_t group, uint32_t granule, uint32_t i)
+{
+    return MapArgs(groups, granule) && i < pt_group_unit_count(tiles, groups, group, granule)
+               ? pt_group_unit(groups, group, i, granule) : 0u;
+}
+uint32_t ptBlockMapGroupUnitStart(uint32_t tiles, uint32_t groups, uint32_t group, uint32_t granule)
+{
+    return MapArgs(groups, granule) ? pt_group_unit_start(tiles, groups, std::min(group, groups), granule) : 0u;
+}
+uint32_t ptBlockMapUnitTile(uint32_t unit, uint32_t wave, uint32_t granule)
+{
+    return MapArgs(1, granule) && wave < 4 ? pt_unit_tile(unit, wave, granule) : 0u;
+}
+uint32_t ptBlockMapUnitQuarter(uint32_t unit, uint32_t wave, uint32_t granule)
+{
+    return MapArgs(1, granule) && wave < 4 ? pt_unit_quarter(unit, wave, granule) : 0u;
+}
+
 int ptReadBasicRendererRayPositions(pt_device* d, pt_basic_renderer* r, uint16_t* positions)
 {
     if (!d || !r || !positions) { SetError("ptReadBasicRendererRayPositions: null argument"); return -1; }
@@ -197,7 +264,7 @@
     if (!r) { SetError("ptGetBasicRendererSplit: null renderer"); return -1; }
     const uint32_t K = SplitGroups(r);
     if (groups) *groups = K;
-    if (timed_tiles) *timed_tiles = pt_tile_group_count(r->slots.tile_count, K, 0);
+    if (timed_tiles) *timed_tiles = pt_group_tile_count(r->slots.tile_count, K, 0, K > 1 ? OrderGranule(r) : 1u);
     if (tiles) *tiles = r->slots.tile_count;
     return 0;
 }
@@ -402,7 +469,8 @@
     info->grey_records = r->grey ? 1u : 0u;
     info->ray_order = LengthOrder(r) ? PT_RAY_ORDER_LENGTH : PT_RAY_ORDER_OCTANT;
     info->length_trained = r->scene->len_trained ? 1u : 0u;
-    return 0;
-}
-
-}
+    info->block_map = RunMap(r) ? PT_BLOCK_MAP_RUN : PT_BLOCK_MAP_TILE;
+    return 0;
+}
+
+}
diff --git a/path-tracer_amd/csrc/hip/rt_rounds.hip b/path-tracer_amd/csrc/hip/rt_rounds.hip
--- a/path-tracer_amd/csrc/hip/rt_rounds.hip
+++ b/path-tracer_amd/csrc/hip/rt_rounds.hip
@@ -131,6 +131,22 @@
     return r->ray_order != PT_RAY_ORDER_OCTANT && LengthSupported(r);
 }
 
+bool ptrt::RunMapPossible(const pt_basic_renderer* r)
+{
+    return LengthOrder(r) && pt_block_map_run_supported(r->scene->d, Spills(r));
+}
+
+bool ptrt::RunMap(const pt_basic_renderer* r)
+{
+    return r->block_map != PT_BLOCK_MAP_TILE && RunMapPossible(r) && !Masked(r) && r->round_batch < 2 &&
+           !RoundFused(r, ActiveSlots(r));
+}
+
+uint32_t ptrt::OrderGranule(const pt_basic_renderer* r)
+{
+    return RunMap(r) ? PT_BLOCK_MAP_RUN_GRANULE : PT_BLOCK_MAP_TILE_GRANULE;
+}
+
 int ptrt::SyncRayOrder(pt_basic_renderer* r)
 {
     ptd::dslots& L = r->slots;
@@ -177,34 +193,41 @@
     return SyncRayOrder(r);
 }
 
-static int WriteOrder(pt_device* d, pt_basic_renderer* r, uint32_t K)
+static int WriteOrder(pt_device* d, pt_basic_renderer* r, uint32_t K, uint32_t granule)
 {
     if (!r->slots.order) return 0;
     const uint32_t T = r->slots.tile_count;
-    std::vector<uint32_t> order(T);
+    std::vector<uint32_t> order(T), units;
     uint32_t i = 0;
     for (uint32_t g = 0; g < PT_MAX_SPLIT; g++) r->group_active[g] = 0;
     for (uint32_t g = 0; g < K; g++) {
-        const uint32_t n = pt_tile_group_count(T, K, g);
+        const uint32_t n = pt_group_tile_count(T, K, g, granule);
         for (uint32_t pass = 0; pass < (Masked(r) ? 2u : 1u); pass++) {
             for (uint32_t j = 0; j < n; j++) {
-                const uint32_t t = pt_tile_group_tile(T, K, g, j);
+                const uint32_t t = pt_group_tile(K, g, j, granule);
                 if (Masked(r) && (r->mask[t] != 0) != (pass == 0)) continue;
                 order[i++] = t;
                 if (Masked(r) && pass == 0) r->group_active[g]++;
             }
         }
+        if (granule == PT_BLOCK_MAP_RUN_GRANULE)
+            for (uint32_t j = 0; j < pt_group_unit_count(T, K, g, granule); j++)
+                units.push_back(pt_group_unit(K, g, j, granule));
     }
     PT_WAIT(d);
     PT_HIP(hipMemcpy(r->order.ptr, order.data(), (size_t)T * 4, hipMemcpyHostToDevice));
+    if (!units.empty()) PT_HIP(hipMemcpy(r->units.ptr, units.data(), units.size() * 4, hipMemcpyHostToDevice));
     r->order_groups = K;
-    return 0;
-}
-
-static int EnsureOrderGroups(pt_device* d, pt_basic_renderer* r, uint32_t K)
-{
-    if (r->order_groups == K || !r->slots.order) return 0;
-    return WriteOrder(d, r, K);
+    r->order_granule = granule;
+    return 0;
+}
+
+static int EnsureOrderGroups(pt_device* d, pt_basic_renderer* r, uint32_t K, uint32_t granule)
+{
+    if (!r->slots.order) return 0;
+    const bool grouped = K > 1 || Masked(r);
+    if (r->order_granule == granule && (!grouped || r->order_groups == K)) return 0;
+    return WriteOrder(d, r, grouped ? K : r->order_groups, granule);
 }
 
 static int EnsureGroupStreams(pt_device* d, uint32_t K)
@@ -250,6 +273,7 @@
     bool compact;
     bool fused;
     bool lists;
+    bool run;
 };
 
 static int BeginRounds(pt_device* d, pt_basic_renderer* r, uint32_t K, uint64_t seeds, round_setup& S)
@@ -261,10 +285,14 @@
         r->params.FrameIndex += (uint32_t)seeds;
         return 0;
     }
+    if (r->block_map == PT_BLOCK_MAP_RUN && !RunMapPossible(r)) {
+        SetError("renderer: the RUN block map does not run on this scene and ray order (ptSetBasicRendererBlockMap)");
+        return -1;
+    }
     if (int e = EnsureSpill(r)) return e;
     if (int e = SyncRecordForm(d, r)) return e;
-    if (K > 1 || Masked(r))
-        if (int e = EnsureOrderGroups(d, r, K)) return e;
+    S.run = RunMap(r);
+    if (int e = EnsureOrderGroups(d, r, K, OrderGranule(r))) return e;
     if (K > 1)
         if (int e = EnsureGroupStreams(d, K)) return e;
     S.F = Frame(r);
@@ -298,7 +326,8 @@
 
 static int Resort(pt_basic_renderer* r, uint32_t g0, uint32_t g1, hipStream_t st)
 {
-    for (uint32_t g = g0; g < g1; g++) PT_HIP(pt_launch_tile_order(r->slots, st, r->order_groups, g));
+    for (uint32_t g = g0; g < g1; g++)
+        PT_HIP(pt_launch_tile_order(r->slots, st, r->order_groups, g, r->order_granule, r->units.ptr));
     return 0;
 }
 
@@ -314,7 +343,15 @@
         return EndTimed(d, ep);
     }
     if (int e = BeginTimed(d, PT_KERNEL_EXTEND, ep, timed)) return e;
-    PT_HIP(pt_launch_extend(r->scene->d, L, S.F, L.spill, st, train));
+    if (S.run) {
+        constexpr uint32_t G = PT_BLOCK_MAP_RUN_GRANULE;
+        const uint32_t T = r->slots.tile_count;
+        const uint32_t* units = r->units.ptr + (K > 1 ? pt_group_unit_start(T, K, g, G) : 0u);
+        PT_HIP(pt_launch_extend(r->scene->d, L, S.F, L.spill, st, train, units,
+                                K > 1 ? pt_group_unit_count(T, K, g, G) : pt_unit_count(T, G)));
+    } else {
+        PT_HIP(pt_launch_extend(r->scene->d, L, S.F, L.spill, st, train));
+    }
     if (int e = EndTimed(d, ep)) return e;
     if (int e = BeginTimed(d, PT_KERNEL_SHADE, ep, timed)) return e;
     if (S.lists) {
@@ -354,8 +391,8 @@
     hipStream_t St[PT_MAX_SPLIT];
     for (uint32_t g = 0; g < K; g++) {
         G[g] = r->slots;
-        G[g].order = r->slots.order + pt_tile_group_start(r->slots.tile_count, K, g);
-        G[g].tile_count = Masked(r) ? r->group_active[g] : pt_tile_group_count(r->slots.tile_count, K, g);
+        G[g].order = r->slots.order + pt_group_tile_start(r->slots.tile_count, K, g, r->order_granule);
+        G[g].tile_count = Masked(r) ? r->group_active[g] : pt_group_tile_count(r->slots.tile_count, K, g, r->order_granule);
         St[g] = g ? d->group_stream[g - 1] : d->stream;
     }
     if (S.lists)
@@ -518,7 +555,7 @@
             r->active_slots += (uint64_t)std::min(16u, w - tx * 16u) * std::min(16u, h - ty * 16u);
         }
     }
-    if (int e = WriteOrder(d, r, r->order_groups)) {
+    if (int e = WriteOrder(d, r, r->order_groups, PT_BLOCK_MAP_TILE_GRANULE)) {
         r->mask.swap(previous);
         r->active_tiles = previous_tiles;
         r->active_slots = previous_slots;
diff --git a/path-tracer_amd/csrc/hip/runtime.hpp b/path-tracer_amd/csrc/hip/runtime.hpp
--- a/path-tracer_amd/csrc/hip/runtime.hpp
+++ b/path-tracer_amd/csrc/hip/runtime.hpp
@@ -193,6 +193,9 @@
     uint32_t split = 0;
     ptrt::dbuf<uint32_t> guard;
     uint32_t order_groups = 1;
+    uint32_t block_map = PT_BLOCK_MAP_AUTO;
+    uint32_t order_granule = PT_BLOCK_MAP_TILE_GRANULE;
+    ptrt::dbuf<uint32_t> units;
     std::vector<uint8_t> mask;
     uint32_t active_tiles = 0;
     uint64_t active_slots = 0;
@@ -317,6 +320,9 @@
 uint32_t SplitGroups(const pt_basic_renderer* r);
 bool ClassListRounds(const pt_basic_renderer* r);
 bool LengthOrder(const pt_basic_renderer* r);
+bool RunMapPossible(const pt_basic_renderer* r);
+bool RunMap(const pt_basic_renderer* r);
+uint32_t OrderGranule(const pt_basic_renderer* r);
 int SyncRayOrder(pt_basic_renderer* r);
 
 }
diff --git a/path-tracer_amd/csrc/hip/variants.hpp b/path-tracer_amd/csrc/hip/variants.hpp
--- a/path-tracer_amd/csrc/hip/variants.hpp
+++ b/path-tracer_amd/csrc/hip/variants.hpp
@@ -70,4 +70,6 @@
 
 constexpr bool HasTrain(bool renderer_source, bool mesh, bool spill) { return renderer_source && mesh && !spill; }
 
+constexpr bool HasRunMap(bool renderer_source, bool mesh, bool spill) { return HasTrain(renderer_source, mesh, spill); }
+
 }
diff --git a/path-tracer_amd/renderer.py b/path-tracer_amd/renderer.py
--- a/path-tracer_amd/renderer.py
+++ b/path-tracer_amd/renderer.py
@@ -127,6 +127,12 @@
     def ray_order(self) -> dict:
         return dict(zip(("order", "used"), hip_get("ptGetBasicRendererRayOrder", self._h, types=(U32, U32))))
 
+    def set_block_map(self, block_map: int):
+        hip("ptSetBasicRendererBlockMap", self._h, int(block_map))
+
+    def block_map(self) -> dict:
+        return dict(zip(("map", "used"), hip_get("ptGetBasicRendererBlockMap", self._h, types=(U32, U32))))
+
     def ray_positions(self) -> np.ndarray:
         out = np.zeros(self.slot_count, dtype=np.uint16)
         hip("ptReadBasicRendererRayPositions", self.device.handle, self._h, out.ctypes.data)
@@ -207,4 +213,5 @@
         hip("ptGetBasicRendererShadeInfo", self._h, C.byref(info))
         return {"scene_mask": int(info.scene_mask), "kernel_mask": int(info.kernel_mask),
                 "completion_queue": bool(info.completion_queue), "grey_records": bool(info.grey_records),
-                "ray_order": int(info.ray_order), "length_trained": bool(info.length_trained)}
+                "ray_order": int(info.ray_order), "length_trained": bool(info.length_trained),
+                "block_map": int(info.block_map)}
```

Result: faster. 6665 Mrays/s, median of 6 (+2.2%).
